# vr308/Generalised-Gaussian-Processes

Hardware: AMD Instinct MI355X
Metric: ELBO evals/sec (higher is better)
Workload: dtype f64

## Files before the change

generalised-gaussian-processes_amd/_lib.py:

```python
from __future__ import annotations

import ctypes as C
import os

HERE = os.path.dirname(os.path.abspath(__file__))
LIB_PATH = os.path.join(HERE, "csrc", "libsgp_hip.so")

SGP_ABI_VERSION = 3
SGP_MAX_DIM = 32
SGP_MAX_INDUCING = 4096
KERNEL_IDS = {"rbf": 0, "matern32": 1, "matern52": 2, "composite": 3}
COMP_LEN = 33
OPT_CONTRACTION, OPT_ASM_OVERLAP, OPT_KFU_BUDGET_BYTES, OPT_COND_LIMIT, OPT_CU_BUDGET, OPT_TIMING, OPT_SHARED_DEVICE = range(7)
OUT_F, OUT_LOGMARG, OUT_TRACE, OUT_LOGDETB, OUT_QUAD, OUT_TRW, OUT_S2BAR, OUT_KAPPABAR, OUT_LEN = range(9)


class SgpLibraryError(RuntimeError):
    pass


class SgpStatusError(RuntimeError):
    def __init__(self, fn, status, text):
        super().__init__("%s returned %d: %s" % (fn, status, text))
        self.status = status


_vp, _i64, _i32, _dbl, _sz = C.c_void_p, C.c_int64, C.c_int, C.c_double, C.c_size_t
_dp = C.POINTER(C.c_double)
_ip = C.POINTER(C.c_int)

PROTOTYPES = {
    "sgp_abi_version": (_i32, []),
    "sgp_status_string": (C.c_char_p, [_i32]),
    "sgp_ctx_create": (_vp, [_i32]),
    "sgp_ctx_destroy": (None, [_vp]),
    "sgp_ctx_device": (_i32, [_vp]),
    "sgp_ctx_set_option": (_i32, [_vp, _i32, _dbl]),
    "sgp_ctx_get_option": (_dbl, [_vp, _i32]),
    "sgp_ctx_bind_thread": (None, [_vp]),
    "sgp_ctx_set_pass1_gate": (None, [_vp, _vp]),
    "sgp_ctx_contraction_last": (_i32, [_vp]),
    "sgp_ctx_contraction_would_use_i8": (_i32, [_vp, _i64, _i32]),
    "sgp_ctx_timing_last_ms": (_i32, [_vp, _i32, C.POINTER(C.c_float)]),
    "sgp_ctx_timing_last_rows": (_i64, [_vp, _i32]),
    "sgp_ctx_suffstats_workspace_bytes": (_sz, [_vp, _i64, _i32, _i32, _i32]),
    "sgp_ctx_suffstats_fwd": (_i32, [_vp, _vp, _i64, _vp, _vp, _i64, _dp, _dbl, _i64, _i32, _i32, _i32,
                                     _vp, _vp, _vp, _vp, _vp, _vp, _sz, _vp]),
    "sgp_ctx_suffstats_bwd": (_i32, [_vp, _vp, _i64, _vp, _vp, _i64, _dp, _dbl, _vp, _vp, _dbl, _vp, _i64, _i32, _i32, _i32,
                                     _vp, _vp, _vp, _vp, _sz, _vp]),
    "sgp_ctx_kuu_factor": (_i32, [_vp, _vp, _i32, _vp, _vp, _vp, _sz, _vp]),
    "sgp_ctx_kuu_factor_ex": (_i32, [_vp, _vp, _i32, _vp, _vp, _vp, _vp, _sz, _vp]),
    "sgp_ctx_bound_from_stats": (_i32, [_vp, _vp, _vp, _vp, _vp, _vp, _dbl, _i64, _i32, _i32, _vp,
                                        _vp, _vp, _vp, _vp, _vp, _vp, _vp, _sz, _vp]),
    "sgp_ctx_suffstats_whitened_workspace_bytes": (_sz, [_vp, _i64, _i32, _i32]),
    "sgp_ctx_suffstats_fwd_whitened": (_i32, [_vp, _vp, _i64, _vp, _vp, _i64, _dp, _dbl, _i64, _i32, _i32, _i32, _vp,
                                              _vp, _vp, _vp, _vp, _vp, _sz, _vp]),
    "sgp_ctx_suffstats_whitened_rows_workspace_bytes": (_sz, [_vp, _i64, _i32, _i32, _i32]),
    "sgp_ctx_suffstats_fwd_whitened_rows": (_i32, [_vp, _vp, _i64, _vp, _vp, _i64, _dp, _dbl, _i64, _i32, _i32, _i32, _vp,
                                                   _vp, _vp, _vp, _vp, _vp, _vp, _sz, _vp]),
    "sgp_ctx_suffstats_extended_workspace_bytes": (_sz, [_vp, _i64, _i32, _i32]),
    "sgp_ctx_suffstats_fwd_extended": (_i32, [_vp, _vp, _i64, _vp, _vp, _i64, _dp, _dbl, _i64, _i32, _i32, _i32, _vp, _i32,
                                              _vp, _vp, _vp, _vp, _vp, _vp, _vp, _sz, _vp]),
    "sgp_ctx_suffstats_fwd_extended_f16": (_i32, [_vp, _vp, _i64, _vp, _vp, _i64, _dp, _dbl, _i64, _i32, _i32, _i32, _vp, _i32,
                                                  _vp, _vp, _vp, _vp, _vp, _vp, _vp, _vp, _sz, _vp]),
    "sgp_ctx_suffstats_bwd_factored_workspace_bytes": (_sz, [_vp, _i64, _i32, _i32, _i32]),
    "sgp_ctx_suffstats_bwd_factored": (_i32, [_vp, _vp, _i64, _vp, _vp, _i64, _dp, _dbl, _vp, _vp, _dbl, _vp, _dbl, _i64, _i32, _i32, _i32,
                                              _vp, _vp, _vp, _vp, _vp, _sz, _vp]),
    "sgp_ctx_bound_from_whitened_stats": (_i32, [_vp, _vp, _vp, _vp, _vp, _dbl, _i64, _i32, _i32, _vp,
                                                 _vp, _vp, _vp, _vp, _vp, _vp, _vp, _vp, _sz, _vp]),
    "sgp_ctx_mixture_predict": (_i32, [_vp, _vp, _i64, _vp, _i64, _vp, _i64, _i64, _vp, _i64, _i32, _dp, _dp, _dp, _dbl, _i32, _i32, _i32, _i32,
                                       _dbl, _vp, _vp, _vp, _vp, _vp, _vp, _sz, _vp]),
    "sgp_ctx_mixture_predict_zs": (_i32, [_vp, _vp, _i64, _vp, _i64, _vp, _i64, _i64, _vp, _i64, _i64, _i32, _dp, _dp, _dp, _dbl, _i32, _i32, _i32, _i32, _dbl, _vp, _vp, _vp, _vp, _vp, _vp, _sz, _vp]),
    "sgp_timing_enable": (None, [_i32]),
    "sgp_timing_last_ms": (_i32, [_i32, C.POINTER(C.c_float)]),
    "sgp_timing_last_rows": (_i64, [_i32]),
    "sgp_set_asm_overlap": (None, [_i32]),
    "sgp_set_cond_limit": (None, [_dbl]),
    "sgp_suffstats_workspace_bytes": (_sz, [_i64, _i32, _i32]),
    "sgp_suffstats_workspace_bytes_ex": (_sz, [_i64, _i32, _i32, _i32]),
    "sgp_suffstats_bwd_workspace_bytes_ex": (_sz, [_i64, _i32, _i32, _i32]),
    "sgp_kfu_len": (_sz, [_i64, _i32]),
    "sgp_set_kfu_budget_bytes": (None, [_sz]),
    "sgp_set_contraction": (_i32, [_i32]),
    "sgp_contraction_last": (_i32, []),
    "sgp_set_pass1_gate": (None, [_vp]),
    "sgp_suffstats_fwd": (_i32, [_vp, _i64, _vp, _vp, _i64, _dp, _dbl, _i64, _i32, _i32, _i32,
                                 _vp, _vp, _vp, _vp, _vp, _vp, _sz, _vp]),
    "sgp_stats_packed_len": (_sz, [_i32]),
    "sgp_stats_pack_lower": (_i32, [_vp, _i32, _vp, _vp]),
    "sgp_stats_unpack_lower": (_i32, [_vp, _i32, _vp, _vp]),
    "sgp_kuu": (_i32, [_vp, _i64, _dp, _dbl, _dbl, _i32, _i32, _i32, _vp, _vp]),
    "sgp_chol_workspace_bytes": (_sz, [_i32]),
    "sgp_chol_lower": (_i32, [_vp, _i64, _i32, _vp, _vp, _sz, _vp]),
    "sgp_trsm_workspace_bytes": (_sz, [_i32, _i32]),
    "sgp_trsm_lower": (_i32, [_vp, _i64, _vp, _i64, _i32, _i32, _i32, _vp, _sz, _vp]),
    "sgp_logdiag_sum": (_i32, [_vp, _i64, _i32, _vp, _vp]),
    "sgp_bound_workspace_bytes": (_sz, [_i32, _i32]),
    "sgp_bound_factors_len": (_sz, [_i32]),
    "sgp_kuu_inverse_trace_len": (_sz, []),
    "sgp_kuu_inverse_trace": (_i32, [_vp, _i32, _vp, _vp]),
    "sgp_streaming_error_estimate": (_i32, [_vp, _vp, _dbl, _i64, _i32, _vp, _vp]),
    "sgp_streaming_error_bound": (_i32, [_vp, _dbl, _dbl, _vp, _vp]),
    "sgp_streaming_error_report": (_i32, [_vp, _i64, _vp, _dbl, _dbl, _i64, _i32, _vp, _vp]),
    "sgp_kuu_factor_len": (_sz, [_i32]),
    "sgp_kuu_factor_workspace_bytes": (_sz, [_i32]),
    "sgp_kuu_factor": (_i32, [_vp, _i32, _vp, _vp, _vp, _sz, _vp]),
    "sgp_kuu_factor_ex": (_i32, [_vp, _i32, _vp, _vp, _vp, _vp, _sz, _vp]),
    "sgp_bound_from_stats": (_i32, [_vp, _vp, _vp, _vp, _vp, _dbl, _i64, _i32, _i32, _vp,
                                    _vp, _vp, _vp, _vp, _vp, _vp, _vp, _sz, _vp]),
    "sgp_suffstats_whitened_workspace_bytes": (_sz, [_i64, _i32, _i32]),
    "sgp_suffstats_fwd_whitened": (_i32, [_vp, _i64, _vp, _vp, _i64, _dp, _dbl, _i64, _i32, _i32, _i32, _vp,
                                          _vp, _vp, _vp, _vp, _vp, _sz, _vp]),
    "sgp_suffstats_whitened_rows_workspace_bytes": (_sz, [_i64, _i32, _i32, _i32]),
    "sgp_suffstats_fwd_whitened_rows": (_i32, [_vp, _i64, _vp, _vp, _i64, _dp, _dbl, _i64, _i32, _i32, _i32, _vp,
                                               _vp, _vp, _vp, _vp, _vp, _vp, _sz, _vp]),
    "sgp_suffstats_extended_workspace_bytes": (_sz, [_i64, _i32, _i32]),
    "sgp_suffstats_fwd_extended": (_i32, [_vp, _i64, _vp, _vp, _i64, _dp, _dbl, _i64, _i32, _i32, _i32, _vp, _i32,
                                          _vp, _vp, _vp, _vp, _vp, _vp, _sz, _vp]),
    "sgp_suffstats_fwd_extended_ex": (_i32, [_vp, _i64, _vp, _vp, _i64, _dp, _dbl, _i64, _i32, _i32, _i32, _vp, _i32,
                                             _vp, _vp, _vp, _vp, _vp, _vp, _vp, _sz, _vp]),
    "sgp_phibar_dd_workspace_bytes": (_sz, [_i32]),
    "sgp_phibar_dd": (_i32, [_vp, _vp, _i32, _dbl, _vp, _vp, _vp, _sz, _vp]),
    "sgp_suffstats_bwd_lo_workspace_bytes": (_sz, [_i64, _i32, _i32]),
    "sgp_suffstats_bwd_lo": (_i32, [_vp, _i64, _vp, _vp, _i64, _dp, _dbl, _vp, _vp, _i64, _i32, _i32, _i32, _vp, _vp, _vp, _vp, _sz, _vp]),
    "sgp_suffstats_bwd_lo_workspace_bytes_ex": (_sz, [_i64, _i32, _i32, _i32]),
    "sgp_suffstats_bwd_lo_f16": (_i32, [_vp, _i64, _vp, _vp, _i64, _dp, _dbl, _vp, _vp, _vp, _i64, _i32, _i32, _i32, _vp, _vp, _vp, _vp, _sz, _vp]),
    "sgp_suffstats_fwd_extended_f16": (_i32, [_vp, _i64, _vp, _vp, _i64, _dp, _dbl, _i64, _i32, _i32, _i32, _vp, _i32,
                                              _vp, _vp, _vp, _vp, _vp, _vp, _vp, _vp, _sz, _vp]),
    "sgp_bound_from_whitened_stats": (_i32, [_vp, _vp, _vp, _vp, _dbl, _i64, _i32, _i32, _vp,
                                             _vp, _vp, _vp, _vp, _vp, _vp, _vp, _sz, _vp]),
    "sgp_bound_from_whitened_stats_ex": (_i32, [_vp, _vp, _vp, _vp, _dbl, _i64, _i32, _i32, _vp,
                                                _vp, _vp, _vp, _vp, _vp, _vp, _vp, _vp, _sz, _vp]),
    "sgp_suffstats_bwd_factored_workspace_bytes": (_sz, [_i64, _i32, _i32]),
    "sgp_suffstats_bwd_factored": (_i32, [_vp, _i64, _vp, _vp, _i64, _dp, _dbl, _vp, _vp, _dbl, _vp, _dbl, _i64, _i32, _i32, _i32,
# ... 87 lines not shown
```

generalised-gaussian-processes_amd/core.py:

```python
from __future__ import annotations

import math

import numpy as np

import torch

try:
    import torch.distributed as dist
except Exception:
    dist = None

from ._lib import COMP_LEN, OUT_F, OUT_LOGMARG, OUT_S2BAR, OUT_TRACE


class NotPositiveDefiniteError(RuntimeError):

    def __init__(self, info):
        super().__init__("matrix not positive definite: leading minor of order %d (1..M: Kuu, M+1..2M: B)" % info)
        self.info = info


class SgpTimeoutError(RuntimeError):

# ... 53 lines not shown
        self.predicted = estimate
        self.open = not (estimate < 0.5 * tol) if self.open else not (estimate <= tol)

    def note_bound(self, bound, tol):
        if math.isfinite(bound) and bound > 0.0:
            self.predicted = self.ratio * bound
            self.open = not (self.predicted < 0.5 * tol)


def _world(group):
    if dist is None or not dist.is_available() or not dist.is_initialized():
        return 1
    return dist.get_world_size(group)


class CollapsedBound:

    WHITENED_MAX_WORK = 1 << 20

    def __init__(self, X, y, kernel="rbf", jitter=0.0, engine=None, group=None, form="auto"):
        if engine is None:
            from .engine import HipEngine
            engine = HipEngine(X.device if X.is_cuda else None)
        self.engine = engine
        if X.dim() == 1:
            X = X[:, None]
        self.X = X.to(dtype=torch.float64, device=engine.device).contiguous()
        self.y = y.to(dtype=torch.float64, device=engine.device).reshape(-1).contiguous()
        if self.X.shape[0] != self.y.shape[0]:
            raise ValueError("X has %d rows, y has %d" % (self.X.shape[0], self.y.shape[0]))
        self.d = int(self.X.shape[1])
        self.kernel = kernel
        self.jitter = float(jitter)
        if form not in ("auto", "streaming", "whitened", "extended"):
            raise ValueError("form must be 'auto', 'streaming', 'extended' or 'whitened'")
        self.form = form
        self.group = group
        self.world = _world(group)
        n_local = int(self.X.shape[0])
        if self.world > 1:
            t = torch.tensor([n_local], dtype=torch.int64, device=engine.device)
            dist.all_reduce(t, group=group)
            self.N = int(t.item())
            dist.all_reduce(t.fill_(n_local), op=dist.ReduceOp.MAX, group=group)
            self._rows_for_form = int(t.item())
        else:
            self.N = n_local
            self._rows_for_form = n_local
        self.n_evals = 0
        self.n_grads = 0
        self.n_collectives = 0
        self._kfu = None
        self._kfu_f16 = None
        self.kfu_budget_bytes = 64 << 30
        self.whitened_rows_min_work = 1 << 26
        self.factored_adjoint = True
        self.fused = True
        self._small = None
        self.overlap_tail = True
        self.overlap_min_work = 1 << 21
        self.early_check_min_work = 1 << 28
        self._side = None
        self.streaming_tol = 1e-9
        self.extended_level = 2
        self.extended_range = 16384.0
        self.extended_grad_range = 3.0
        self.extended_dd_phibar = True
        self.extended_lo = True
        self.extended_grad_range_lo = 1000.0
        self.extended_lo_max_correction = 1e-4
        self._lo_skip, self._lo_pause = 0, 0
        self.last_lo_correction = None
        self.n_lo_rejections = 0
        self.guard = GuardState()
        self.last_estimate = None
        self.last_tier = None
        self.n_guard_reruns = 0
        self.n_direct_whitened = 0
        self.n_extended = 0
        self.n_timeout_retries = 0
        self._phi_diag = None

    def _allreduce(self, buf):
        if self.world > 1:
            dist.all_reduce(buf, group=self.group)
            self.n_collectives += 1
        return buf

    def _allreduce_stats(self, stats, M):
        if self.world > 1:
            e = self.engine
            if hasattr(e, "pack_lower"):
                tri = e.pack_lower(stats, M)
                dist.all_reduce(tri, group=self.group)
                e.unpack_lower(tri, M, stats)
            else:
                dist.all_reduce(stats, group=self.group)
            self.n_collectives += 1
        return stats

    def _fetch(self, res, upto=None):
        buf = res["buf"] if upto is None else res["buf"][:upto]
        host = buf.detach().to("cpu")
        o, info = self.engine.read_result(host)
        if info < 0:
            raise SgpTimeoutError()
        return o, info, host

    def _prep_Z(self, Z):
        if Z.dim() == 1:
            Z = Z[:, None]
        return Z.detach().to(dtype=torch.float64, device=self.engine.device).contiguous()

    def _kfu_for(self, M):
        e = self.engine
        if not hasattr(e, "kfu_buffer"):
            return None
        n_local = int(self.X.shape[0])
        need = ((max(n_local, 1) + 255) // 256 * 256) * ((M + 127) // 128 * 128)
        if need * 8 > self.kfu_budget_bytes:
            return None
        if self._kfu is None or self._kfu.numel() < need:
            self._kfu = e.kfu_buffer(n_local, M)
        return self._kfu

    def _kfu_f16_for(self, M):
        e = self.engine
        if not hasattr(e, "kfu_f16_buffer"):
            return None
        n_local = int(self.X.shape[0])
        need = ((max(n_local, 1) + 255) // 256 * 256) * ((M + 127) // 128 * 128)
        if need * 10 > self.kfu_budget_bytes:
            return None
        if self._kfu_f16 is None or self._kfu_f16.numel() < need:
            self._kfu_f16 = e.kfu_f16_buffer(n_local, M)
        return self._kfu_f16

    def _small_ok(self, M, want_gz=False, sf2=1.0):
        e = self.engine
        if self.kernel == "composite" and (want_gz or float(sf2) != 1.0):
            return False
        return (self.fused and self.world == 1 and self.form != "streaming" and hasattr(e, "small_eval")
                and e.small_supported(int(self.X.shape[0]), int(M), self.d, self.kernel))

    def _small_eval(self, Z, theta_host, mode, want_grad, want_gz, composite=None):
        e = self.engine
        nt = len(theta_host)
        if self._small is None or self._small[0].numel() != nt:
            pin = e.device.type == "cuda"
            host = torch.empty(nt, dtype=torch.float64, pin_memory=pin)
            self._small = (host, torch.empty(nt, dtype=torch.float64, device=e.device), e.small_result(nt - 2)[0], host.numpy())
        host, dev_theta, buf, host_np = self._small
        host_np[:] = theta_host
        dev_theta.copy_(host, non_blocking=True)
        kw = {"composite": composite} if composite is not None else {}
        out, gz, _ = e.small_eval(self.X, self.y, Z, dev_theta, self.jitter, self.kernel, mode=mode, want_grad=want_grad,
                                  want_gz=want_gz, out=buf, **kw)
        h = out.detach().to("cpu")
        info = int(h.numpy()[nt + 3:nt + 4].view("int32")[0])
        if info < 0:
            if hasattr(e, "small_reset"):
                e.small_reset()
            raise SgpTimeoutError()
        return h, info, gz

    def _whitened(self, M):
        if self.form == "auto":
            return hasattr(self.engine, "suffstats_whitened") and self._rows_for_form * int(M) <= self.WHITENED_MAX_WORK
        return self.form == "whitened"

    def _side_state(self, M):
        e = self.engine
        if self._side is None:
            if getattr(e, "_side_stream", None) is None:
                e._side_stream = torch.cuda.Stream(device=e.device, priority=-1)
            self._side = (e._side_stream, (torch.cuda.Event(), torch.cuda.Event()), {})
        bufs = self._side[2].get(M)
# ... 68 lines not shown

    def _forward(self, Z, ls, sf2, s2, with_adjoints, want_factors=False, extra=0, tier=TIER_STREAMING, report=False, want_lo=True):
        e = self.engine
        M = int(Z.shape[0])
        result = e.result_buffer(extra)
        if tier == TIER_EXTENDED:
            self.n_extended += 1
            Kuu = e.kuu(Z, ls, sf2, self.jitter, self.kernel)
            linv, _ = e.kuu_factor(Kuu, info=result[2], trace_out=self._trace_buf() if report else None)
            kfu = self._kfu_for(M) if with_adjoints else None
            diag = None
            if report:
                if self._phi_diag is None or self._phi_diag.numel() < M:
                    self._phi_diag = e.empty(M)
                diag = self._phi_diag
            dd = with_adjoints and self.extended_dd_phibar and hasattr(e, "phibar_dd")
            lo = dd and want_lo and kfu is not None and self._bwd_lo_ok(M)
            kfu_f16 = self._kfu_f16_for(M) if lo else None
            packed = e.suffstats_extended(self.X, self.y, Z, ls, sf2, linv, self.kernel, kfu=kfu, level=self.extended_level,
                                          **({"phi_diag": diag} if diag is not None else {}), **({"kfu_f16": kfu_f16} if kfu_f16 is not None else {}))
            self._allreduce_stats(packed, M)
            res = e.bound(Kuu, packed, s2, self.N, with_adjoints=with_adjoints, want_factors=want_factors, kuu_linv=linv,
                          result=result, whitened=True, **({"want_cw": True} if dd else {}))
            if dd:
                res["Phibar"], res["Phibar_lo"] = e.phibar_dd(res["Cw"], linv, s2, want_lo=lo)
                res["Cw"] = None
            if report:
                self._allreduce(diag[:M])
                e.streaming_error_report(diag, 1, self._trace_buf(), sf2, s2, self.N, M, result)
                res["reported"] = True
            res.update(packed=packed, kfu=kfu, kfu_f16=kfu_f16, t_keep=None, linv=linv)
            return res
        if tier == TIER_WHITENED:
            Kuu = e.kuu(Z, ls, sf2, self.jitter, self.kernel)
            rep = report and self.kernel != "composite"
            linv, _ = e.kuu_factor(Kuu, info=result[2], trace_out=self._trace_buf() if rep else None)
            factored = with_adjoints and self.factored_adjoint and hasattr(e, "suffstats_bwd_factored")
            t_keep = None
            if (hasattr(e, "suffstats_whitened_rows") and self.kernel != "composite"
                    and int(self.X.shape[0]) * M >= self.whitened_rows_min_work):
                t_keep = self._kfu_for(M) if factored else None
                packed = e.suffstats_whitened_rows(self.X, self.y, Z, ls, sf2, linv, self.kernel, t_out=t_keep)
            else:
                packed = e.suffstats_whitened(self.X, self.y, Z, ls, sf2, linv, self.kernel)
            self._allreduce_stats(packed, M)
            kw = {"want_cw": True} if factored else {}
            res = e.bound(Kuu, packed, s2, self.N, with_adjoints=with_adjoints, want_factors=want_factors, kuu_linv=linv,
                          result=result, whitened=True, **kw)
            if rep:
                e.streaming_error_report(None, 1, self._trace_buf(), sf2, s2, self.N, M, result)
                res["reported"] = True
            res.update(packed=packed, kfu=None, t_keep=t_keep, linv=linv)
            return res
        kfu = self._kfu_for(M) if with_adjoints else None
        gate = None
        guard = report
        trace = self._trace_buf() if guard and hasattr(e, "kuu_factor") else None
        overlap = (self.overlap_tail and hasattr(e, "kuu_factor") and e.device.type == "cuda"
                   and int(self.X.shape[0]) * M >= self.overlap_min_work)
        if overlap:
            main = torch.cuda.current_stream(e.device)
            side, (z_ready, ready), (Kuu, linv) = self._side_state(M)
            z_ready.record(main)
            side.wait_event(z_ready)
            e.kuu(Z, ls, sf2, self.jitter, self.kernel, out=Kuu, stream=side)
            e.kuu_factor(Kuu, info=result[2], trace_out=trace, out=linv, stream=side)
            ready.record(side)
            if (hasattr(e, "would_use_i8") and self.kernel != "composite" and int(self.X.shape[0]) >= 300 * M
                    and e.would_use_i8(int(self.X.shape[0]), M)):
                gate = ready
        try:
            packed = e.suffstats(self.X, self.y, Z, ls, sf2, self.kernel, kfu=kfu, **({"gate": gate} if gate is not None else {}))
            self._allreduce_stats(packed, M)
        finally:
            if overlap:
                main.wait_event(ready)
        if overlap:
            res = e.bound(Kuu, packed, s2, self.N, with_adjoints=with_adjoints, want_factors=want_factors, kuu_linv=linv,
                          result=result)
        elif guard and hasattr(e, "kuu_factor"):
            Kuu = e.kuu(Z, ls, sf2, self.jitter, self.kernel)
            linv, _ = e.kuu_factor(Kuu, info=result[2], trace_out=trace)
            res = e.bound(Kuu, packed, s2, self.N, with_adjoints=with_adjoints, want_factors=want_factors, kuu_linv=linv,
                          result=result)
        else:
            Kuu = e.kuu(Z, ls, sf2, self.jitter, self.kernel)
            res = e.bound(Kuu, packed, s2, self.N, with_adjoints=with_adjoints, want_factors=want_factors, result=result)
        if guard and trace is not None:
            e.streaming_error_report(packed, M + 1, trace, sf2, s2, self.N, M, result)
            res["reported"] = True
        res["packed"] = packed
        res["kfu"] = kfu
        return res

    def _pass2(self, res, Z, ls, sf2, s2, want_gz, g):
        e = self.engine
        if res.get("Cw") is not None:
            e.suffstats_bwd_factored(self.X, self.y, Z, ls, sf2, res["linv"], res["Cw"], s2, res["bbar"], -1.0 / (2.0 * float(s2)),
                                     self.kernel, want_gz=want_gz, out=g,
                                     **({"t_in": res["t_keep"]} if res.get("t_keep") is not None else {}))
        else:
            e.suffstats_bwd(self.X, self.y, Z, ls, sf2, res["Phibar"], res["bbar"], -1.0 / (2.0 * float(s2)),
                            self.kernel, want_gz=want_gz, out=g, kfu=res["kfu"])
            if res.get("Phibar_lo") is not None:
                n_lo = int(res.get("lo_slots", 0))
                e.suffstats_bwd_lo(self.X, self.y, Z, ls, sf2, res["Phibar_lo"], res["kfu"], g, self.kernel,
                                   **({"delta": g[g.numel() - n_lo:]} if n_lo else {}),
                                   **({"kfu_f16": res["kfu_f16"]} if res.get("kfu_f16") is not None else {}))
        if int(res.get("lo_slots", 0)) and res.get("Phibar_lo") is None:
            g[g.numel() - int(res["lo_slots"]):].zero_()
        self._allreduce(g)
        e.kuu_bwd(Z, ls, sf2, res["Kuubar"], g, self.kernel, want_gz=want_gz)

    def _evaluate(self, *args, **kw):
        try:
            return self._evaluate_once(*args, **kw)
        except SgpTimeoutError:
            e = self.engine
            if "shared_device" not in getattr(e, "OPTIONS", {}) or e.get_option("shared_device") != 0:
                raise
            e.set_option("shared_device", 1)
            self.n_timeout_retries += 1
            return self._evaluate_once(*args, **kw)

    def _evaluate_once(self, Z, ls, sf2, s2, with_grad=False, want_gz=False, want_factors=False, grad_reach=None, strict=False):
        e = self.engine
        M, d = int(Z.shape[0]), int(Z.shape[1])
        guard = self._guard_on(M)
        reach = self.extended_range
        if with_grad:
            reach = float(grad_reach) if grad_reach is not None else (self.extended_grad_range_lo if self._bwd_lo_ok(M) else self.extended_grad_range)
        ext_ok = self._extended_ok(M)
        if guard:
            tier = self.guard.start_tier(self.streaming_tol, reach, ext_ok)
            if strict and tier == TIER_WHITENED:
                tier = TIER_EXTENDED if ext_ok else TIER_STREAMING
            if tier != TIER_STREAMING:
                self.n_direct_whitened += 1
        else:
            tier = self._fixed_tier(M)
        nh = (e.hyper_len(self.kernel, d) if hasattr(e, "hyper_len") else d) if with_grad else 0
        lo_slots = (nh + 1) if (with_grad and guard and ext_ok and self._bwd_lo_ok(M)) else 0
        extra = nh + 1 + (M * d if want_gz else 0) + lo_slots if with_grad else 0
        if guard and with_grad and tier == TIER_EXTENDED and grad_reach is None and self._lo_skip > 0:
            self._lo_skip -= 1
            tier = TIER_WHITENED
        early = with_grad and self._rows_for_form * M >= self.early_check_min_work
        done = {}
        may_go_down = strict
        while True:
            res = self._forward(Z, ls, sf2, s2, with_adjoints=with_grad, want_factors=want_factors, extra=extra, tier=tier, report=guard,
                                want_lo=grad_reach is None)
            head = res["buf"].numel() - extra
            g = res["buf"][head:] if with_grad else None
            res["lo_slots"] = lo_slots
            grad_upto = None if lo_slots else head + nh + 1
# ... 270 lines not shown
```

generalised-gaussian-processes_amd/csrc/sgp_ctx.hip:

```cpp
#include "sgp_common.hpp"
#include "sgp_ctx.hpp"
#include "sgp_stream.hpp"
#include <cstdlib>
#include <new>

namespace sgp {

static int env_int(const char* name, int dflt) {
  const char* v = getenv(name);
  return v ? atoi(v) : dflt;
}

static void ctx_init(Ctx& c, int device) {
  c.device = device;
  c.contraction = env_int("SGP_CONTRACTION", 1);
  if (c.contraction < 0 || c.contraction > 2) c.contraction = 1;
  c.asm_overlap = env_int("SGP_ASM_OVERLAP", 0);
  c.kfu_budget = KFU_BUDGET_DEFAULT;
  c.syrk_skip_upper = env_int("SGP_SYRK_SKIP_UPPER", 1);
  c.syrk_waves = env_int("SGP_SYRK_WAVES", 4);
  c.syrk_glds = env_int("SGP_SYRK_GLDS", 0);
  c.i8_prio = env_int("SGP_I8_PRIO", 0);
  c.shared_device = env_int("SGP_SHARED_DEVICE", 0) != 0 ? 1 : 0;
}

Ctx& default_ctx() {
  static Ctx* c = [] {
    Ctx* p = new Ctx();
    int dev = 0;
    if (hipGetDevice(&dev) != hipSuccess) dev = 0;
    ctx_init(*p, dev);
    return p;
  }();
  return *c;
}

static thread_local Ctx* t_cur = nullptr;
static thread_local Ctx* t_bound = nullptr;
Ctx& cur_ctx() { return t_cur ? *t_cur : (t_bound ? *t_bound : default_ctx()); }
void bind_thread_ctx(void* ctx) { t_bound = static_cast<Ctx*>(ctx); }
CtxScope::CtxScope(void* ctx) : prev(t_cur) { t_cur = ctx ? static_cast<Ctx*>(ctx) : &default_ctx(); }
CtxScope::~CtxScope() { t_cur = prev; }

}

using namespace sgp;

static bool ctx_on_current_device(const sgp_ctx* ctx) {
  if (!ctx) return true;
  int dev = -1;
  if (hipGetDevice(&dev) != hipSuccess) return true;
  return dev == reinterpret_cast<const Ctx*>(ctx)->device;
}

extern "C" sgp_ctx* sgp_ctx_create(int device) {
  if (device < 0) return nullptr;
  Ctx* c = new (std::nothrow) Ctx();
  if (!c) return nullptr;
  ctx_init(*c, device);
  return reinterpret_cast<sgp_ctx*>(c);
}

extern "C" void sgp_ctx_destroy(sgp_ctx* ctx) {
  if (!ctx) return;
  Ctx* c = reinterpret_cast<Ctx*>(ctx);
  if (c == &default_ctx()) return;
  if (c->ev_ready)
    for (int s = 0; s < CTX_TIMING_SLOTS; ++s)
      for (int k = 0; k < 2; ++k) (void)hipEventDestroy(c->ev[s][k]);
  if (c->side) {
    (void)hipStreamDestroy(c->side);
    (void)hipEventDestroy(c->ev_fork);
    (void)hipEventDestroy(c->ev_join);
  }
  delete c;
}

extern "C" int sgp_ctx_set_option(sgp_ctx* ctx, int option, double value) {
  Ctx& c = ctx ? *reinterpret_cast<Ctx*>(ctx) : default_ctx();
  switch (option) {
    case SGP_OPT_CONTRACTION:
      if (!(value >= 0.0 && value <= 2.0)) return SGP_ERR_ARG;
      c.contraction = (int)value;
      return SGP_OK;
    case SGP_OPT_ASM_OVERLAP:
      if (!(value >= 0.0 && value <= 2.0)) return SGP_ERR_ARG;
      c.asm_overlap = (int)value;
      return SGP_OK;
    case SGP_OPT_KFU_BUDGET_BYTES:
      if (!(value >= 0.0)) return SGP_ERR_ARG;
      c.kfu_budget = value > 0.0 ? (size_t)value : KFU_BUDGET_DEFAULT;
      return SGP_OK;
    case SGP_OPT_COND_LIMIT:
      c.cond_limit = value >= 0.0 ? value : 1e13;
      return SGP_OK;
    case SGP_OPT_CU_BUDGET:
      c.cu_budget = value > 0.0 ? (int)value : 0;
      return SGP_OK;
    case SGP_OPT_TIMING:
      c.timing = value != 0.0 ? 1 : 0;
      return SGP_OK;
    case SGP_OPT_SHARED_DEVICE:
      c.shared_device = value != 0.0 ? 1 : 0;
      return SGP_OK;
    default:
      return SGP_ERR_ARG;
  }
}

extern "C" double sgp_ctx_get_option(const sgp_ctx* ctx, int option) {
  const Ctx& c = ctx ? *reinterpret_cast<const Ctx*>(ctx) : default_ctx();
  switch (option) {
    case SGP_OPT_CONTRACTION: return (double)c.contraction;
    case SGP_OPT_ASM_OVERLAP: return (double)c.asm_overlap;
    case SGP_OPT_KFU_BUDGET_BYTES: return (double)c.kfu_budget;
    case SGP_OPT_COND_LIMIT: return c.cond_limit;
    case SGP_OPT_CU_BUDGET: return (double)c.cu_budget;
    case SGP_OPT_TIMING: return (double)c.timing;
    case SGP_OPT_SHARED_DEVICE: return (double)c.shared_device;
    default: return -1.0;
  }
}

extern "C" void sgp_ctx_bind_thread(sgp_ctx* ctx) { sgp::bind_thread_ctx(ctx); }

extern "C" int sgp_ctx_device(const sgp_ctx* ctx) { return (ctx ? *reinterpret_cast<const Ctx*>(ctx) : default_ctx()).device; }

extern "C" void sgp_ctx_set_pass1_gate(sgp_ctx* ctx, void* hip_event) {
  (ctx ? *reinterpret_cast<Ctx*>(ctx) : default_ctx()).pass1_gate = (hipEvent_t)hip_event;
}

extern "C" int sgp_ctx_contraction_last(const sgp_ctx* ctx) {
  return (ctx ? *reinterpret_cast<const Ctx*>(ctx) : default_ctx()).contraction_used;
}

extern "C" size_t sgp_ctx_suffstats_workspace_bytes(const sgp_ctx* ctx, int64_t N, int M, int d, int caller_owns_kfu) {
  CtxScope scope(const_cast<sgp_ctx*>(ctx));
  return sgp_suffstats_workspace_bytes_ex(N, M, d, caller_owns_kfu);
}
extern "C" int sgp_ctx_suffstats_fwd(sgp_ctx* ctx, const double* X, int64_t ldx, const double* y, const double* Z, int64_t ldz,
                                     const double* inv_ls, double sf2, int64_t N, int M, int d, int kernel_id, double* Phi, double* b,
                                     double* yy, double* kappa, double* Kfu_out, void* ws, size_t ws_bytes, sgp_stream_t stream) {
  if (!ctx_on_current_device(ctx)) return SGP_ERR_ARG;
  CtxScope scope(ctx);
  return sgp_suffstats_fwd(X, ldx, y, Z, ldz, inv_ls, sf2, N, M, d, kernel_id, Phi, b, yy, kappa, Kfu_out, ws, ws_bytes, stream);
}
extern "C" int sgp_ctx_suffstats_bwd(sgp_ctx* ctx, const double* X, int64_t ldx, const double* y, const double* Z, int64_t ldz,
                                     const double* inv_ls, double sf2, const double* Phibar, const double* bbar, double kappabar,
                                     const double* Kfu_in, int64_t N, int M, int d, int kernel_id, double* g_ls, double* g_sf2,
                                     double* g_Z, void* ws, size_t ws_bytes, sgp_stream_t stream) {
  if (!ctx_on_current_device(ctx)) return SGP_ERR_ARG;
  CtxScope scope(ctx);
  return sgp_suffstats_bwd(X, ldx, y, Z, ldz, inv_ls, sf2, Phibar, bbar, kappabar, Kfu_in, N, M, d, kernel_id, g_ls, g_sf2, g_Z, ws,
                           ws_bytes, stream);
}
extern "C" int sgp_ctx_kuu_factor(sgp_ctx* ctx, const double* Kuu, int M, double* Linv_out, int* info, void* ws, size_t ws_bytes,
                                  sgp_stream_t stream) {
  if (!ctx_on_current_device(ctx)) return SGP_ERR_ARG;
  CtxScope scope(ctx);
  return sgp_kuu_factor(Kuu, M, Linv_out, info, ws, ws_bytes, stream);
}
extern "C" int sgp_ctx_kuu_factor_ex(sgp_ctx* ctx, const double* Kuu, int M, double* Linv_out, int* info, double* trace_out, void* ws,
                                     size_t ws_bytes, sgp_stream_t stream) {
  if (!ctx_on_current_device(ctx)) return SGP_ERR_ARG;
  CtxScope scope(ctx);
  return sgp_kuu_factor_ex(Kuu, M, Linv_out, info, trace_out, ws, ws_bytes, stream);
}
extern "C" int sgp_ctx_bound_from_stats(sgp_ctx* ctx, const double* Kuu, const double* Phi, const double* b, const double* yy,
                                        const double* kappa, double s2, int64_t N, int M, int with_adjoints, double* out,
                                        double* Phibar, double* bbar, double* Kuubar, double* factors, const double* kuu_linv,
                                        int* info, void* ws, size_t ws_bytes, sgp_stream_t stream) {
  if (!ctx_on_current_device(ctx)) return SGP_ERR_ARG;
  CtxScope scope(ctx);
  return sgp_bound_from_stats(Kuu, Phi, b, yy, kappa, s2, N, M, with_adjoints, out, Phibar, bbar, Kuubar, factors, kuu_linv, info, ws,
                              ws_bytes, stream);
}
extern "C" int sgp_ctx_mixture_predict(sgp_ctx* ctx, const double* X, int64_t ldx, const double* y, int64_t N, const double* Xs,
                                       int64_t ldxs, int64_t T, const double* Z, int64_t ldz, int S, const double* inv_ls,
                                       const double* sf2, const double* s2, double jitter, int M, int d, int kernel_id, int pred_noise,
                                       double gate_jitter, double* mean, double* var, double* cov, int* info, int* gate_info, void* ws,
                                       size_t ws_bytes, sgp_stream_t stream) {
  if (!ctx_on_current_device(ctx)) return SGP_ERR_ARG;
  CtxScope scope(ctx);
  return sgp_mixture_predict(X, ldx, y, N, Xs, ldxs, T, Z, ldz, S, inv_ls, sf2, s2, jitter, M, d, kernel_id, pred_noise, gate_jitter,
                             mean, var, cov, info, gate_info, ws, ws_bytes, stream);
}

extern "C" size_t sgp_ctx_suffstats_whitened_workspace_bytes(const sgp_ctx* ctx, int64_t N, int M, int d) {
  CtxScope scope(const_cast<sgp_ctx*>(ctx));
  return sgp_suffstats_whitened_workspace_bytes(N, M, d);
}
extern "C" int sgp_ctx_suffstats_fwd_whitened(sgp_ctx* ctx, const double* X, int64_t ldx, const double* y, const double* Z, int64_t ldz,
                                              const double* inv_ls, double sf2, int64_t N, int M, int d, int kernel_id,
                                              const double* kuu_linv, double* W, double* u, double* yy, double* kappa, void* ws,
                                              size_t ws_bytes, sgp_stream_t stream) {
  if (!ctx_on_current_device(ctx)) return SGP_ERR_ARG;
  CtxScope scope(ctx);
  return sgp_suffstats_fwd_whitened(X, ldx, y, Z, ldz, inv_ls, sf2, N, M, d, kernel_id, kuu_linv, W, u, yy, kappa, ws, ws_bytes, stream);
}
extern "C" size_t sgp_ctx_suffstats_whitened_rows_workspace_bytes(const sgp_ctx* ctx, int64_t N, int M, int d, int caller_owns_t) {
  CtxScope scope(const_cast<sgp_ctx*>(ctx));
  return sgp_suffstats_whitened_rows_workspace_bytes(N, M, d, caller_owns_t);
}
extern "C" int sgp_ctx_suffstats_fwd_whitened_rows(sgp_ctx* ctx, const double* X, int64_t ldx, const double* y, const double* Z,
                                                   int64_t ldz, const double* inv_ls, double sf2, int64_t N, int M, int d, int kernel_id,
                                                   const double* kuu_linv, double* W, double* u, double* yy, double* kappa,
                                                   double* T_out, void* ws, size_t ws_bytes, sgp_stream_t stream) {
// ... 62 lines not shown
```

generalised-gaussian-processes_amd/csrc/sgp_ctx.hpp:

```cpp
#pragma once
#include <hip/hip_runtime.h>
#include <cstddef>
#include <cstdint>

namespace sgp {

constexpr int CTX_TIMING_SLOTS = 3;

struct Ctx {
  int device = 0;
  int contraction = 1;
  int asm_overlap = 0;
  size_t kfu_budget = 0;
  double cond_limit = 1e13;
  int cu_budget = 0;
  int timing = 0;
  int shared_device = 0;
  int syrk_skip_upper = 1, syrk_waves = 4, syrk_glds = 0, i8_prio = 0;
  int contraction_used = 0;
  hipEvent_t pass1_gate = nullptr;
  int64_t syrk_timed_rows = 0;
  hipEvent_t ev[CTX_TIMING_SLOTS][2] = {};
  int ev_ready = 0, ev_used[CTX_TIMING_SLOTS] = {0, 0, 0};
  hipStream_t side = nullptr;
  hipEvent_t ev_fork = nullptr, ev_join = nullptr;
};

Ctx& default_ctx();
Ctx& cur_ctx();

void bind_thread_ctx(void* ctx);

struct CtxScope {
  Ctx* prev;
  explicit CtxScope(void* ctx);
  ~CtxScope();
  CtxScope(const CtxScope&) = delete;
  CtxScope& operator=(const CtxScope&) = delete;
};

}
```

generalised-gaussian-processes_amd/csrc/sgp_stream.hpp:

```cpp
#pragma once
#include <cstdlib>
#include "sgp_common.hpp"

namespace sgp {

constexpr int TILE = 128;
constexpr int NB = 16;
constexpr int KROW = 2 * TILE + 16;
constexpr int ASM_ROWS = 256;
constexpr int TARGET_WGS = 2048;
constexpr int RESIDENT_WGS = 512;
constexpr size_t KFU_BUDGET_DEFAULT = size_t(16) << 30;
size_t stream_kfu_budget();

static inline int dp_for(int d) {
  const int opts[] = {2, 4, 8, 16, 24, 32};
  for (int o : opts)
    if (d <= o) return o;
  return -1;
}

struct StreamPlan {
  int Mp, ntr, ntiles, DP;
  int64_t Npad;
// ... 108 lines not shown
  if (taper_b_on && nsb % 32 == 0 && nblocks / nsb >= 8) {
    const int B = (int)(nsb / 8);
    p.taper_b[0] = 3 * B / 4; p.taper_b[1] = B / 4; p.taper_b[2] = B / 4; p.taper_b[3] = B / 2;
    p.nsplit_b = 8 * (p.taper_b[0] + p.taper_b[1] + p.taper_b[2] + p.taper_b[3]);
  }
  return p;
}

enum { TIMING_ASSEMBLE = 0, TIMING_SYRK = 1, TIMING_KBAR = 2, TIMING_SLOTS = 3 };
void timing_begin(int slot, hipStream_t st);
void timing_end(int slot, hipStream_t st);

struct PadSymJob {
  const double* P = nullptr;
  double* out = nullptr;
  const double* vec = nullptr;
  double* vout = nullptr;
};
void stream_prologue(const StreamPlan& p, const KernArgs& ka, const double* X, int64_t ldx, const double* y,
                     const double* Z, int64_t ldz, int64_t N, int M, double* Xs, double* ys, double* Zs, double* yypart,
                     hipStream_t st, const PadSymJob& pad = PadSymJob());
void stream_assemble(const StreamPlan& p, int kid, const double* Xs, const double* ys, const double* Zs, int64_t row0,
                     int64_t rows, int64_t N, int M, double* Kfu, double* bpart, hipStream_t st);

constexpr int I8_SPLIT_ROWS = 16384;
static inline int i8_nsplit(int64_t rows, int Mp) {
  const int nrt = Mp / 128, ntiles = nrt * (nrt + 1);
  int64_t lo = (rows + I8_SPLIT_ROWS - 1) / I8_SPLIT_ROWS;
  lo = (lo + 7) / 8 * 8;
  if (lo < 8) lo = 8;
  int64_t best = lo;
  double best_waste = 2.0;
  for (int64_t cand = lo; cand <= 2 * lo + 8; cand += 8) {
    if (cand > lo && rows / cand < 2048) break;
    const double r = (double)ntiles * (double)cand / 256.0;
    const double rounds = (double)(int64_t)(r + 0.999999);
    const double waste = (rounds - r) / rounds;
    if (waste < best_waste - 1e-9) {
      best_waste = waste;
      best = cand;
    }
  }
  return (int)best;
}
__host__ __device__ inline void i8_split_steps(int64_t nsteps, int nsplit, int split, int64_t& c0, int64_t& c1) {
  const int64_t per = (nsteps + nsplit - 1) / nsplit;
  c0 = (int64_t)split * per;
  c1 = c0 + per;
  if (c0 > nsteps) c0 = nsteps;
  if (c1 > nsteps) c1 = nsteps;
}
void i8_assemble(const StreamPlan& p, int kid, const double* Xs, const double* ys, const double* Zs, int64_t row0, int64_t rows,
                 int64_t N, int M, uint8_t* Q, double* Kfu , double* bpart, hipStream_t st,
                 uint16_t* Kh = nullptr );
int i8_contract(const uint8_t* Q, int Mp, int64_t rows, int nsplit, int accumulate, double* slab, hipStream_t st, double* slab_lo = nullptr,
                int level = 1);

}
```

generalised-gaussian-processes_amd/csrc/sgp_suffstats_bwd.hip:

```cpp
#include "sgp_common.hpp"
#include "sgp_stream.hpp"
#include "sgp_composite.hpp"
#include "sgp_dense.hpp"
#include <cstdlib>

namespace sgp {

constexpr int BK = 16;
constexpr int ALD = BK + 2;
constexpr int BROW = TILE + 16;
constexpr int A_DBL = TILE * ALD;
constexpr int B_DBL = BK * BROW;
constexpr int BSM = 2 * (A_DBL + B_DBL);
constexpr int CS = 129;
static_assert(64 * CS <= BSM, "epilogue image must fit in the main-loop buffers");

__global__ void bwd_pad_vec_kernel(const double* __restrict__ in, int64_t n, int64_t npad, double* __restrict__ out) {
  for (int64_t i = (int64_t)blockIdx.x * blockDim.x + threadIdx.x; i < npad; i += (int64_t)gridDim.x * blockDim.x)
    out[i] = i < n ? in[i] : 0.0;
}
__global__ void bwd_pad_plain_kernel(const double* __restrict__ P, int M, int Mp, double scale, double* __restrict__ out) {
  const int64_t total = (int64_t)Mp * Mp;
  for (int64_t e = (int64_t)blockIdx.x * blockDim.x + threadIdx.x; e < total; e += (int64_t)gridDim.x * blockDim.x) {
    const int r = (int)(e / Mp), c = (int)(e - (int64_t)r * Mp);
    out[e] = (r < M && c < M) ? scale * P[e] : 0.0;
  }
}
__global__ void bwd_pad_small_kernel(const double* __restrict__ P, int M, int Mp, double scale, double* __restrict__ out) {
  const int64_t total = (int64_t)Mp * Mp;
  for (int64_t e = (int64_t)blockIdx.x * blockDim.x + threadIdx.x; e < total; e += (int64_t)gridDim.x * blockDim.x) {
    const int r = (int)(e / Mp), c = (int)(e - (int64_t)r * Mp);
    out[e] = (r < M && c < M) ? scale * P[(int64_t)r * M + c] : 0.0;
  }
}

template <int KID>
__device__ __forceinline__ double hprime_from_k(double kp, double r2) {
  if constexpr (KID == SGP_KERNEL_RBF) {
    return -0.5 * kp;
  } else if constexpr (KID == SGP_KERNEL_MATERN32) {
    const double a = 1.7320508075688772 * sqrt(r2);
    return -1.5 * kp / (1.0 + a);
  } else {
    const double a = 2.23606797749979 * sqrt(r2);
    return -(5.0 / 6.0) * (1.0 + a) * kp / (1.0 + a + a * a * (1.0 / 3.0));
  }
}

template <int DP, int KID, bool KP>
constexpr bool kbar_two_pass() {
#ifdef SGP_AB_KBAR_TWO_PASS_ALL
  return KP && KID == SGP_KERNEL_RBF;
#else
  return KP && DP > 8 && KID == SGP_KERNEL_RBF;
#endif
}
// ... 150 lines not shown
            gl[k] = fresh ? 0.0 : gmine[(size_t)(j0 + k) * 256];
            gz[k] = (fresh || !GZ) ? 0.0 : gmine[(size_t)(DP + j0 + k) * 256];
          }
#pragma unroll 2
          for (int i = 0; i < 32; ++i) {
            const double* __restrict__ xq = Xs + (nbase + i) * DP + j0;
            const double E = Ct[half * 32 + i][erow];
#pragma unroll
            for (int k = 0; k < DG; ++k) {
              const double df = zg[k] - xq[k];
              const double t = E * df;
              if constexpr (GZ) gz[k] += t;
              gl[k] = fma(t, df, gl[k]);
            }
          }
#pragma unroll
          for (int k = 0; k < DG; ++k) {
            gmine[(size_t)(j0 + k) * 256] = gl[k];
            if constexpr (GZ) gmine[(size_t)(DP + j0 + k) * 256] = gz[k];
          }
        }
        __syncthreads();
      }
      gmine[(size_t)(2 * DP) * 256] = gs;
    } else {
    double zrow[DP], gl[DP], gz[DP], gs;
#pragma unroll
    for (int j = 0; j < DP; ++j) {
      zrow[j] = Zs[(size_t)(m0 + erow) * DP + j];
      gl[j] = first ? 0.0 : gmine[(size_t)j * 256];
      gz[j] = (first || !want_gz) ? 0.0 : gmine[(size_t)(DP + j) * 256];
    }
    gs = first ? 0.0 : gmine[(size_t)(2 * DP) * 256];
#pragma unroll
    for (int h = 0; h < 2; ++h) {
      if (wi == h) {
#pragma unroll
        for (int u = 0; u < 4; ++u)
#pragma unroll
          for (int v = 0; v < 4; ++v)
#pragma unroll
            for (int r = 0; r < 4; ++r) Ct[u * 16 + l4 + 4 * r][wj * 64 + v * 16 + l15] = acc[u][v][r];
      }
      __syncthreads();
#if defined(SGP_AB_KBAR_NO_EPI_MATH)
      for (int i = 0; i < 32; ++i) gs += Ct[half * 32 + i][erow];
      if (false)
#endif
      SGP_KBAR_EPI_UNROLL
      for (int i = 0; i < 32; ++i) {
        const int nl = half * 32 + i;
        const int64_t n = row0 + r0 + h * 64 + nl;
        const double* __restrict__ xq = Xs + n * DP;
        double df[DP];
        double r2 = 0.0;
#pragma unroll
        for (int j = 0; j < DP; ++j) {
          df[j] = zrow[j] - xq[j];
          r2 = fma(df[j], df[j], r2);
        }
        double kp, hp;
        kprofile_grad<KID>(r2, kp, hp);
        const double msk = n < N ? mmask : 0.0;
        const double kbar = (2.0 * sf2 * Ct[nl][erow] + bbm * ys[n]) * msk;
        gs = fma(kbar, kp, gs);
        const double E = kbar * sf2 * hp;
#pragma unroll
        for (int j = 0; j < DP; ++j) {
          const double t = E * df[j];
          if constexpr (GZ) gz[j] += t;
          gl[j] = fma(t, df[j], gl[j]);
        }
      }
      __syncthreads();
    }
#pragma unroll
    for (int j = 0; j < DP; ++j) {
      gmine[(size_t)j * 256] = gl[j];
      if (want_gz) gmine[(size_t)(DP + j) * 256] = gz[j];
    }
    gmine[(size_t)(2 * DP) * 256] = gs;
    }
  }

  double gl[DP], gz[DP], gs;
  {
    const bool any = nb0 < nb1;
#pragma unroll
    for (int j = 0; j < DP; ++j) {
      gl[j] = any ? gmine[(size_t)j * 256] : 0.0;
      gz[j] = (any && want_gz) ? gmine[(size_t)(DP + j) * 256] : 0.0;
    }
    gs = any ? gmine[(size_t)(2 * DP) * 256] : 0.0;
  }
  double* scratch = smem;
  if (want_gz) {
#pragma unroll
    for (int j = 0; j < DP; ++j) {
      __syncthreads();
      if (half == 1) scratch[erow] = gz[j];
      __syncthreads();
      if (half == 0) {
        double* dst = gzpart + ((size_t)split * Mp + m0 + erow) * DP + j;
        const double v = gz[j] + scratch[erow];
        *dst = accumulate ? *dst + v : v;
      }
    }
  }
  auto block_total = [&](double v, int slot) {
    v = wave_sum(v);
    __syncthreads();
    if (lane == 0) scratch[wave] = v;
    __syncthreads();
    if (tid == 0) {
      double* dst = glpart + ((size_t)split * nmb + mb) * (DP + 1) + slot;
      const double t = scratch[0] + scratch[1] + scratch[2] + scratch[3];
      *dst = accumulate ? *dst + t : t;
    }
  };
#pragma unroll
  for (int j = 0; j < DP; ++j) block_total(gl[j], j);
  block_total(gs, DP);
}

__global__ __launch_bounds__(256) void bwd_reduce_kernel(const double* __restrict__ gzpart, const double* __restrict__ glpart,
// ... 96 lines not shown
  if (kernel_id == SGP_KERNEL_COMPOSITE) {
    CompSpec cs;
    if (comp_parse(inv_ls, d, &cs) != SGP_OK) return SGP_ERR_ARG;
    fill_zero(g_sf2, 1, (hipStream_t)stream);
    return comp_suffstats_bwd(X, ldx, y, Z, ldz, cs, Phibar, bbar, kappabar, N, M, d, g_ls, g_Z, ws, ws_bytes, (hipStream_t)stream);
  }
  StreamPlan p = make_stream_plan(N, M, d);
  if (Kfu_in) p.sc_rows = p.Npad;
  BwdWs w = carve_bwd(ws, p, Kfu_in == nullptr);
  if (!ws || ws_bytes < w.bytes) return SGP_ERR_WORKSPACE;
  hipStream_t st = (hipStream_t)stream;

  KernArgs ka;
  for (int j = 0; j < SGP_MAX_DIM; ++j) ka.inv_ls[j] = j < d ? inv_ls[j] : 0.0;
  ka.sf2 = sf2;
  ka.d = d;

  {
    PadSymJob pad;
    pad.P = Phibar; pad.out = w.Pb; pad.vec = bbar; pad.vout = w.bb;
    stream_prologue(p, ka, X, ldx, y, Z, ldz, N, M, w.Xs, w.ys, w.Zs, w.yypart, st, pad);
  }

  const int want_gz = g_Z != nullptr;
  const int grid = p.nmb * p.nsplit_b;
  auto launch = [&](const double* Kfu, int64_t row0, int64_t nblocks, int accumulate) {
    int bps = (int)((nblocks + p.nsplit_b - 1) / p.nsplit_b);
    if (bps < 1) bps = 1;
    switch (p.DP) {
      case 2: launch_bwd<2>(kernel_id, grid, st, Kfu, w, sf2, row0, nblocks, bps, N, M, p, want_gz, accumulate); break;
      case 4: launch_bwd<4>(kernel_id, grid, st, Kfu, w, sf2, row0, nblocks, bps, N, M, p, want_gz, accumulate); break;
      case 8: launch_bwd<8>(kernel_id, grid, st, Kfu, w, sf2, row0, nblocks, bps, N, M, p, want_gz, accumulate); break;
      case 16: launch_bwd<16>(kernel_id, grid, st, Kfu, w, sf2, row0, nblocks, bps, N, M, p, want_gz, accumulate); break;
      case 24: launch_bwd<24>(kernel_id, grid, st, Kfu, w, sf2, row0, nblocks, bps, N, M, p, want_gz, accumulate); break;
      default: launch_bwd<32>(kernel_id, grid, st, Kfu, w, sf2, row0, nblocks, bps, N, M, p, want_gz, accumulate); break;
    }
  };
  if (p.Npad == 0) launch(nullptr, 0, 0, 0);
  for (int64_t r0 = 0; r0 < p.Npad; r0 += p.sc_rows) {
    const int64_t rows = (p.Npad - r0) < p.sc_rows ? (p.Npad - r0) : p.sc_rows;
    const double* Kfu = Kfu_in ? Kfu_in + r0 * p.Mp : nullptr;
    if (!Kfu_in) {
      stream_assemble(p, kernel_id, w.Xs, w.ys, w.Zs, r0, rows, N, M, w.Kfu, w.bpart, st);
      Kfu = w.Kfu;
    }
    timing_begin(TIMING_KBAR, st);
    launch(Kfu, r0, rows / TILE, r0 > 0 ? 1 : 0);
    timing_end(TIMING_KBAR, st);
  }
  const int64_t tot = (int64_t)M * d;
  const int rg = (int)((tot + 255) / 256 < 1024 ? (tot + 255) / 256 : 1024);
  bwd_reduce_kernel<<<rg < 1 ? 1 : rg, 256, 0, st>>>(w.gzpart, w.glpart, p.nsplit_b, p.nmb, p.Mp, M, p.DP, ka,
                                                    kappabar * (double)N, g_ls, g_sf2, g_Z);
  return check_launch();
}

static int bwd_fully_factored() {
  static const int v = getenv("SGP_BWD_FULLY_FACTORED") ? atoi(getenv("SGP_BWD_FULLY_FACTORED")) : 0;
  return v;
}
static size_t bwd_factored_workspace_bytes(int64_t N, int M, int d, bool caller_t) {
  if (N < 0 || M <= 0 || d <= 0 || d > SGP_MAX_DIM || M > SGP_MAX_INDUCING) return 0;
  StreamPlan p = make_stream_plan(N, M, d);
  p.sc_rows = p.Npad;
  const int nt = (caller_t ? 0 : 1) + (bwd_fully_factored() ? 1 : 0);
  const size_t fast = carve_bwd(nullptr, p, !caller_t).bytes + nt * round_up64((int64_t)(p.Npad > 0 ? p.Npad : 1) * p.Mp * 8 + 256, 256) +
                      3 * round_up64((int64_t)p.Mp * p.Mp * 8 + 256, 256);
  const size_t comp = d <= COMP_MAX_DIM ? comp_bwd_factored_workspace_bytes(N, M, d) : 0;
  return fast > comp ? fast : comp;
}
extern "C" size_t sgp_suffstats_bwd_factored_workspace_bytes(int64_t N, int M, int d) { return bwd_factored_workspace_bytes(N, M, d, false); }
extern "C" size_t sgp_suffstats_bwd_factored_workspace_bytes_ex(int64_t N, int M, int d, int caller_owns_t) {
  return bwd_factored_workspace_bytes(N, M, d, caller_owns_t != 0);
}

static int bwd_factored(const double* X, int64_t ldx, const double* y, const double* Z, int64_t ldz, const double* inv_ls, double sf2,
                        const double* kuu_linv, const double* Cw, double s2, const double* bbar, double kappabar, int64_t N, int M,
                        int d, int kernel_id, const double* T_in, double* g_ls, double* g_sf2, double* g_Z, void* ws, size_t ws_bytes,
                        sgp_stream_t stream) {
  if (!Z || !inv_ls || !kuu_linv || !Cw || !bbar || !g_ls || !g_sf2 || N < 0 || M <= 0 || d <= 0 || ldz < d || !(s2 > 0.0))
    return SGP_ERR_ARG;
  if (N > 0 && (!X || !y || ldx < d)) return SGP_ERR_ARG;
  if (kernel_id < 0 || kernel_id > SGP_KERNEL_COMPOSITE) return SGP_ERR_ARG;
  if (T_in && kernel_id == SGP_KERNEL_COMPOSITE) return SGP_ERR_ARG;
  if (d > SGP_MAX_DIM || M > SGP_MAX_INDUCING) return SGP_ERR_DIM;
  hipStream_t st = (hipStream_t)stream;
  if (!ws || ws_bytes < bwd_factored_workspace_bytes(N, M, d, T_in != nullptr)) return SGP_ERR_WORKSPACE;
  if (kernel_id == SGP_KERNEL_COMPOSITE) {
    CompSpec cs;
    if (comp_parse(inv_ls, d, &cs) != SGP_OK) return SGP_ERR_ARG;
    fill_zero(g_sf2, 1, st);
    return comp_suffstats_bwd_factored(X, ldx, y, Z, ldz, cs, kuu_linv, Cw, s2, bbar, kappabar, N, M, d, g_ls, g_Z, ws, ws_bytes, st);
  }
  const int fully = bwd_fully_factored();
  StreamPlan p = make_stream_plan(N, M, d);
  p.sc_rows = p.Npad;
  BwdWs w = carve_bwd(ws, p, T_in == nullptr);
  Carver c(static_cast<char*>(ws) + round_up64((int64_t)w.bytes, 256));
  const size_t rows = (size_t)(p.Npad > 0 ? p.Npad : 1);
  double* T1 = T_in ? nullptr : c.take<double>(rows * p.Mp);
  double* T2 = fully ? c.take<double>(rows * p.Mp) : nullptr;
  double* P2 = c.take<double>((size_t)p.Mp * p.Mp);
  double* Q0 = c.take<double>((size_t)p.Mp * p.Mp);
  double* R = c.take<double>((size_t)p.Mp * p.Mp);

  KernArgs ka;
// ... 71 lines not shown
```

generalised-gaussian-processes_amd/csrc/sgp_suffstats_fwd.hip:

```cpp
#include "sgp_common.hpp"
#include "sgp_stream.hpp"
#include "sgp_dense.hpp"
#include "sgp_composite.hpp"
#include "sgp_ctx.hpp"
#include <cstdlib>

namespace sgp {

static_assert(TIMING_SLOTS == CTX_TIMING_SLOTS, "timing slots");
size_t stream_kfu_budget() { return cur_ctx().kfu_budget; }

void timing_begin(int slot, hipStream_t st) {
  Ctx& c = cur_ctx();
  if (!c.timing) return;
  if (!c.ev_ready) {
    bool ok = true;
    for (int s = 0; s < TIMING_SLOTS; ++s)
      for (int k = 0; k < 2; ++k) ok = (hipEventCreate(&c.ev[s][k]) == hipSuccess) && ok;
    if (!ok) return;
    c.ev_ready = 1;
  }
  if (hipEventRecord(c.ev[slot][0], st) != hipSuccess) c.ev_used[slot] = 0;
}
void timing_end(int slot, hipStream_t st) {
// ... 754 lines not shown
  return w;
}

}

using namespace sgp;

static int ctx_timing_last_ms(Ctx& c, int slot, float* ms) {
  if (slot < 0 || slot >= TIMING_SLOTS || !ms) return SGP_ERR_ARG;
  if (!c.ev_ready || !c.ev_used[slot]) return SGP_ERR_ARG;
  if (hipEventSynchronize(c.ev[slot][1]) != hipSuccess) return SGP_ERR_LAUNCH;
  return hipEventElapsedTime(ms, c.ev[slot][0], c.ev[slot][1]) == hipSuccess ? SGP_OK : SGP_ERR_LAUNCH;
}
extern "C" int sgp_ctx_timing_last_ms(sgp_ctx* ctx, int slot, float* ms) {
  return ctx_timing_last_ms(ctx ? *reinterpret_cast<Ctx*>(ctx) : default_ctx(), slot, ms);
}
extern "C" int64_t sgp_ctx_timing_last_rows(const sgp_ctx* ctx, int slot) {
  return slot == TIMING_SYRK ? (ctx ? *reinterpret_cast<const Ctx*>(ctx) : default_ctx()).syrk_timed_rows : -1;
}
extern "C" int sgp_ctx_contraction_would_use_i8(const sgp_ctx* ctx, int64_t N, int M) {
  if (N <= 0 || M <= 0 || M > SGP_MAX_INDUCING) return 0;
  return i8_rule((ctx ? *reinterpret_cast<const Ctx*>(ctx) : default_ctx()).contraction, round_up64(N, ASM_ROWS), padded_m(M)) ? 1 : 0;
}

extern "C" void sgp_timing_enable(int on) { default_ctx().timing = on ? 1 : 0; }
extern "C" int sgp_timing_last_ms(int slot, float* ms) { return ctx_timing_last_ms(default_ctx(), slot, ms); }
extern "C" int64_t sgp_timing_last_rows(int slot) { return sgp_ctx_timing_last_rows(nullptr, slot); }
extern "C" void sgp_set_asm_overlap(int mode) { default_ctx().asm_overlap = (mode < 0 || mode > 2) ? 0 : mode; }
extern "C" int sgp_set_contraction(int mode) {
  const int prev = default_ctx().contraction;
  default_ctx().contraction = (mode < 0 || mode > 2) ? 1 : mode;
  return prev;
}
extern "C" int sgp_contraction_last(void) { return default_ctx().contraction_used; }
extern "C" void sgp_set_pass1_gate(void* hip_event) { default_ctx().pass1_gate = (hipEvent_t)hip_event; }
extern "C" void sgp_set_kfu_budget_bytes(size_t bytes) { default_ctx().kfu_budget = bytes ? bytes : KFU_BUDGET_DEFAULT; }

extern "C" size_t sgp_kfu_len(int64_t N, int M) {
  if (N < 0 || M <= 0 || M > SGP_MAX_INDUCING) return 0;
  return (size_t)round_up64(N > 0 ? N : 1, ASM_ROWS) * padded_m(M);
}

static size_t fwd_workspace_bytes(int64_t N, int M, int d, bool library_kfu) {
  if (N < 0 || M <= 0 || d <= 0 || d > SGP_MAX_DIM || M > SGP_MAX_INDUCING) return 0;
  StreamPlan p = make_stream_plan(N, M, d);
  const size_t fast = carve_fwd(nullptr, p, library_kfu, p.sc_rows).bytes, comp = comp_fwd_workspace_bytes(N, M);
  return fast > comp ? fast : comp;
}
extern "C" size_t sgp_suffstats_workspace_bytes(int64_t N, int M, int d) { return fwd_workspace_bytes(N, M, d, true); }
extern "C" size_t sgp_suffstats_workspace_bytes_ex(int64_t N, int M, int d, int caller_owns_kfu) {
  return fwd_workspace_bytes(N, M, d, caller_owns_kfu == 0);
}

extern "C" int sgp_suffstats_fwd(const double* X, int64_t ldx, const double* y, const double* Z, int64_t ldz,
                                 const double* inv_ls, double sf2, int64_t N, int M, int d, int kernel_id,
                                 double* Phi, double* b, double* yy, double* kappa, double* Kfu_out, void* ws,
                                 size_t ws_bytes, sgp_stream_t stream) {
  Ctx& cx = cur_ctx();
  hipEvent_t gate = cx.pass1_gate;
  cx.pass1_gate = nullptr;
  if (!Z || !inv_ls || !Phi || !b || !yy || !kappa || N < 0 || M <= 0 || d <= 0 || ldz < d) return SGP_ERR_ARG;
  if (N > 0 && (!X || !y || ldx < d)) return SGP_ERR_ARG;
  if (kernel_id < 0 || kernel_id > SGP_KERNEL_COMPOSITE) return SGP_ERR_ARG;
  if (d > SGP_MAX_DIM || M > SGP_MAX_INDUCING) return SGP_ERR_DIM;
  if (kernel_id == SGP_KERNEL_COMPOSITE) {
    CompSpec cs;
    if (comp_parse(inv_ls, d, &cs) != SGP_OK) return SGP_ERR_ARG;
    return comp_suffstats_fwd(X, ldx, y, Z, ldz, cs, N, M, d, Phi, b, yy, kappa, ws, ws_bytes, (hipStream_t)stream);
  }
  StreamPlan p = make_stream_plan(N, M, d);
  const int64_t qrows = p.sc_rows;
  if (Kfu_out) p.sc_rows = p.Npad;
  FwdWs w = carve_fwd(ws, p, Kfu_out == nullptr, qrows);
  if (!ws || ws_bytes < w.bytes) return SGP_ERR_WORKSPACE;
  hipStream_t st = (hipStream_t)stream;

  KernArgs ka;
  for (int j = 0; j < SGP_MAX_DIM; ++j) ka.inv_ls[j] = j < d ? inv_ls[j] : 0.0;
  ka.sf2 = sf2;
  ka.d = d;

  stream_prologue(p, ka, X, ldx, y, Z, ldz, N, M, w.Xs, w.ys, w.Zs, w.yypart, st);
  double* Kfu = Kfu_out ? Kfu_out : w.Kfu;
  const int grid = p.ntiles * p.nsplit;
  if (p.Npad == 0) {
    syrk_tile_kernel<4, false, false><<<grid, 256, 0, st>>>(Kfu, p.Mp, 0, SplitMap{{0, 0, 0, 0}, 1}, p.ntiles, 0, w.slab, p.nsplit);
  }
  auto contract = [&](const double* K, int64_t nchunks, const SplitMap& smap, int nsplit, int accum, double* slab) {
    launch_syrk(cx, K, p.Mp, nchunks, smap, p.ntiles, nsplit, accum, slab, st);
  };
  int nslabs = p.nsplit;
  int head_ns = 0;
  int64_t head_chunks = 0;
  const bool use_i8 = i8_rule(cx.contraction, p.Npad, p.Mp);
  cx.contraction_used = use_i8 ? 1 : 0;
  if (!use_i8) gate = nullptr;
  if (p.Npad > 0 && !use_i8) head_block(p, p.Npad / NB, &head_ns, &head_chunks);
  if (use_i8) {
    const int ns = i8_nsplit(qrows, p.Mp);
    for (int64_t r0 = 0; r0 < p.Npad; r0 += qrows) {
      const int64_t rows = (p.Npad - r0) < qrows ? (p.Npad - r0) : qrows;
      timing_begin(TIMING_ASSEMBLE, st);
      i8_assemble(p, kernel_id, w.Xs, w.ys, w.Zs, r0, rows, N, M, w.Q, Kfu_out ? Kfu_out + (size_t)r0 * p.Mp : nullptr, w.bpart, st);
      timing_end(TIMING_ASSEMBLE, st);
      if (gate && hipStreamWaitEvent(st, gate, 0) != hipSuccess) return SGP_ERR_LAUNCH;
      gate = nullptr;
      timing_begin(TIMING_SYRK, st);
      if (i8_contract(w.Q, p.Mp, rows, ns, r0 > 0 ? 1 : 0, w.slab, st) != SGP_OK) return SGP_ERR_LAUNCH;
      timing_end(TIMING_SYRK, st);
      cx.syrk_timed_rows = rows;
    }
    nslabs = ns;
  } else if (head_ns > 0) {
    const int64_t hrows = head_chunks * NB, trows = p.Npad - hrows, tchunks = trows / NB;
    const bool side = cx.asm_overlap == 1 && side_stream_ready(cx);
    double* head_slab = w.slab + (size_t)p.nsplit * p.ntiles * TILE * TILE;
    const int hcps = (int)((head_chunks + head_ns - 1) / head_ns);
    const int tcps = (int)((tchunks + p.nsplit - 1) / p.nsplit);
    const SplitMap hmap{{0, 0, 0, 0}, hcps < 1 ? 1 : hcps};
    const SplitMap tmap{{p.taper[0], p.taper[1], p.taper[2], p.taper[3]}, tcps < 1 ? 1 : tcps};
    timing_begin(TIMING_ASSEMBLE, st);
    stream_assemble(p, kernel_id, w.Xs, w.ys, w.Zs, 0, hrows, N, M, Kfu, w.bpart, st);
    bool forked = false;
    if (side && hipEventRecord(cx.ev_fork, st) == hipSuccess && hipStreamWaitEvent(cx.side, cx.ev_fork, 0) == hipSuccess) {
      stream_assemble(p, kernel_id, w.Xs, w.ys, w.Zs, hrows, trows, N, M, Kfu + (size_t)hrows * p.Mp, w.bpart, cx.side);
      forked = hipEventRecord(cx.ev_join, cx.side) == hipSuccess;
      if (!forked) (void)hipStreamSynchronize(cx.side);
    } else {
      stream_assemble(p, kernel_id, w.Xs, w.ys, w.Zs, hrows, trows, N, M, Kfu + (size_t)hrows * p.Mp, w.bpart, st);
    }
    timing_end(TIMING_ASSEMBLE, st);
    contract(Kfu, head_chunks, hmap, head_ns, 0, head_slab);
    if (forked && hipStreamWaitEvent(st, cx.ev_join, 0) != hipSuccess) (void)hipStreamSynchronize(cx.side);
    timing_begin(TIMING_SYRK, st);
    contract(Kfu + (size_t)hrows * p.Mp, tchunks, tmap, p.nsplit, 0, w.slab);
    timing_end(TIMING_SYRK, st);
    cx.syrk_timed_rows = trows;
    nslabs = p.nsplit + head_ns;
  } else {
    for (int64_t r0 = 0; r0 < p.Npad; r0 += p.sc_rows) {
      const int64_t rows = (p.Npad - r0) < p.sc_rows ? (p.Npad - r0) : p.sc_rows;
      timing_begin(TIMING_ASSEMBLE, st);
      stream_assemble(p, kernel_id, w.Xs, w.ys, w.Zs, r0, rows, N, M, Kfu, w.bpart, st);
      timing_end(TIMING_ASSEMBLE, st);
      const int64_t nchunks = rows / NB;
      const int cps = (int)((nchunks + p.nsplit - 1) / p.nsplit);
      const SplitMap smap{{p.taper[0], p.taper[1], p.taper[2], p.taper[3]}, cps < 1 ? 1 : cps};
      timing_begin(TIMING_SYRK, st);
      contract(Kfu, nchunks, smap, p.nsplit, r0 > 0 ? 1 : 0, w.slab);
      timing_end(TIMING_SYRK, st);
      cx.syrk_timed_rows = rows;
    }
  }
  const int nb32 = p.Mp / 32;
  reduce_phi_kernel<<<nb32 * (nb32 + 1) / 2, 256, 0, st>>>(w.slab, nslabs, p.ntiles, M, sf2 * sf2, Phi);
  bpart_stage1_kernel<<<dim3(p.Mp / 64, BRED_G), 256, 0, st>>>(w.bpart, p.Npad / ASM_ROWS * (use_i8 ? 1 : p.asm_sub), p.Mp, BRED_G, w.btmp);
  finalize_stats_kernel<<<(M + 255) / 256, 256, 0, st>>>(w.btmp, BRED_G, p.Mp, M, w.yypart, 256, sf2,
                                                         sf2 * (double)N, b, yy, kappa);
  return check_launch();
}

extern "C" size_t sgp_suffstats_whitened_rows_workspace_bytes(int64_t N, int M, int d, int caller_owns_t) {
  if (N < 0 || M <= 0 || d <= 0 || d > SGP_MAX_DIM || M > SGP_MAX_INDUCING) return 0;
  StreamPlan p = make_stream_plan(N, M, d);
  if (caller_owns_t) p.sc_rows = p.Npad;
  return carve_wh_rows(nullptr, p, caller_owns_t != 0).bytes;
}
extern "C" int sgp_suffstats_fwd_whitened_rows(const double* X, int64_t ldx, const double* y, const double* Z, int64_t ldz,
                                               const double* inv_ls, double sf2, int64_t N, int M, int d, int kernel_id,
                                               const double* kuu_linv, double* W, double* u, double* yy, double* kappa, double* T_out,
                                               void* ws, size_t ws_bytes, sgp_stream_t stream) {
  Ctx& cx = cur_ctx();
  if (!Z || !inv_ls || !kuu_linv || !W || !u || !yy || !kappa || N < 0 || M <= 0 || d <= 0 || ldz < d) return SGP_ERR_ARG;
  if (N > 0 && (!X || !y || ldx < d)) return SGP_ERR_ARG;
  if (kernel_id < 0 || kernel_id >= SGP_KERNEL_COMPOSITE) return SGP_ERR_ARG;
  if (d > SGP_MAX_DIM || M > SGP_MAX_INDUCING) return SGP_ERR_DIM;
  StreamPlan p = make_stream_plan(N, M, d);
  if (T_out) p.sc_rows = p.Npad;
  WhRowsWs w = carve_wh_rows(ws, p, T_out != nullptr);
  if (!ws || ws_bytes < w.bytes) return SGP_ERR_WORKSPACE;
  hipStream_t st = (hipStream_t)stream;
  KernArgs ka;
  for (int j = 0; j < SGP_MAX_DIM; ++j) ka.inv_ls[j] = j < d ? inv_ls[j] : 0.0;
  ka.sf2 = sf2;
  ka.d = d;
  stream_prologue(p, ka, X, ldx, y, Z, ldz, N, M, w.f.Xs, w.f.ys, w.f.Zs, w.f.yypart, st);
  transpose_square(kuu_linv, p.Mp, w.R, st);
  if (p.Npad == 0)
    syrk_tile_kernel<4, false, false><<<p.ntiles * p.nsplit, 256, 0, st>>>(w.f.Kfu, p.Mp, 0, SplitMap{{0, 0, 0, 0}, 1}, p.ntiles, 0, w.f.slab,
                                                                           p.nsplit);
  for (int64_t r0 = 0; r0 < p.Npad; r0 += p.sc_rows) {
    const int64_t rows = (p.Npad - r0) < p.sc_rows ? (p.Npad - r0) : p.sc_rows;
    double* T = T_out ? T_out + (size_t)r0 * p.Mp : w.T;
    timing_begin(TIMING_ASSEMBLE, st);
    stream_assemble(p, kernel_id, w.f.Xs, w.f.ys, w.f.Zs, r0, rows, N, M, w.f.Kfu, w.f.bpart, st);
    timing_end(TIMING_ASSEMBLE, st);
    GemmDesc g;
    g.A = w.f.Kfu; g.lda = p.Mp; g.B = w.R; g.ldb = p.Mp; g.C = T; g.ldc = p.Mp;
    g.m = (int)rows; g.n = p.Mp; g.k = p.Mp; g.khi_mask = 2;
    gemm(g, st);
    tpart_kernel<<<dim3((unsigned)(rows / ASM_ROWS), (p.Mp + 255) / 256), 256, 0, st>>>(T, w.f.ys, r0, p.Mp, w.f.bpart);
    const int64_t nchunks = rows / NB;
    const int cps = (int)((nchunks + p.nsplit - 1) / p.nsplit);
    const SplitMap smap{{p.taper[0], p.taper[1], p.taper[2], p.taper[3]}, cps < 1 ? 1 : cps};
    timing_begin(TIMING_SYRK, st);
    launch_syrk(cx, T, p.Mp, nchunks, smap, p.ntiles, p.nsplit, r0 > 0 ? 1 : 0, w.f.slab, st);
    timing_end(TIMING_SYRK, st);
    cx.syrk_timed_rows = rows;
  }
  const int nb32 = p.Mp / 32;
  reduce_phi_kernel<<<nb32 * (nb32 + 1) / 2, 256, 0, st>>>(w.f.slab, p.nsplit, p.ntiles, M, sf2 * sf2, W);
  bpart_stage1_kernel<<<dim3(p.Mp / 64, BRED_G), 256, 0, st>>>(w.f.bpart, p.Npad / ASM_ROWS, p.Mp, BRED_G, w.f.btmp);
// ... 74 lines not shown
```

generalised-gaussian-processes_amd/csrc/sgp_suffstats_i8.hip:

```cpp
#include <atomic>
#include "sgp_common.hpp"
#include "sgp_stream.hpp"
#include "sgp_ctx.hpp"
#include <cstdlib>
#include <type_traits>

namespace sgp {

typedef int i4v __attribute__((ext_vector_type(4)));
typedef int i16v __attribute__((ext_vector_type(16)));

constexpr int I8_NP = 7;
constexpr int I8_TR = 128, I8_TC = 64;
constexpr int I8_SCOLS = I8_TR + I8_TC;
constexpr int I8_STAGE_BYTES = 2 * I8_NP * I8_SCOLS * 16;
constexpr int I8_NSTAGE = 3;
constexpr int I8_PIECES = 2 * I8_NP * 3;
constexpr int I8_PPW = (I8_PIECES + 7) / 8;
constexpr int I8_LDS_BYTES = I8_NSTAGE * I8_STAGE_BYTES;

template <int DP, int KID, bool WK>
__global__ __launch_bounds__(256) void kfu_digits_kernel(const double* __restrict__ Xs, const double* __restrict__ ys,
                                                         const double* __restrict__ Zs, int64_t row0, int64_t N, int M, int Mp,
                                                         uint8_t* __restrict__ Q, double* __restrict__ Kfu, uint16_t* __restrict__ Kh,
                                                         double* __restrict__ bpart) {
  __shared__ double xs[ASM_ROWS][DP];
  __shared__ double ysh[ASM_ROWS];
  __shared__ double etab[EXP_TAB_N];
  const int64_t rbase = (int64_t)blockIdx.x * ASM_ROWS;
  {
    const double* src = Xs + (row0 + rbase) * DP;
    double* dst = &xs[0][0];
    for (int e = threadIdx.x; e < ASM_ROWS * DP; e += 256) dst[e] = src[e];
    ysh[threadIdx.x] = ys[row0 + rbase + threadIdx.x];
    sgp_exp_tab_load(etab);
  }
  __syncthreads();
  const int m = blockIdx.y * 256 + threadIdx.x;
  if (m >= Mp) return;
  const double zmask = m < M ? 1.0 : 0.0;
  double zr[DP];
#pragma unroll
  for (int j = 0; j < DP; ++j) zr[j] = Zs[(size_t)m * DP + j];

  constexpr unsigned long long C = 0x0080808080808080ULL;
  double bacc = 0.0;
#ifdef SGP_AB_DIGITS_NO_INTERIOR
  const bool interior = false;
#else
  const bool interior = (row0 + rbase + ASM_ROWS <= N) && ((int)(blockIdx.y * 256 + 255) < M);
#endif
  auto run = [&](auto masked_tag) {
  constexpr bool MASKED = decltype(masked_tag)::value;
  for (int g = 0; g < ASM_ROWS / 16; ++g) {
    unsigned lo[16], hi[16];
#pragma unroll
    for (int e = 0; e < 16; ++e) {
      const int i = g * 16 + e;
      const int64_t n = row0 + rbase + i;
      double r2 = 0.0;
#pragma unroll
      for (int j = 0; j < DP; ++j) {
        const double df = xs[i][j] - zr[j];
        r2 = fma(df, df, r2);
      }
      double kv = kprofile_tab<KID>(r2, etab);
      if constexpr (MASKED) kv *= (n < N ? zmask : 0.0);
      bacc = fma(kv, ysh[i], bacc);
      if constexpr (WK) {
        __builtin_nontemporal_store(kv, &Kfu[(rbase + i) * Mp + m]);
        if (Kh) {
          float kf = (float)kv;
          asm volatile("" : "+v"(kf));
          Kh[(rbase + i) * Mp + m] = __builtin_bit_cast(uint16_t, (_Float16)kf);
        }
      }
      const double th = fma(kv, 0x1p22, 0x1p52);
      const double hf = th - 0x1p52;
      const double tl = fma(-hf, 0x1p32, kv * 0x1p54) + 0x1.8p52;
      const unsigned long long tb = (unsigned long long)__double_as_longlong(tl);
      const unsigned q_hi = (unsigned)__double_as_longlong(th) - ((unsigned)(tb >> 32) & 1u);
      const unsigned long long q = ((unsigned long long)q_hi << 32) | (unsigned)tb;
      const unsigned long long qq = (q + C) ^ C;
      lo[e] = (unsigned)qq;
      hi[e] = (unsigned)(qq >> 32);
    }
    const size_t rb = (size_t)(rbase / 16 + g);
    i4v plane[8];
#pragma unroll
    for (int j = 0; j < 4; ++j) {
#pragma unroll
      for (int h = 0; h < 2; ++h) {
        const unsigned* s4 = (h ? hi : lo) + 4 * j;
        const unsigned u0 = __builtin_amdgcn_perm(s4[1], s4[0], 0x05010400u), u1 = __builtin_amdgcn_perm(s4[1], s4[0], 0x07030602u);
        const unsigned v0 = __builtin_amdgcn_perm(s4[3], s4[2], 0x05010400u), v1 = __builtin_amdgcn_perm(s4[3], s4[2], 0x07030602u);
        plane[4 * h + 0][j] = (int)__builtin_amdgcn_perm(v0, u0, 0x05040100u);
        plane[4 * h + 1][j] = (int)__builtin_amdgcn_perm(v0, u0, 0x07060302u);
        plane[4 * h + 2][j] = (int)__builtin_amdgcn_perm(v1, u1, 0x05040100u);
        if (h == 0) plane[3][j] = (int)__builtin_amdgcn_perm(v1, u1, 0x07060302u);
      }
    }
#pragma unroll
    for (int p = 0; p < I8_NP; ++p)
      __builtin_nontemporal_store(plane[p], reinterpret_cast<i4v*>(Q + ((rb * I8_NP + p) * Mp + m) * 16));
  }
  };
  if (interior) run(std::false_type{}); else run(std::true_type{});
  bpart[((row0 + rbase) / ASM_ROWS) * Mp + m] = bacc;
}

constexpr int I8_PSPLIT = 5;
#ifdef SGP_AB_I8_PAIRS34
constexpr int I8_MINSUM_DEFAULT = 5;
#else
constexpr int I8_MINSUM_DEFAULT = 6;
#endif
static_assert(2 * I8_PPW - 1 <= I8_PSPLIT * (I8_PSPLIT + 1) / 2, "every DMA piece must find its MFMA in the first half");

template <bool ACT, int I8_MINSUM, bool DD>
__device__ __forceinline__ void i8_tile_loop(uint8_t* lds, const uint8_t* __restrict__ Q, int Mp, int64_t c0, int64_t c1, int I0,
                                             int J0, int accumulate, double* __restrict__ out, size_t lo_off, int wave, int lane, int prio) {
  constexpr int I8_NG = 13 - I8_MINSUM;
  const int grp = wave >> 2, w4 = wave & 3;
  const int wi = (w4 >> 1) * 2 + grp, wj = w4 & 1;
  const int l32 = lane & 31, lh = lane >> 5;
  i16v acc[I8_NG];
#pragma unroll
  for (int g = 0; g < I8_NG; ++g)
#pragma unroll
    for (int r = 0; r < 16; ++r) acc[g][r] = 0;

  unsigned goff[I8_PPW];
  int soff[I8_PPW];
#pragma unroll
  for (int k = 0; k < I8_PPW; ++k) {
    int e = wave + 8 * k;
    if (e >= I8_PIECES) e -= I8_PIECES;
    const int rbl = e / (I8_NP * 3), rem = e % (I8_NP * 3), p = rem / 3, cg = rem % 3;
    const int col = cg < 2 ? I0 + cg * 64 : J0;
    goff[k] = (unsigned)(((rbl * I8_NP + p) * Mp + col + lane) * 16);
    soff[k] = __builtin_amdgcn_readfirstlane(((rbl * I8_NP + p) * I8_SCOLS + cg * 64) * 16);
  }
  const size_t gstride = (size_t)2 * I8_NP * Mp * 16;
  auto dma_piece = [&](const uint8_t* gbase, int sbase, int k) {
    __builtin_amdgcn_global_load_lds((const __attribute__((address_space(1))) void*)(gbase + goff[k]),
                                     (__attribute__((address_space(3))) void*)(lds + sbase + soff[k]), 16, 0, 0);
  };
  const int64_t nst = c1 - c0;
  auto wait_stage = [&](int64_t sE) {
    if (sE + 1 >= nst)
      __builtin_amdgcn_s_waitcnt(0 | (7 << 4) | (15 << 8));
    else
      __builtin_amdgcn_s_waitcnt((I8_PPW & 15) | ((I8_PPW >> 4) << 14) | (7 << 4) | (15 << 8));
  };
  auto bar = [&]() {
    __builtin_amdgcn_s_barrier();
    asm volatile("" ::: "memory");
  };
  i4v b[I8_NP], a[I8_NP];
  auto reads = [&](int64_t sidx) {
    if (ACT) {
      const uint8_t* sb = lds + (int)(sidx % I8_NSTAGE) * I8_STAGE_BYTES + lh * (I8_NP * I8_SCOLS * 16);
#pragma unroll
      for (int p = 0; p < I8_NP; ++p) {
        b[I8_NP - 1 - p] = *reinterpret_cast<const i4v*>(sb + ((I8_NP - 1 - p) * I8_SCOLS + I8_TR + wj * 32 + l32) * 16);
        a[p] = *reinterpret_cast<const i4v*>(sb + (p * I8_SCOLS + wi * 32 + l32) * 16);
      }
    }
    __builtin_amdgcn_sched_barrier(0);
  };
  auto half = [&](int p0, int p1, bool dma_on, int64_t sE) {
    if (prio) { if (dma_on) __builtin_amdgcn_s_setprio(1); else __builtin_amdgcn_s_setprio(0); }
    const bool pre = dma_on && sE + 2 < nst;
    const uint8_t* gnext = Q + (size_t)(c0 + sE + 2) * gstride;
    const int snext = (int)((sE + 2) % I8_NSTAGE) * I8_STAGE_BYTES;
    int issued = 0, kpiece = 0;
#pragma unroll
    for (int p = p0; p < p1; ++p)
#pragma unroll
      for (int r = (I8_MINSUM - p > 0 ? I8_MINSUM - p : 0); r < I8_NP; ++r) {
        if (ACT) acc[p + r - I8_MINSUM] = __builtin_amdgcn_mfma_i32_32x32x32_i8(a[p], b[r], acc[p + r - I8_MINSUM], 0, 0, 0);
        ++issued;
        if (dma_on && (issued & 1) && kpiece < I8_PPW) {
          __builtin_amdgcn_sched_barrier(0);
          if (pre) dma_piece(gnext, snext, kpiece);
          __builtin_amdgcn_sched_barrier(0);
          ++kpiece;
        }
      }
  };
  if (nst > 0) {
#pragma unroll
    for (int k = 0; k < I8_PPW; ++k) dma_piece(Q + (size_t)c0 * gstride, 0, k);
    if (nst > 1) {
#pragma unroll
      for (int k = 0; k < I8_PPW; ++k) dma_piece(Q + (size_t)(c0 + 1) * gstride, I8_STAGE_BYTES, k);
    }
    if (grp == 0) {
      for (int64_t sidx = 0; sidx < nst; ++sidx) {
        wait_stage(sidx);
        bar();
        reads(sidx);
        half(0, I8_PSPLIT, true, sidx);
        bar();
        half(I8_PSPLIT, I8_NP, false, sidx);
      }
      wait_stage(nst);
      bar();
    } else {
      wait_stage(0);
      bar();
      for (int64_t sidx = 0; sidx < nst; ++sidx) {
        bar();
        reads(sidx);
        half(0, I8_PSPLIT, true, sidx);
        __builtin_amdgcn_s_waitcnt(15 | (3 << 14) | (7 << 4) | (0 << 8));
        wait_stage(sidx + 1);
        bar();
        half(I8_PSPLIT, I8_NP, false, sidx + 1);
      }
    }
  }
  if (ACT) {
#pragma unroll
    for (int r = 0; r < 16; ++r) {
      const int row = wi * 32 + (r >> 2) * 8 + lh * 4 + (r & 3);
      double* dst = out + row * TILE + wj * 32 + l32;
      if constexpr (DD) {
#pragma clang fp contract(off)
        double hi = 0.0, lo = 0.0;
        if (accumulate) { hi = dst[0]; lo = dst[lo_off]; }
#pragma unroll
        for (int g = 0; g < I8_NG; ++g) {
          const double t = (double)acc[g][r] * __builtin_ldexp(1.0, 8 * (g + I8_MINSUM) - 108);
          const double sum = hi + t;
          const double z = sum - hi;
          lo += (hi - (sum - z)) + (t - z);
          hi = sum;
        }
        const double sum = hi + lo;
        dst[lo_off] = lo - (sum - hi);
        dst[0] = sum;
      } else {
        double v = 0.0;
#pragma unroll
        for (int g = 0; g < I8_NG; ++g) v = fma((double)acc[g][r], __builtin_ldexp(1.0, 8 * (g + I8_MINSUM) - 108), v);
        *dst = accumulate ? *dst + v : v;
      }
    }
  }
}

template <int MINSUM, bool DD>
__global__ __launch_bounds__(512, 1) void i8_syrk_tile_kernel(const uint8_t* __restrict__ Q, int Mp, int64_t nsteps, int nsplit,
                                                              int ntiles, int ntiles128, int accumulate, double* __restrict__ slab,
                                                              size_t lo_off, int prio) {
  extern __shared__ __attribute__((aligned(16))) uint8_t i8_lds[];
  const int id = blockIdx.x;
  const int xcd = id & 7, jj = id >> 3;
  const int t = jj % ntiles, split = (jj / ntiles) * 8 + xcd;
  if (split >= nsplit) return;
  int ti = (int)((sqrtf(4.0f * t + 1.0f) - 1.0f) * 0.5f);
  while ((ti + 1) * (ti + 2) <= t) ++ti;
  while (ti * (ti + 1) > t) --ti;
  const int tj = t - ti * (ti + 1);
  const int I0 = ti * I8_TR, J0 = tj * I8_TC;
  int64_t c0, c1;
  i8_split_steps(nsteps, nsplit, split, c0, c1);
  const int lane = threadIdx.x & 63;
  const int wave = __builtin_amdgcn_readfirstlane(threadIdx.x >> 6);
  double* out = slab + ((size_t)split * ntiles128 + (ti * (ti + 1) / 2 + (tj >> 1))) * (TILE * TILE) + (tj & 1) * I8_TC;
  const int grp = wave >> 2, w4 = wave & 3;
  const int wi = (w4 >> 1) * 2 + grp, wj = w4 & 1;
  if (J0 + 32 * wj <= I0 + 32 * wi + 31)
    i8_tile_loop<true, MINSUM, DD>(i8_lds, Q, Mp, c0, c1, I0, J0, accumulate, out, lo_off, wave, lane, prio);
  else
    i8_tile_loop<false, MINSUM, DD>(i8_lds, Q, Mp, c0, c1, I0, J0, accumulate, out, lo_off, wave, lane, prio);
}

template <int DP, bool WK>
static void launch_digits(int kid, dim3 grid, hipStream_t st, const double* Xs, const double* ys, const double* Zs, int64_t row0,
                          int64_t N, int M, int Mp, uint8_t* Q, double* Kfu, uint16_t* Kh, double* bpart) {
  switch (kid) {
    case SGP_KERNEL_RBF: kfu_digits_kernel<DP, SGP_KERNEL_RBF, WK><<<grid, 256, 0, st>>>(Xs, ys, Zs, row0, N, M, Mp, Q, Kfu, Kh, bpart); break;
    case SGP_KERNEL_MATERN32: kfu_digits_kernel<DP, SGP_KERNEL_MATERN32, WK><<<grid, 256, 0, st>>>(Xs, ys, Zs, row0, N, M, Mp, Q, Kfu, Kh, bpart); break;
    default: kfu_digits_kernel<DP, SGP_KERNEL_MATERN52, WK><<<grid, 256, 0, st>>>(Xs, ys, Zs, row0, N, M, Mp, Q, Kfu, Kh, bpart); break;
  }
}
template <bool WK>
static void launch_digits_dp(int DP, int kid, dim3 grid, hipStream_t st, const double* Xs, const double* ys, const double* Zs,
                             int64_t row0, int64_t N, int M, int Mp, uint8_t* Q, double* Kfu, uint16_t* Kh, double* bpart) {
  switch (DP) {
    case 2: launch_digits<2, WK>(kid, grid, st, Xs, ys, Zs, row0, N, M, Mp, Q, Kfu, Kh, bpart); break;
    case 4: launch_digits<4, WK>(kid, grid, st, Xs, ys, Zs, row0, N, M, Mp, Q, Kfu, Kh, bpart); break;
    case 8: launch_digits<8, WK>(kid, grid, st, Xs, ys, Zs, row0, N, M, Mp, Q, Kfu, Kh, bpart); break;
    case 16: launch_digits<16, WK>(kid, grid, st, Xs, ys, Zs, row0, N, M, Mp, Q, Kfu, Kh, bpart); break;
    case 24: launch_digits<24, WK>(kid, grid, st, Xs, ys, Zs, row0, N, M, Mp, Q, Kfu, Kh, bpart); break;
    default: launch_digits<32, WK>(kid, grid, st, Xs, ys, Zs, row0, N, M, Mp, Q, Kfu, Kh, bpart); break;
  }
}

void i8_assemble(const StreamPlan& p, int kid, const double* Xs, const double* ys, const double* Zs, int64_t row0, int64_t rows,
                 int64_t N, int M, uint8_t* Q, double* Kfu, double* bpart, hipStream_t st, uint16_t* Kh) {
  dim3 grid((unsigned)(rows / ASM_ROWS), (p.Mp + 255) / 256);
  if (Kfu)
    launch_digits_dp<true>(p.DP, kid, grid, st, Xs, ys, Zs, row0, N, M, p.Mp, Q, Kfu, Kh, bpart);
  else
    launch_digits_dp<false>(p.DP, kid, grid, st, Xs, ys, Zs, row0, N, M, p.Mp, Q, nullptr, nullptr, bpart);
}

int i8_contract(const uint8_t* Q, int Mp, int64_t rows, int nsplit, int accumulate, double* slab, hipStream_t st, double* slab_lo, int level) {
  Ctx& cx = cur_ctx();
  static std::atomic<bool> attr_done[64];
  int dev = 0;
  if (hipGetDevice(&dev) != hipSuccess || dev < 0) return SGP_ERR_LAUNCH;
  if (dev >= 64 || !attr_done[dev].load(std::memory_order_acquire)) {
    if (hipFuncSetAttribute((const void*)i8_syrk_tile_kernel<I8_MINSUM_DEFAULT, false>, hipFuncAttributeMaxDynamicSharedMemorySize,
                            I8_LDS_BYTES) != hipSuccess ||
        hipFuncSetAttribute((const void*)i8_syrk_tile_kernel<5, true>, hipFuncAttributeMaxDynamicSharedMemorySize, I8_LDS_BYTES) !=
            hipSuccess ||
        hipFuncSetAttribute((const void*)i8_syrk_tile_kernel<4, true>, hipFuncAttributeMaxDynamicSharedMemorySize, I8_LDS_BYTES) !=
            hipSuccess)
      return SGP_ERR_LAUNCH;
    if (dev < 64) attr_done[dev].store(true, std::memory_order_release);
  }
  const int nrt = Mp / I8_TR, ntiles = nrt * (nrt + 1), ntiles128 = nrt * (nrt + 1) / 2;
  const int prio = cx.i8_prio;
  if (slab_lo && level >= 2)
    i8_syrk_tile_kernel<4, true><<<nsplit * ntiles, 512, I8_LDS_BYTES, st>>>(Q, Mp, rows / 32, nsplit, ntiles, ntiles128, accumulate, slab,
                                                                             (size_t)(slab_lo - slab), prio);
  else if (slab_lo)
    i8_syrk_tile_kernel<5, true><<<nsplit * ntiles, 512, I8_LDS_BYTES, st>>>(Q, Mp, rows / 32, nsplit, ntiles, ntiles128, accumulate, slab,
                                                                             (size_t)(slab_lo - slab), prio);
  else
    i8_syrk_tile_kernel<I8_MINSUM_DEFAULT, false><<<nsplit * ntiles, 512, I8_LDS_BYTES, st>>>(Q, Mp, rows / 32, nsplit, ntiles, ntiles128,
                                                                                               accumulate, slab, 0, prio);
  return SGP_OK;
}

}
```

generalised-gaussian-processes_amd/engine.py:

```python
from __future__ import annotations

import ctypes as C
from typing import Optional, Sequence

import numpy as np
import torch

from . import _lib
from ._lib import COMP_LEN, KERNEL_IDS, OUT_LEN

RESULT_HEAD = OUT_LEN + 4


def _kernel_id(kernel) -> int:
    if isinstance(kernel, int):
        if kernel not in KERNEL_IDS.values():
            raise ValueError("unknown kernel id %r" % (kernel,))
        return kernel
    try:
        return KERNEL_IDS[str(kernel).lower()]
    except KeyError:
        raise ValueError("unknown kernel %r (expected one of %s)" % (kernel, sorted(KERNEL_IDS))) from None


class HipEngine:

    OPTIONS = {"contraction": _lib.OPT_CONTRACTION, "asm_overlap": _lib.OPT_ASM_OVERLAP, "kfu_budget_bytes": _lib.OPT_KFU_BUDGET_BYTES,
               "cond_limit": _lib.OPT_COND_LIMIT, "cu_budget": _lib.OPT_CU_BUDGET, "timing": _lib.OPT_TIMING,
               "shared_device": _lib.OPT_SHARED_DEVICE}

    def __init__(self, device: Optional[torch.device] = None, own_context: bool = False):
        self.lib = _lib.load_library()
        if not torch.cuda.is_available():
            raise _lib.SgpLibraryError("HipEngine needs a HIP device (torch.cuda.is_available() is False); "
                                       "there is no CPU implementation of the sparse-GP core")
        self.device = torch.device(device) if device is not None else torch.device("cuda", torch.cuda.current_device())
        self._ws = {}
        self._ctx = None
        if own_context:
            self._ctx = self.lib.sgp_ctx_create(self.device.index if self.device.index is not None else torch.cuda.current_device())
            if not self._ctx:
                raise _lib.SgpLibraryError("sgp_ctx_create failed")

    def __del__(self):
        ctx, self._ctx = getattr(self, "_ctx", None), None
        if ctx:
            try:
                self.lib.sgp_ctx_destroy(C.c_void_p(ctx))
            except Exception:
                pass

    class _ContextFree:

        def __init__(self, eng):
            self._eng = eng

        def __getattr__(self, name):
            eng = self._eng
            fn = getattr(eng.lib, name)
            if not eng._ctx:
                return fn
            bind = eng.lib.sgp_ctx_bind_thread

            def call(*a):
                bind(C.c_void_p(eng._ctx))
                try:
                    return fn(*a)
                finally:
                    bind(C.c_void_p(0))
            return call

    @property
    def _cf(self):
        cf = self.__dict__.get("_cf_obj")
        if cf is None:
            cf = self.__dict__["_cf_obj"] = HipEngine._ContextFree(self)
        return cf

    def _c(self):
        return C.c_void_p(self._ctx) if self._ctx else C.c_void_p(0)

    def set_option(self, name: str, value) -> float:
        prev = self.lib.sgp_ctx_get_option(self._c(), self.OPTIONS[name])
        _lib.check("sgp_ctx_set_option", self.lib.sgp_ctx_set_option(self._c(), self.OPTIONS[name], float(value)))
        return prev

    def get_option(self, name: str) -> float:
        return self.lib.sgp_ctx_get_option(self._c(), self.OPTIONS[name])

    def contraction_last(self) -> int:
        return int(self.lib.sgp_ctx_contraction_last(self._c()))

    def would_use_i8(self, N: int, M: int) -> bool:
        return bool(self.lib.sgp_ctx_contraction_would_use_i8(self._c(), int(N), int(M)))

    def _workspace(self, name: str, nbytes: int) -> torch.Tensor:
        buf = self._ws.get(name)
        if buf is None or buf.numel() < nbytes:
            buf = torch.empty(max(int(nbytes), 256), dtype=torch.uint8, device=self.device)
            self._ws[name] = buf
        return buf

    def _stream(self, stream=None):
        return C.c_void_p((stream if stream is not None else torch.cuda.current_stream(self.device)).cuda_stream)

    def _chk(self, t: torch.Tensor, name: str) -> torch.Tensor:
        if t.dtype != torch.float64 or t.device != self.device or not t.is_contiguous():
            raise ValueError("%s must be a contiguous float64 tensor on %s (got %s, %s)" % (name, self.device, t.dtype, t.device))
        return t

    @staticmethod
    def hyper_len(kernel, d: int) -> int:
        return COMP_LEN if _kernel_id(kernel) == KERNEL_IDS["composite"] else d

    def _inv_ls(self, ls: Sequence[float], d: int, kernel="rbf"):
        c = self.__dict__.get("_ils")
        if c is not None and type(ls) is list and c[1] == d and c[2] == kernel and c[0] == ls:
            return c[3]
        vals = [float(v) for v in (ls.tolist() if hasattr(ls, "tolist") else ls)]
        if _kernel_id(kernel) == KERNEL_IDS["composite"]:
            if len(vals) != COMP_LEN:
                raise ValueError("a composite kernel takes a %d-entry parameter block (got %d)" % (COMP_LEN, len(vals)))
            arr = (C.c_double * COMP_LEN)(*vals)
        else:
            if len(vals) == 1 and d > 1:
                vals = vals * d
            if len(vals) != d:
                raise ValueError("lengthscale has %d entries, expected %d" % (len(vals), d))
            arr = (C.c_double * d)(*[1.0 / v for v in vals])
        if type(ls) is list:
            self._ils = (list(ls), d, kernel, arr)
        return arr

    @staticmethod
    def _ptr(t: Optional[torch.Tensor]):
        return C.c_void_p(t.data_ptr()) if t is not None and t.numel() > 0 else C.c_void_p(0)

    def empty(self, *shape):
        return torch.empty(*shape, dtype=torch.float64, device=self.device)

    def kfu_buffer(self, N: int, M: int) -> torch.Tensor:
        return self.empty(self.lib.sgp_kfu_len(N, M))

    def kfu_f16_buffer(self, N: int, M: int) -> torch.Tensor:
        return torch.empty(self.lib.sgp_kfu_len(N, M), dtype=torch.float16, device=self.device)

    def suffstats(self, X, y, Z, ls, sf2, kernel="rbf", out: Optional[torch.Tensor] = None,
                  kfu: Optional[torch.Tensor] = None, gate: Optional[torch.cuda.Event] = None) -> torch.Tensor:
        N, d = X.shape
        M = Z.shape[0]
        self._chk(Z, "Z")
        if N > 0:
            self._chk(X, "X"), self._chk(y, "y")
        if out is None:
            out = self.empty(M * M + M + 2)
        nbytes = self.lib.sgp_ctx_suffstats_workspace_bytes(self._c(), N, M, d, 1 if kfu is not None else 0)
        if nbytes == 0:
            raise ValueError("unsupported shape N=%d M=%d d=%d (d <= %d, M <= %d)" % (N, M, d, _lib.SGP_MAX_DIM, _lib.SGP_MAX_INDUCING))
        ws = self._workspace("fwd_kfu" if kfu is not None else "fwd", nbytes)
        base = out.data_ptr()
        if gate is not None:
            self.lib.sgp_ctx_set_pass1_gate(self._c(), C.c_void_p(gate.cuda_event))
        st = self.lib.sgp_ctx_suffstats_fwd(
            self._c(), self._ptr(X), d, self._ptr(y), self._ptr(Z), d, self._inv_ls(ls, d, kernel), float(sf2), N, M, d, _kernel_id(kernel),
            C.c_void_p(base), C.c_void_p(base + 8 * M * M), C.c_void_p(base + 8 * (M * M + M)),
            C.c_void_p(base + 8 * (M * M + M + 1)), self._ptr(kfu), self._ptr(ws), ws.numel(), self._stream())
        _lib.check("sgp_suffstats_fwd", st)
        return out

    def suffstats_whitened(self, X, y, Z, ls, sf2, kuu_linv, kernel="rbf", out: Optional[torch.Tensor] = None) -> torch.Tensor:
        N, d = X.shape
        M = Z.shape[0]
        self._chk(Z, "Z"), self._chk(kuu_linv, "kuu_linv")
        if N > 0:
            self._chk(X, "X"), self._chk(y, "y")
        if out is None:
            out = self.empty(M * M + M + 2)
        nbytes = self.lib.sgp_ctx_suffstats_whitened_workspace_bytes(self._c(), N, M, d)
        if nbytes == 0:
            raise ValueError("unsupported shape N=%d M=%d d=%d" % (N, M, d))
        ws = self._workspace("fwd_whitened", nbytes)
        base = out.data_ptr()
        st = self.lib.sgp_ctx_suffstats_fwd_whitened(
            self._c(), self._ptr(X), d, self._ptr(y), self._ptr(Z), d, self._inv_ls(ls, d, kernel), float(sf2), N, M, d, _kernel_id(kernel),
            self._ptr(kuu_linv), C.c_void_p(base), C.c_void_p(base + 8 * M * M), C.c_void_p(base + 8 * (M * M + M)),
            C.c_void_p(base + 8 * (M * M + M + 1)), self._ptr(ws), ws.numel(), self._stream())
        _lib.check("sgp_suffstats_fwd_whitened", st)
        return out

    def suffstats_whitened_rows(self, X, y, Z, ls, sf2, kuu_linv, kernel="rbf", out: Optional[torch.Tensor] = None,
                                t_out: Optional[torch.Tensor] = None) -> torch.Tensor:
        N, d = X.shape
        M = Z.shape[0]
        self._chk(Z, "Z"), self._chk(kuu_linv, "kuu_linv")
        if N > 0:
            self._chk(X, "X"), self._chk(y, "y")
        if out is None:
            out = self.empty(M * M + M + 2)
        if t_out is not None:
            self._chk(t_out, "t_out")
            if t_out.numel() < self.lib.sgp_kfu_len(N, M):
                raise ValueError("t_out holds %d doubles, sgp_kfu_len(N, M) = %d" % (t_out.numel(), self.lib.sgp_kfu_len(N, M)))
        nbytes = self.lib.sgp_ctx_suffstats_whitened_rows_workspace_bytes(self._c(), N, M, d, 1 if t_out is not None else 0)
        if nbytes == 0:
            raise ValueError("unsupported shape N=%d M=%d d=%d" % (N, M, d))
        ws = self._workspace("fwd_whitened_rows_t" if t_out is not None else "fwd_whitened_rows", nbytes)
        base = out.data_ptr()
        st = self.lib.sgp_ctx_suffstats_fwd_whitened_rows(
            self._c(), self._ptr(X), d, self._ptr(y), self._ptr(Z), d, self._inv_ls(ls, d, kernel), float(sf2), N, M, d, _kernel_id(kernel),
            self._ptr(kuu_linv), C.c_void_p(base), C.c_void_p(base + 8 * M * M), C.c_void_p(base + 8 * (M * M + M)),
            C.c_void_p(base + 8 * (M * M + M + 1)), self._ptr(t_out) if t_out is not None else C.c_void_p(0), self._ptr(ws), ws.numel(),
            self._stream())
        _lib.check("sgp_suffstats_fwd_whitened_rows", st)
        return out

# ... 292 lines not shown
        c = counters.to("cpu")
        res = {"samples": samples.to("cpu"), "stats": h[: n_draws * (cols - 1)].reshape(n_draws, cols - 1),
               "seconds": h[n_draws * (cols - 1):], "evaluations": int(c[0]), "draws": int(c[1]), "info": int(info.to("cpu")[0])}
        if res["info"] < 0:
            self.small_reset()
        return res

    def small_nuts_joint(self, X, y, M, q0, n_tune, n_draws, seed, jitter=1e-6, kernel="rbf", max_treedepth=10, step_scale=0.25,
                         target_accept=0.8):
        N, d = X.shape
        M = int(M)
        for t, n in ((X, "X"), (y, "y")):
            self._chk(t, n)
        if _kernel_id(kernel) == _kernel_id("composite"):
            raise ValueError("the joint sampler takes stationary kernels")
        nd = d + 2 + M * d
        q0d = torch.as_tensor(np.asarray(q0, dtype=np.float64).reshape(-1)).to(self.device)
        if q0d.numel() != nd:
            raise ValueError("q0 has %d entries, expected %d" % (q0d.numel(), nd))
        nbytes = self.lib.sgp_small_nuts_joint_workspace_bytes(N, M, d)
        if nbytes == 0:
            raise ValueError("shape N=%d M=%d d=%d is outside the single-launch path" % (N, M, d))
        small = self._small_ws(N, M, d, nbytes)
        cols = int(self.lib.sgp_small_nuts_stat_cols())
        samples = self.empty(n_draws, nd)
        stats = torch.zeros(n_draws * cols, dtype=torch.float64, device=self.device)
        counters = torch.zeros(4, dtype=torch.int64, device=self.device)
        out = self.empty(d + 5)
        info = torch.zeros(1, dtype=torch.int32, device=self.device)
        _lib.check("sgp_small_nuts_joint", self._cf.sgp_small_nuts_joint(
            self._ptr(X), d, self._ptr(y), self._ptr(q0d), N, M, d, _kernel_id(kernel), float(jitter), int(n_tune), int(n_draws),
            int(max_treedepth), float(step_scale), float(target_accept), int(seed) & ((1 << 64) - 1), self._ptr(samples),
            self._ptr(stats), C.c_void_p(counters.data_ptr()), self._ptr(out), C.c_void_p(info.data_ptr()), self._ptr(small),
            small.numel(), self._stream()))
        h = stats.to("cpu")
        c = counters.to("cpu")
        res = {"samples": samples.to("cpu"), "stats": h[: n_draws * (cols - 1)].reshape(n_draws, cols - 1),
               "seconds": h[n_draws * (cols - 1):], "evaluations": int(c[0]), "draws": int(c[1]), "info": int(info.to("cpu")[0]),
               "sampler_seconds": int(c[2]) * 1e-8, "eval_seconds": int(c[3]) * 1e-8}
        if res["info"] < 0:
            self.small_reset()
        return res

    def small_result(self, d: int):
        buf = self.empty(d + 6)
        return buf, buf[d + 5:d + 6].view(torch.int32)[:1]

    def small_reset(self):
        for key, ws in self._ws.items():
            if isinstance(key, tuple) and key[0] == "small":
                ws[: self.lib.sgp_small_sync_bytes()].zero_()

    def suffstats_bwd(self, X, y, Z, ls, sf2, Phibar, bbar, kappabar, kernel="rbf", want_gz=False,
                      out: Optional[torch.Tensor] = None, kfu: Optional[torch.Tensor] = None) -> torch.Tensor:
        N, d = X.shape
        M = Z.shape[0]
        nh = self.hyper_len(kernel, d)
        if out is None:
            out = self.empty(nh + 1 + (M * d if want_gz else 0))
        nbytes = self.lib.sgp_suffstats_bwd_workspace_bytes_ex(N, M, d, 1 if kfu is not None else 0)
        ws = self._workspace("bwd_kfu" if kfu is not None else "bwd", nbytes)
        base = out.data_ptr()
        st = self.lib.sgp_ctx_suffstats_bwd(
            self._c(), self._ptr(X), d, self._ptr(y), self._ptr(Z), d, self._inv_ls(ls, d, kernel), float(sf2), self._ptr(Phibar),
            self._ptr(bbar), float(kappabar), self._ptr(kfu), N, M, d, _kernel_id(kernel), C.c_void_p(base),
            C.c_void_p(base + 8 * nh),
            C.c_void_p(base + 8 * (nh + 1)) if want_gz else C.c_void_p(0), self._ptr(ws), ws.numel(), self._stream())
        _lib.check("sgp_suffstats_bwd", st)
        return out

    def suffstats_bwd_factored(self, X, y, Z, ls, sf2, kuu_linv, Cw, s2, bbar, kappabar, kernel="rbf", want_gz=False,
                               out: Optional[torch.Tensor] = None, t_in: Optional[torch.Tensor] = None) -> torch.Tensor:
        N, d = X.shape
        M = Z.shape[0]
        nh = self.hyper_len(kernel, d)
        if out is None:
            out = self.empty(nh + 1 + (M * d if want_gz else 0))
        if t_in is not None:
            self._chk(t_in, "t_in")
        nbytes = self.lib.sgp_ctx_suffstats_bwd_factored_workspace_bytes(self._c(), N, M, d, 1 if t_in is not None else 0)
        ws = self._workspace("bwd_factored_t" if t_in is not None else "bwd_factored", nbytes)
        base = out.data_ptr()
        st = self.lib.sgp_ctx_suffstats_bwd_factored(
            self._c(), self._ptr(X), d, self._ptr(y), self._ptr(Z), d, self._inv_ls(ls, d, kernel), float(sf2), self._ptr(kuu_linv),
            self._ptr(Cw), float(s2), self._ptr(bbar), float(kappabar), N, M, d, _kernel_id(kernel),
            self._ptr(t_in) if t_in is not None else C.c_void_p(0), C.c_void_p(base),
            C.c_void_p(base + 8 * nh), C.c_void_p(base + 8 * (nh + 1)) if want_gz else C.c_void_p(0), self._ptr(ws), ws.numel(),
            self._stream())
        _lib.check("sgp_suffstats_bwd_factored_ex", st)
        return out

    def kuu_bwd(self, Z, ls, sf2, Kuubar, grads: torch.Tensor, kernel="rbf", want_gz=False) -> torch.Tensor:
        M, d = Z.shape
        nbytes = self.lib.sgp_kuu_bwd_workspace_bytes(M, d)
        ws = self._workspace("kuu_bwd", nbytes)
        base = grads.data_ptr()
        nh = self.hyper_len(kernel, d)
        st = self.lib.sgp_kuu_bwd(
            self._ptr(Z), d, self._inv_ls(ls, d, kernel), float(sf2), self._ptr(Kuubar), M, d, _kernel_id(kernel),
            C.c_void_p(base), C.c_void_p(base + 8 * nh), C.c_void_p(base + 8 * (nh + 1)) if want_gz else C.c_void_p(0),
            self._ptr(ws), ws.numel(), self._stream())
        _lib.check("sgp_kuu_bwd", st)
        return grads

    def predict(self, Xs, Z, ls, sf2, s2, factors, kernel="rbf", pred_noise=True, full_cov=False):
        T, d = Xs.shape
        M = Z.shape[0]
        self._chk(Xs, "Xs"), self._chk(factors, "factors")
        mean, var = self.empty(T), self.empty(T)
        cov = self.empty(T, T) if full_cov else None
        nbytes = self.lib.sgp_predict_workspace_bytes(T, M, d, 1 if full_cov else 0)
        ws = self._workspace("predict", nbytes)
# ... 206 lines not shown
```

include/sgp.h:

```cpp
#ifndef SGP_H
#define SGP_H

#include <stddef.h>
#include <stdint.h>

#ifdef __cplusplus
extern "C" {
#endif
#if defined(__GNUC__) || defined(__clang__)
#pragma GCC visibility push(default)
#endif

typedef void* sgp_stream_t;

#define SGP_ABI_VERSION 3
#define SGP_MAX_DIM 32
#define SGP_MAX_INDUCING 4096

#define SGP_INFO_TIMEOUT (-7777)

#define SGP_KERNEL_RBF 0
#define SGP_KERNEL_MATERN32 1
#define SGP_KERNEL_MATERN52 2
#define SGP_KERNEL_COMPOSITE 3
#define SGP_COMP_MAX_TERMS 4
#define SGP_COMP_MAX_FACTORS 2
#define SGP_COMP_LEN 33
#define SGP_FAC_EXPQUAD 0
#define SGP_FAC_MATERN32 1
#define SGP_FAC_MATERN52 2
#define SGP_FAC_RATQUAD 3
#define SGP_FAC_PERIODIC 4

#define SGP_OK 0
#define SGP_ERR_ARG (-1)
#define SGP_ERR_DIM (-2)
#define SGP_ERR_WORKSPACE (-3)
#define SGP_ERR_LAUNCH (-4)

#define SGP_OUT_F 0
#define SGP_OUT_LOGMARG 1
#define SGP_OUT_TRACE 2
#define SGP_OUT_LOGDETB 3
#define SGP_OUT_QUAD 4
#define SGP_OUT_TRW 5
#define SGP_OUT_S2BAR 6
#define SGP_OUT_KAPPABAR 7
#define SGP_OUT_LEN 8

int sgp_abi_version(void);

typedef struct sgp_ctx sgp_ctx;
#define SGP_OPT_CONTRACTION 0
#define SGP_OPT_ASM_OVERLAP 1
#define SGP_OPT_KFU_BUDGET_BYTES 2
#define SGP_OPT_COND_LIMIT 3
#define SGP_OPT_CU_BUDGET 4
#define SGP_OPT_TIMING 5
#define SGP_OPT_SHARED_DEVICE 6
sgp_ctx* sgp_ctx_create(int device);
void sgp_ctx_destroy(sgp_ctx* ctx);
int sgp_ctx_device(const sgp_ctx* ctx);
int sgp_ctx_set_option(sgp_ctx* ctx, int option, double value);
double sgp_ctx_get_option(const sgp_ctx* ctx, int option);
void sgp_ctx_bind_thread(sgp_ctx* ctx);
void sgp_ctx_set_pass1_gate(sgp_ctx* ctx, void* hip_event);
int sgp_ctx_contraction_last(const sgp_ctx* ctx);
int sgp_ctx_contraction_would_use_i8(const sgp_ctx* ctx, int64_t N, int M);
int sgp_ctx_timing_last_ms(sgp_ctx* ctx, int slot, float* ms);
int64_t sgp_ctx_timing_last_rows(const sgp_ctx* ctx, int slot);
size_t sgp_ctx_suffstats_workspace_bytes(const sgp_ctx* ctx, int64_t N, int M, int d, int caller_owns_kfu);
int sgp_ctx_suffstats_fwd(sgp_ctx* ctx, const double* X, int64_t ldx, const double* y, const double* Z, int64_t ldz,
                          const double* inv_ls, double sf2, int64_t N, int M, int d, int kernel_id, double* Phi, double* b,
                          double* yy, double* kappa, double* Kfu_out, void* ws, size_t ws_bytes, sgp_stream_t stream);
int sgp_ctx_suffstats_bwd(sgp_ctx* ctx, const double* X, int64_t ldx, const double* y, const double* Z, int64_t ldz,
                          const double* inv_ls, double sf2, const double* Phibar, const double* bbar, double kappabar,
                          const double* Kfu_in, int64_t N, int M, int d, int kernel_id, double* g_ls, double* g_sf2, double* g_Z,
                          void* ws, size_t ws_bytes, sgp_stream_t stream);
int sgp_ctx_kuu_factor(sgp_ctx* ctx, const double* Kuu, int M, double* Linv_out, int* info, void* ws, size_t ws_bytes,
                       sgp_stream_t stream);
int sgp_ctx_kuu_factor_ex(sgp_ctx* ctx, const double* Kuu, int M, double* Linv_out, int* info, double* trace_out, void* ws,
                          size_t ws_bytes, sgp_stream_t stream);
int sgp_ctx_bound_from_stats(sgp_ctx* ctx, const double* Kuu, const double* Phi, const double* b, const double* yy,
                             const double* kappa, double s2, int64_t N, int M, int with_adjoints, double* out, double* Phibar,
                             double* bbar, double* Kuubar, double* factors, const double* kuu_linv, int* info, void* ws,
                             size_t ws_bytes, sgp_stream_t stream);
size_t sgp_ctx_suffstats_whitened_workspace_bytes(const sgp_ctx* ctx, int64_t N, int M, int d);
int sgp_ctx_suffstats_fwd_whitened(sgp_ctx* ctx, const double* X, int64_t ldx, const double* y, const double* Z, int64_t ldz,
                                   const double* inv_ls, double sf2, int64_t N, int M, int d, int kernel_id, const double* kuu_linv,
                                   double* W, double* u, double* yy, double* kappa, void* ws, size_t ws_bytes, sgp_stream_t stream);
size_t sgp_ctx_suffstats_whitened_rows_workspace_bytes(const sgp_ctx* ctx, int64_t N, int M, int d, int caller_owns_t);
int sgp_ctx_suffstats_fwd_whitened_rows(sgp_ctx* ctx, const double* X, int64_t ldx, const double* y, const double* Z, int64_t ldz,
                                        const double* inv_ls, double sf2, int64_t N, int M, int d, int kernel_id,
                                        const double* kuu_linv, double* W, double* u, double* yy, double* kappa, double* T_out,
                                        void* ws, size_t ws_bytes, sgp_stream_t stream);
size_t sgp_ctx_suffstats_extended_workspace_bytes(const sgp_ctx* ctx, int64_t N, int M, int d);
int sgp_ctx_suffstats_fwd_extended(sgp_ctx* ctx, const double* X, int64_t ldx, const double* y, const double* Z, int64_t ldz,
                                   const double* inv_ls, double sf2, int64_t N, int M, int d, int kernel_id, const double* kuu_linv,
                                   int level, double* W, double* u, double* yy, double* kappa, double* Kfu_out, double* phi_diag,
                                   void* ws, size_t ws_bytes, sgp_stream_t stream);
size_t sgp_ctx_suffstats_bwd_factored_workspace_bytes(const sgp_ctx* ctx, int64_t N, int M, int d, int caller_owns_t);
int sgp_ctx_suffstats_bwd_factored(sgp_ctx* ctx, const double* X, int64_t ldx, const double* y, const double* Z, int64_t ldz,
                                   const double* inv_ls, double sf2, const double* kuu_linv, const double* Cw, double s2,
                                   const double* bbar, double kappabar, int64_t N, int M, int d, int kernel_id, const double* T_in,
                                   double* g_ls, double* g_sf2, double* g_Z, void* ws, size_t ws_bytes, sgp_stream_t stream);
int sgp_ctx_bound_from_whitened_stats(sgp_ctx* ctx, const double* W, const double* u, const double* yy, const double* kappa, double s2,
                                      int64_t N, int M, int with_adjoints, double* out, double* Phibar, double* bbar, double* Kuubar,
                                      double* factors, const double* kuu_linv, int* info, double* Cw, void* ws, size_t ws_bytes,
                                      sgp_stream_t stream);
int sgp_ctx_mixture_predict(sgp_ctx* ctx, const double* X, int64_t ldx, const double* y, int64_t N, const double* Xs, int64_t ldxs,
                            int64_t T, const double* Z, int64_t ldz, int S, const double* inv_ls, const double* sf2, const double* s2,
                            double jitter, int M, int d, int kernel_id, int pred_noise, double gate_jitter, double* mean, double* var,
                            double* cov, int* info, int* gate_info, void* ws, size_t ws_bytes, sgp_stream_t stream);
int sgp_ctx_mixture_predict_zs(sgp_ctx* ctx, const double* X, int64_t ldx, const double* y, int64_t N, const double* Xs,
                               int64_t ldxs, int64_t T, const double* Z, int64_t ldz, int64_t z_stride, int S, const double* inv_ls,
                               const double* sf2, const double* s2, double jitter, int M, int d, int kernel_id, int pred_noise,
                               double gate_jitter, double* mean, double* var, double* cov, int* info, int* gate_info, void* ws,
                               size_t ws_bytes, sgp_stream_t stream);

void sgp_set_cu_budget(int n);
const char* sgp_status_string(int status);

void sgp_timing_enable(int on);
int sgp_timing_last_ms(int slot, float* ms);
int64_t sgp_timing_last_rows(int slot);
void sgp_set_asm_overlap(int mode);

size_t sgp_suffstats_workspace_bytes(int64_t N, int M, int d);
size_t sgp_suffstats_workspace_bytes_ex(int64_t N, int M, int d, int caller_owns_kfu);
size_t sgp_kfu_len(int64_t N, int M);
int sgp_set_contraction(int mode);
int sgp_contraction_last(void);
void sgp_set_pass1_gate(void* hip_event);

void sgp_set_kfu_budget_bytes(size_t bytes);
int sgp_suffstats_fwd(const double* X, int64_t ldx, const double* y,
                      const double* Z, int64_t ldz, const double* inv_ls, double sf2,
                      int64_t N, int M, int d, int kernel_id,
                      double* Phi, double* b, double* yy, double* kappa, double* Kfu_out,
                      void* ws, size_t ws_bytes, sgp_stream_t stream);

size_t sgp_stats_packed_len(int M);
int sgp_stats_pack_lower(const double* stats, int M, double* tri, sgp_stream_t stream);
int sgp_stats_unpack_lower(const double* tri, int M, double* stats, sgp_stream_t stream);

int sgp_kuu(const double* Z, int64_t ldz, const double* inv_ls, double sf2, double jitter,
            int M, int d, int kernel_id, double* Kuu, sgp_stream_t stream);

size_t sgp_chol_workspace_bytes(int M);
int sgp_chol_lower(double* A, int64_t lda, int M, int* info, void* ws, size_t ws_bytes, sgp_stream_t stream);
size_t sgp_trsm_workspace_bytes(int M, int k);
int sgp_trsm_lower(const double* L, int64_t ldl, double* B, int64_t ldb, int trans, int M, int k,
                   void* ws, size_t ws_bytes, sgp_stream_t stream);
int sgp_logdiag_sum(const double* L, int64_t ldl, int M, double* out, sgp_stream_t stream);

size_t sgp_bound_workspace_bytes(int M, int with_adjoints);
size_t sgp_bound_factors_len(int M);
void sgp_set_cond_limit(double limit);
size_t sgp_kuu_inverse_trace_len(void);
int sgp_kuu_inverse_trace(const double* kuu_linv, int M, double* trace_out, sgp_stream_t stream);
int sgp_streaming_error_estimate(const double* stats, const double* trace_inv, double s2, int64_t N, int M, double* est,
                                 sgp_stream_t stream);
int sgp_streaming_error_bound(const double* trace_inv, double sf2, double s2, double* est, sgp_stream_t stream);
int sgp_streaming_error_report(const double* diag, int64_t stride, const double* trace_inv, double sf2, double s2, int64_t N, int M,
                               double* est, sgp_stream_t stream);
size_t sgp_kuu_factor_len(int M);
size_t sgp_kuu_factor_workspace_bytes(int M);
int sgp_kuu_factor(const double* Kuu, int M, double* Linv_out, int* info,
                   void* ws, size_t ws_bytes, sgp_stream_t stream);
int sgp_kuu_factor_ex(const double* Kuu, int M, double* Linv_out, int* info, double* trace_out,
                      void* ws, size_t ws_bytes, sgp_stream_t stream);
int sgp_bound_from_stats(const double* Kuu, const double* Phi, const double* b,
                         const double* yy, const double* kappa, double s2, int64_t N, int M,
                         int with_adjoints, double* out,
                         double* Phibar, double* bbar, double* Kuubar, double* factors,
                         const double* kuu_linv ,
                         int* info, void* ws, size_t ws_bytes, sgp_stream_t stream);

size_t sgp_suffstats_whitened_workspace_bytes(int64_t N, int M, int d);
int sgp_suffstats_fwd_whitened(const double* X, int64_t ldx, const double* y,
                               const double* Z, int64_t ldz, const double* inv_ls, double sf2,
                               int64_t N, int M, int d, int kernel_id, const double* kuu_linv,
                               double* W, double* u, double* yy, double* kappa,
// ... 42 lines not shown
                                  const double* kuu_linv, int* info, void* ws, size_t ws_bytes, sgp_stream_t stream);

int sgp_bound_from_whitened_stats_ex(const double* W, const double* u, const double* yy, const double* kappa,
                                     double s2, int64_t N, int M, int with_adjoints, double* out,
                                     double* Phibar, double* bbar, double* Kuubar, double* factors,
                                     const double* kuu_linv, int* info, double* Cw,
                                     void* ws, size_t ws_bytes, sgp_stream_t stream);

#define SGP_SMALL_NATURAL 0
#define SGP_SMALL_HMC 1
int sgp_small_supported(int64_t N, int M, int d, int kernel_id);
void sgp_small_debug_stamps(void* dev_buffer);
size_t sgp_small_workspace_bytes(int64_t N, int M, int d);
size_t sgp_small_sync_bytes(void);
int sgp_small_eval(const double* X, int64_t ldx, const double* y, const double* Z, int64_t ldz,
                   const double* theta, int64_t N, int M, int d, int kernel_id, double jitter, int mode,
                   int want_grad, double* out, double* g_Z, int* info,
                   void* ws, size_t ws_bytes, sgp_stream_t stream);

int sgp_small_eval_composite(const double* X, int64_t ldx, const double* y, const double* Z, int64_t ldz,
                             const double* theta, const double* structure, int n_free, const int* free_slot,
                             const int* free_role, const double* free_prior_sd, int64_t N, int M, int d,
                             double jitter, int mode, int want_grad, double* out, int* info,
                             void* ws, size_t ws_bytes, sgp_stream_t stream);

int sgp_small_eval_batch(const double* X, int64_t ldx, const double* y, const double* Z, int64_t ldz,
                         const double* thetas, int S, int64_t N, int M, int d, int kernel_id, double jitter, int mode,
                         int want_grad, double* theta_scratch, double* outs, double* g_Z, int* infos,
                         void* ws, size_t ws_bytes, sgp_stream_t stream);

size_t sgp_small_nuts_stat_cols(void);
int sgp_small_nuts(const double* X, int64_t ldx, const double* y, const double* Z, int64_t ldz, const double* q0,
                   int64_t N, int M, int d, int kernel_id, double jitter, int n_tune, int n_draws, int max_treedepth,
                   double step_scale, double target_accept, uint64_t seed, double* theta_scratch, double* samples,
                   double* stats, long long* counters, double* out, int* info,
                   void* ws, size_t ws_bytes, sgp_stream_t stream);

size_t sgp_small_nuts_joint_workspace_bytes(int64_t N, int M, int d);
int sgp_small_nuts_joint(const double* X, int64_t ldx, const double* y, const double* q0, int64_t N, int M, int d,
                         int kernel_id, double jitter, int n_tune, int n_draws, int max_treedepth, double step_scale,
                         double target_accept, uint64_t seed, double* samples, double* stats, long long* counters,
                         double* out, int* info, void* ws, size_t ws_bytes, sgp_stream_t stream);

int sgp_small_nuts_composite(const double* X, int64_t ldx, const double* y, const double* Z, int64_t ldz,
                             const double* q0, const double* structure, int n_free, const int* free_slot,
                             const int* free_role, const double* free_prior_sd, int64_t N, int M, int d,
                             double jitter, int n_tune, int n_draws, int max_treedepth, double step_scale,
                             double target_accept, uint64_t seed, double* theta_scratch, double* samples,
                             double* stats, long long* counters, double* out, int* info,
                             void* ws, size_t ws_bytes, sgp_stream_t stream);

size_t sgp_suffstats_bwd_workspace_bytes(int64_t N, int M, int d);
size_t sgp_suffstats_bwd_workspace_bytes_ex(int64_t N, int M, int d, int caller_owns_kfu);
int sgp_suffstats_bwd(const double* X, int64_t ldx, const double* y,
                      const double* Z, int64_t ldz, const double* inv_ls, double sf2,
                      const double* Phibar, const double* bbar, double kappabar,
                      const double* Kfu_in ,
                      int64_t N, int M, int d, int kernel_id,
                      double* g_ls, double* g_sf2, double* g_Z,
                      void* ws, size_t ws_bytes, sgp_stream_t stream);
size_t sgp_suffstats_bwd_factored_workspace_bytes(int64_t N, int M, int d);
int sgp_suffstats_bwd_factored(const double* X, int64_t ldx, const double* y,
                               const double* Z, int64_t ldz, const double* inv_ls, double sf2,
                               const double* kuu_linv, const double* Cw, double s2,
                               const double* bbar, double kappabar,
                               int64_t N, int M, int d, int kernel_id,
                               double* g_ls, double* g_sf2, double* g_Z,
                               void* ws, size_t ws_bytes, sgp_stream_t stream);

size_t sgp_suffstats_bwd_factored_workspace_bytes_ex(int64_t N, int M, int d, int caller_owns_t);
int sgp_suffstats_bwd_factored_ex(const double* X, int64_t ldx, const double* y,
                                  const double* Z, int64_t ldz, const double* inv_ls, double sf2,
                                  const double* kuu_linv, const double* Cw, double s2,
                                  const double* bbar, double kappabar,
                                  int64_t N, int M, int d, int kernel_id, const double* T_in,
                                  double* g_ls, double* g_sf2, double* g_Z,
                                  void* ws, size_t ws_bytes, sgp_stream_t stream);

size_t sgp_kuu_bwd_workspace_bytes(int M, int d);
int sgp_kuu_bwd(const double* Z, int64_t ldz, const double* inv_ls, double sf2,
                const double* Kuubar, int M, int d, int kernel_id,
                double* g_ls, double* g_sf2, double* g_Z,
                void* ws, size_t ws_bytes, sgp_stream_t stream);

size_t sgp_predict_workspace_bytes(int64_t T, int M, int d, int want_cov);
int sgp_predict(const double* Xs, int64_t ldxs, int64_t T,
                const double* Z, int64_t ldz, const double* inv_ls, double sf2, double s2,
                const double* factors, int M, int d, int kernel_id, int pred_noise,
                double* mean, double* var, double* cov,
                void* ws, size_t ws_bytes, sgp_stream_t stream);

#define SGP_LIK_GAUSSIAN 0
#define SGP_LIK_BERNOULLI_PROBIT 1
size_t sgp_svgp_workspace_bytes(int64_t B, int M, int d);
int sgp_svgp_elbo(const double* Xb, int64_t ldx, const double* yb, int64_t B,
                  const double* Z, int64_t ldz, const double* inv_ls, double sf2, double s2, double jitter,
                  const double* m, const double* LS, int64_t N_total, int M, int d, int kernel_id, int likelihood_id,
                  int with_grads, double* out,
                  double* g_m, double* g_LS, double* g_Z, double* g_ls, double* g_sf2, double* g_s2,
                  int* info, void* ws, size_t ws_bytes, sgp_stream_t stream);
size_t sgp_svgp_batch_workspace_bytes(int64_t B, int M, int d, int S);
int sgp_svgp_elbo_batch(const double* Xb, int64_t ldx, const double* yb, int64_t B, const double* Z, int64_t ldz,
                        int S, const double* inv_ls, const double* sf2, const double* s2, double jitter,
                        const double* m, const double* LS, int64_t N_total, int M, int d, int kernel_id, int likelihood_id,
                        int with_grads, double* out,
                        double* g_m, double* g_LS, double* g_Z, double* g_ls, double* g_sf2, double* g_s2,
// ... 40 lines not shown
```

Measured before the change: 70.28.

## Reuse int8 digit-split Kfu from pass 1 in backward kbar contraction

The forward pass now writes the int8 digit-decomposed Kfu (7 digit planes) as a side output. The backward pass reuses those digits with a digit-quantized Phibar in a new int8 kbar kernel, replacing the f64 Kfu buffer and its dense contraction. This cuts pass-2 memory traffic and moves the contraction onto integer matrix throughput. In exchange it adds a separate code path gated by shape, kernel type and budget, relies on the digit-split arithmetic reproducing f64 accuracy, and needs a large uint8 buffer.

Result: no change. 70.15, median of 6 (-0.2%).

```diff
diff --git a/generalised-gaussian-processes_amd/_lib.py b/generalised-gaussian-processes_amd/_lib.py
--- a/generalised-gaussian-processes_amd/_lib.py
+++ b/generalised-gaussian-processes_amd/_lib.py
@@ -11,7 +11,7 @@
 SGP_MAX_INDUCING = 4096
 KERNEL_IDS = {"rbf": 0, "matern32": 1, "matern52": 2, "composite": 3}
 COMP_LEN = 33
-OPT_CONTRACTION, OPT_ASM_OVERLAP, OPT_KFU_BUDGET_BYTES, OPT_COND_LIMIT, OPT_CU_BUDGET, OPT_TIMING, OPT_SHARED_DEVICE = range(7)
+OPT_CONTRACTION, OPT_ASM_OVERLAP, OPT_KFU_BUDGET_BYTES, OPT_COND_LIMIT, OPT_CU_BUDGET, OPT_TIMING, OPT_SHARED_DEVICE, OPT_PASS2 = range(8)
 OUT_F, OUT_LOGMARG, OUT_TRACE, OUT_LOGDETB, OUT_QUAD, OUT_TRW, OUT_S2BAR, OUT_KAPPABAR, OUT_LEN = range(9)
 
 
@@ -41,6 +41,8 @@
     "sgp_ctx_set_pass1_gate": (None, [_vp, _vp]),
     "sgp_ctx_contraction_last": (_i32, [_vp]),
     "sgp_ctx_contraction_would_use_i8": (_i32, [_vp, _i64, _i32]),
+    "sgp_ctx_pass2_would_use_i8": (_i32, [_vp, _i64, _i32, _i32, _i32]),
+    "sgp_ctx_pass2_last": (_i32, [_vp]),
     "sgp_ctx_timing_last_ms": (_i32, [_vp, _i32, C.POINTER(C.c_float)]),
     "sgp_ctx_timing_last_rows": (_i64, [_vp, _i32]),
     "sgp_ctx_suffstats_workspace_bytes": (_sz, [_vp, _i64, _i32, _i32, _i32]),
@@ -48,6 +50,10 @@
                                      _vp, _vp, _vp, _vp, _vp, _vp, _sz, _vp]),
     "sgp_ctx_suffstats_bwd": (_i32, [_vp, _vp, _i64, _vp, _vp, _i64, _dp, _dbl, _vp, _vp, _dbl, _vp, _i64, _i32, _i32, _i32,
                                      _vp, _vp, _vp, _vp, _sz, _vp]),
+    "sgp_ctx_suffstats_fwd_qt": (_i32, [_vp, _vp, _i64, _vp, _vp, _i64, _dp, _dbl, _i64, _i32, _i32, _i32,
+                                        _vp, _vp, _vp, _vp, _vp, _vp, _sz, _vp]),
+    "sgp_ctx_suffstats_bwd_qt": (_i32, [_vp, _vp, _i64, _vp, _vp, _i64, _dp, _dbl, _vp, _vp, _dbl, _vp, _i64, _i32, _i32, _i32,
+                                        _vp, _vp, _vp, _vp, _sz, _vp]),
     "sgp_ctx_kuu_factor": (_i32, [_vp, _vp, _i32, _vp, _vp, _vp, _sz, _vp]),
     "sgp_ctx_kuu_factor_ex": (_i32, [_vp, _vp, _i32, _vp, _vp, _vp, _vp, _sz, _vp]),
     "sgp_ctx_bound_from_stats": (_i32, [_vp, _vp, _vp, _vp, _vp, _vp, _dbl, _i64, _i32, _i32, _vp,
@@ -80,6 +86,12 @@
     "sgp_suffstats_workspace_bytes_ex": (_sz, [_i64, _i32, _i32, _i32]),
     "sgp_suffstats_bwd_workspace_bytes_ex": (_sz, [_i64, _i32, _i32, _i32]),
     "sgp_kfu_len": (_sz, [_i64, _i32]),
+    "sgp_kfu_digits_len": (_sz, [_i64, _i32]),
+    "sgp_suffstats_fwd_qt": (_i32, [_vp, _i64, _vp, _vp, _i64, _dp, _dbl, _i64, _i32, _i32, _i32,
+                                    _vp, _vp, _vp, _vp, _vp, _vp, _sz, _vp]),
+    "sgp_suffstats_bwd_qt_workspace_bytes": (_sz, [_i64, _i32, _i32]),
+    "sgp_suffstats_bwd_qt": (_i32, [_vp, _i64, _vp, _vp, _i64, _dp, _dbl, _vp, _vp, _dbl, _vp, _i64, _i32, _i32, _i32,
+                                    _vp, _vp, _vp, _vp, _sz, _vp]),
     "sgp_set_kfu_budget_bytes": (None, [_sz]),
     "sgp_set_contraction": (_i32, [_i32]),
     "sgp_contraction_last": (_i32, []),
diff --git a/generalised-gaussian-processes_amd/core.py b/generalised-gaussian-processes_amd/core.py
--- a/generalised-gaussian-processes_amd/core.py
+++ b/generalised-gaussian-processes_amd/core.py
@@ -129,6 +129,7 @@
         self.n_collectives = 0
         self._kfu = None
         self._kfu_f16 = None
+        self._kfu_q = None
         self.kfu_budget_bytes = 64 << 30
         self.whitened_rows_min_work = 1 << 26
         self.factored_adjoint = True
@@ -200,6 +201,21 @@
         if self._kfu is None or self._kfu.numel() < need:
             self._kfu = e.kfu_buffer(n_local, M)
         return self._kfu
+
+    def _kfu_q_for(self, M):
+        e = self.engine
+        if not hasattr(e, "kfu_digits_buffer") or not hasattr(e, "pass2_would_use_i8") or self.kernel == "composite":
+            return None
+        n_local, d = int(self.X.shape[0]), int(self.X.shape[1])
+        if not e.pass2_would_use_i8(n_local, M, d, self.kernel):
+            return None
+        need = ((max(n_local, 1) + 255) // 256 * 256) * ((M + 127) // 128 * 128) * 7
+        if need > self.kfu_budget_bytes:
+            return None
+        if self._kfu_q is None or self._kfu_q.numel() < need:
+            self._kfu_q = None
+            self._kfu_q = e.kfu_digits_buffer(n_local, M)
+        return self._kfu_q
 
     def _kfu_f16_for(self, M):
         e = self.engine
@@ -374,7 +390,8 @@
                 res["reported"] = True
             res.update(packed=packed, kfu=None, t_keep=t_keep, linv=linv)
             return res
-        kfu = self._kfu_for(M) if with_adjoints else None
+        kfu_q = self._kfu_q_for(M) if with_adjoints else None
+        kfu = self._kfu_for(M) if with_adjoints and kfu_q is None else None
         gate = None
         guard = report
         trace = self._trace_buf() if guard and hasattr(e, "kuu_factor") else None
@@ -392,7 +409,8 @@
                     and e.would_use_i8(int(self.X.shape[0]), M)):
                 gate = ready
         try:
-            packed = e.suffstats(self.X, self.y, Z, ls, sf2, self.kernel, kfu=kfu, **({"gate": gate} if gate is not None else {}))
+            packed = e.suffstats(self.X, self.y, Z, ls, sf2, self.kernel, kfu=kfu, **({"gate": gate} if gate is not None else {}),
+                                 **({"kfu_q": kfu_q} if kfu_q is not None else {}))
             self._allreduce_stats(packed, M)
         finally:
             if overlap:
@@ -413,6 +431,7 @@
             res["reported"] = True
         res["packed"] = packed
         res["kfu"] = kfu
+        res["kfu_q"] = kfu_q
         return res
 
     def _pass2(self, res, Z, ls, sf2, s2, want_gz, g):
@@ -423,7 +442,8 @@
                                      **({"t_in": res["t_keep"]} if res.get("t_keep") is not None else {}))
         else:
             e.suffstats_bwd(self.X, self.y, Z, ls, sf2, res["Phibar"], res["bbar"], -1.0 / (2.0 * float(s2)),
-                            self.kernel, want_gz=want_gz, out=g, kfu=res["kfu"])
+                            self.kernel, want_gz=want_gz, out=g, kfu=res["kfu"],
+                            **({"kfu_q": res["kfu_q"]} if res.get("kfu_q") is not None else {}))
             if res.get("Phibar_lo") is not None:
                 n_lo = int(res.get("lo_slots", 0))
                 e.suffstats_bwd_lo(self.X, self.y, Z, ls, sf2, res["Phibar_lo"], res["kfu"], g, self.kernel,
diff --git a/generalised-gaussian-processes_amd/csrc/sgp_ctx.hip b/generalised-gaussian-processes_amd/csrc/sgp_ctx.hip
--- a/generalised-gaussian-processes_amd/csrc/sgp_ctx.hip
+++ b/generalised-gaussian-processes_amd/csrc/sgp_ctx.hip
@@ -22,6 +22,8 @@
   c.syrk_glds = env_int("SGP_SYRK_GLDS", 0);
   c.i8_prio = env_int("SGP_I8_PRIO", 0);
   c.shared_device = env_int("SGP_SHARED_DEVICE", 0) != 0 ? 1 : 0;
+  c.pass2 = env_int("SGP_PASS2", 1);
+  if (c.pass2 < 0 || c.pass2 > 2) c.pass2 = 1;
 }
 
 Ctx& default_ctx() {
@@ -103,6 +105,10 @@
     case SGP_OPT_SHARED_DEVICE:
       c.shared_device = value != 0.0 ? 1 : 0;
       return SGP_OK;
+    case SGP_OPT_PASS2:
+      if (!(value >= 0.0 && value <= 2.0)) return SGP_ERR_ARG;
+      c.pass2 = (int)value;
+      return SGP_OK;
     default:
       return SGP_ERR_ARG;
   }
@@ -118,6 +124,7 @@
     case SGP_OPT_CU_BUDGET: return (double)c.cu_budget;
     case SGP_OPT_TIMING: return (double)c.timing;
     case SGP_OPT_SHARED_DEVICE: return (double)c.shared_device;
+    case SGP_OPT_PASS2: return (double)c.pass2;
     default: return -1.0;
   }
 }
@@ -132,6 +139,10 @@
 
 extern "C" int sgp_ctx_contraction_last(const sgp_ctx* ctx) {
   return (ctx ? *reinterpret_cast<const Ctx*>(ctx) : default_ctx()).contraction_used;
+}
+
+extern "C" int sgp_ctx_pass2_last(const sgp_ctx* ctx) {
+  return (ctx ? *reinterpret_cast<const Ctx*>(ctx) : default_ctx()).pass2_used;
 }
 
 extern "C" size_t sgp_ctx_suffstats_workspace_bytes(const sgp_ctx* ctx, int64_t N, int M, int d, int caller_owns_kfu) {
@@ -153,6 +164,22 @@
   CtxScope scope(ctx);
   return sgp_suffstats_bwd(X, ldx, y, Z, ldz, inv_ls, sf2, Phibar, bbar, kappabar, Kfu_in, N, M, d, kernel_id, g_ls, g_sf2, g_Z, ws,
                            ws_bytes, stream);
+}
+extern "C" int sgp_ctx_suffstats_fwd_qt(sgp_ctx* ctx, const double* X, int64_t ldx, const double* y, const double* Z, int64_t ldz,
+                                        const double* inv_ls, double sf2, int64_t N, int M, int d, int kernel_id, double* Phi, double* b,
+                                        double* yy, double* kappa, void* Qt_out, void* ws, size_t ws_bytes, sgp_stream_t stream) {
+  if (!ctx_on_current_device(ctx)) return SGP_ERR_ARG;
+  CtxScope scope(ctx);
+  return sgp_suffstats_fwd_qt(X, ldx, y, Z, ldz, inv_ls, sf2, N, M, d, kernel_id, Phi, b, yy, kappa, Qt_out, ws, ws_bytes, stream);
+}
+extern "C" int sgp_ctx_suffstats_bwd_qt(sgp_ctx* ctx, const double* X, int64_t ldx, const double* y, const double* Z, int64_t ldz,
+                                        const double* inv_ls, double sf2, const double* Phibar, const double* bbar, double kappabar,
+                                        const void* Qt_in, int64_t N, int M, int d, int kernel_id, double* g_ls, double* g_sf2,
+                                        double* g_Z, void* ws, size_t ws_bytes, sgp_stream_t stream) {
+  if (!ctx_on_current_device(ctx)) return SGP_ERR_ARG;
+  CtxScope scope(ctx);
+  return sgp_suffstats_bwd_qt(X, ldx, y, Z, ldz, inv_ls, sf2, Phibar, bbar, kappabar, Qt_in, N, M, d, kernel_id, g_ls, g_sf2, g_Z, ws,
+                              ws_bytes, stream);
 }
 extern "C" int sgp_ctx_kuu_factor(sgp_ctx* ctx, const double* Kuu, int M, double* Linv_out, int* info, void* ws, size_t ws_bytes,
                                   sgp_stream_t stream) {
diff --git a/generalised-gaussian-processes_amd/csrc/sgp_ctx.hpp b/generalised-gaussian-processes_amd/csrc/sgp_ctx.hpp
--- a/generalised-gaussian-processes_amd/csrc/sgp_ctx.hpp
+++ b/generalised-gaussian-processes_amd/csrc/sgp_ctx.hpp
@@ -16,8 +16,10 @@
   int cu_budget = 0;
   int timing = 0;
   int shared_device = 0;
+  int pass2 = 1;
   int syrk_skip_upper = 1, syrk_waves = 4, syrk_glds = 0, i8_prio = 0;
   int contraction_used = 0;
+  int pass2_used = 0;
   hipEvent_t pass1_gate = nullptr;
   int64_t syrk_timed_rows = 0;
   hipEvent_t ev[CTX_TIMING_SLOTS][2] = {};
diff --git a/generalised-gaussian-processes_amd/csrc/sgp_kbar_epi.hpp b/generalised-gaussian-processes_amd/csrc/sgp_kbar_epi.hpp
--- /dev/null
+++ b/generalised-gaussian-processes_amd/csrc/sgp_kbar_epi.hpp
@@ -0,0 +1,29 @@
+#pragma once
+#include "sgp_common.hpp"
+
+namespace sgp {
+
+template <int DP, int KID, bool GZ>
+__device__ __forceinline__ void kbar_epi_elem(double c, double bbm, double yn, double msk, double sf2, const double (&zrow)[DP],
+                                              const double* __restrict__ xq, double (&gl)[DP], double (&gz)[DP], double& gs) {
+  double df[DP];
+  double r2 = 0.0;
+#pragma unroll
+  for (int j = 0; j < DP; ++j) {
+    df[j] = zrow[j] - xq[j];
+    r2 = fma(df[j], df[j], r2);
+  }
+  double kp, hp;
+  kprofile_grad<KID>(r2, kp, hp);
+  const double kbar = (2.0 * sf2 * c + bbm * yn) * msk;
+  gs = fma(kbar, kp, gs);
+  const double E = kbar * sf2 * hp;
+#pragma unroll
+  for (int j = 0; j < DP; ++j) {
+    const double t = E * df[j];
+    if constexpr (GZ) gz[j] += t;
+    gl[j] = fma(t, df[j], gl[j]);
+  }
+}
+
+}
diff --git a/generalised-gaussian-processes_amd/csrc/sgp_stream.hpp b/generalised-gaussian-processes_amd/csrc/sgp_stream.hpp
--- a/generalised-gaussian-processes_amd/csrc/sgp_stream.hpp
+++ b/generalised-gaussian-processes_amd/csrc/sgp_stream.hpp
@@ -184,8 +184,16 @@
 }
 void i8_assemble(const StreamPlan& p, int kid, const double* Xs, const double* ys, const double* Zs, int64_t row0, int64_t rows,
                  int64_t N, int M, uint8_t* Q, double* Kfu , double* bpart, hipStream_t st,
-                 uint16_t* Kh = nullptr );
+                 uint16_t* Kh = nullptr ,
+                 uint8_t* Qt = nullptr );
 int i8_contract(const uint8_t* Q, int Mp, int64_t rows, int nsplit, int accumulate, double* slab, hipStream_t st, double* slab_lo = nullptr,
                 int level = 1);
+int i8_kbar_nsplit(int64_t Npad, int Mp);
+struct Ctx;
+bool i8_pass2_rule(const Ctx& c, int64_t N, int M, int d, int kernel_id);
+void i8_pq_digits(const double* Pb, int Mp, uint8_t* Pq, double* psc, hipStream_t st);
+int i8_kbar(const uint8_t* Qt, const uint8_t* Pq, const double* psc, const double* Xs, const double* ys, const double* Zs, const double* bb,
+            double sf2, int64_t Npad, int nsplit, int64_t N, int M, int Mp, int DP, int kid, int want_gz, double* gzpart, double* glpart,
+            hipStream_t st);
 
 }
diff --git a/generalised-gaussian-processes_amd/csrc/sgp_suffstats_bwd.hip b/generalised-gaussian-processes_amd/csrc/sgp_suffstats_bwd.hip
--- a/generalised-gaussian-processes_amd/csrc/sgp_suffstats_bwd.hip
+++ b/generalised-gaussian-processes_amd/csrc/sgp_suffstats_bwd.hip
@@ -2,6 +2,8 @@
 #include "sgp_stream.hpp"
 #include "sgp_composite.hpp"
 #include "sgp_dense.hpp"
+#include "sgp_kbar_epi.hpp"
+#include "sgp_ctx.hpp"
 #include <cstdlib>
 
 namespace sgp {
@@ -258,25 +260,7 @@
         const int nl = half * 32 + i;
         const int64_t n = row0 + r0 + h * 64 + nl;
         const double* __restrict__ xq = Xs + n * DP;
-        double df[DP];
-        double r2 = 0.0;
-#pragma unroll
-        for (int j = 0; j < DP; ++j) {
-          df[j] = zrow[j] - xq[j];
-          r2 = fma(df[j], df[j], r2);
-        }
-        double kp, hp;
-        kprofile_grad<KID>(r2, kp, hp);
-        const double msk = n < N ? mmask : 0.0;
-        const double kbar = (2.0 * sf2 * Ct[nl][erow] + bbm * ys[n]) * msk;
-        gs = fma(kbar, kp, gs);
-        const double E = kbar * sf2 * hp;
-#pragma unroll
-        for (int j = 0; j < DP; ++j) {
-          const double t = E * df[j];
-          if constexpr (GZ) gz[j] += t;
-          gl[j] = fma(t, df[j], gl[j]);
-        }
+        kbar_epi_elem<DP, KID, GZ>(Ct[nl][erow], bbm, ys[n], n < N ? mmask : 0.0, sf2, zrow, xq, gl, gz, gs);
       }
       __syncthreads();
     }
@@ -479,6 +463,70 @@
   const int rg = (int)((tot + 255) / 256 < 1024 ? (tot + 255) / 256 : 1024);
   bwd_reduce_kernel<<<rg < 1 ? 1 : rg, 256, 0, st>>>(w.gzpart, w.glpart, p.nsplit_b, p.nmb, p.Mp, M, p.DP, ka,
                                                     kappabar * (double)N, g_ls, g_sf2, g_Z);
+  cur_ctx().pass2_used = 0;
+  return check_launch();
+}
+
+struct BwdI8Ws {
+  double *Xs, *ys, *Zs, *Pb, *bb, *gzpart, *glpart, *yypart, *psc;
+  uint8_t* Pq;
+  int nsplit;
+  size_t bytes;
+};
+static BwdI8Ws carve_bwd_i8(void* ws, const StreamPlan& p) {
+  Carver c(ws);
+  BwdI8Ws w;
+  w.nsplit = i8_kbar_nsplit(p.Npad, p.Mp);
+  w.Xs = c.take<double>((size_t)(p.Npad > 0 ? p.Npad : 1) * p.DP);
+  w.ys = c.take<double>((size_t)(p.Npad > 0 ? p.Npad : 1));
+  w.Zs = c.take<double>((size_t)p.Mp * p.DP);
+  w.Pb = c.take<double>((size_t)p.Mp * p.Mp);
+  w.bb = c.take<double>((size_t)p.Mp);
+  w.gzpart = c.take<double>((size_t)w.nsplit * p.Mp * p.DP);
+  w.glpart = c.take<double>((size_t)w.nsplit * (p.Mp / 64) * (p.DP + 1));
+  w.yypart = c.take<double>(256);
+  w.psc = c.take<double>((size_t)p.Mp);
+  w.Pq = c.take<uint8_t>((size_t)p.Mp * p.Mp * 7);
+  w.bytes = c.used();
+  return w;
+}
+extern "C" size_t sgp_suffstats_bwd_qt_workspace_bytes(int64_t N, int M, int d) {
+  if (N < 0 || M <= 0 || d <= 0 || d > SGP_MAX_DIM || M > SGP_MAX_INDUCING || dp_for(d) > 8) return 0;
+  return carve_bwd_i8(nullptr, make_stream_plan(N, M, d)).bytes;
+}
+extern "C" int sgp_suffstats_bwd_qt(const double* X, int64_t ldx, const double* y, const double* Z, int64_t ldz,
+                                    const double* inv_ls, double sf2, const double* Phibar, const double* bbar,
+                                    double kappabar, const void* Qt_in, int64_t N, int M, int d, int kernel_id,
+                                    double* g_ls, double* g_sf2, double* g_Z, void* ws, size_t ws_bytes,
+                                    sgp_stream_t stream) {
+  if (!Z || !inv_ls || !Phibar || !bbar || !g_ls || !g_sf2 || N < 0 || M <= 0 || d <= 0 || ldz < d) return SGP_ERR_ARG;
+  if (N > 0 && (!X || !y || !Qt_in || ldx < d)) return SGP_ERR_ARG;
+  if (kernel_id != SGP_KERNEL_RBF && kernel_id != SGP_KERNEL_MATERN32 && kernel_id != SGP_KERNEL_MATERN52) return SGP_ERR_ARG;
+  if (d > SGP_MAX_DIM || M > SGP_MAX_INDUCING || dp_for(d) > 8) return SGP_ERR_DIM;
+  StreamPlan p = make_stream_plan(N, M, d);
+  BwdI8Ws w = carve_bwd_i8(ws, p);
+  if (!ws || ws_bytes < w.bytes) return SGP_ERR_WORKSPACE;
+  hipStream_t st = (hipStream_t)stream;
+  KernArgs ka;
+  for (int j = 0; j < SGP_MAX_DIM; ++j) ka.inv_ls[j] = j < d ? inv_ls[j] : 0.0;
+  ka.sf2 = sf2;
+  ka.d = d;
+  {
+    PadSymJob pad;
+    pad.P = Phibar; pad.out = w.Pb; pad.vec = bbar; pad.vout = w.bb;
+    stream_prologue(p, ka, X, ldx, y, Z, ldz, N, M, w.Xs, w.ys, w.Zs, w.yypart, st, pad);
+  }
+  i8_pq_digits(w.Pb, p.Mp, w.Pq, w.psc, st);
+  timing_begin(TIMING_KBAR, st);
+  if (i8_kbar(static_cast<const uint8_t*>(Qt_in), w.Pq, w.psc, w.Xs, w.ys, w.Zs, w.bb, sf2, p.Npad, w.nsplit, N, M, p.Mp, p.DP, kernel_id,
+              g_Z != nullptr, w.gzpart, w.glpart, st) != SGP_OK)
+    return SGP_ERR_LAUNCH;
+  timing_end(TIMING_KBAR, st);
+  const int64_t tot = (int64_t)M * d;
+  const int rg = (int)((tot + 255) / 256 < 1024 ? (tot + 255) / 256 : 1024);
+  bwd_reduce_kernel<<<rg < 1 ? 1 : rg, 256, 0, st>>>(w.gzpart, w.glpart, w.nsplit, p.Mp / 64, p.Mp, M, p.DP, ka, kappabar * (double)N,
+                                                    g_ls, g_sf2, g_Z);
+  cur_ctx().pass2_used = 1;
   return check_launch();
 }
 
diff --git a/generalised-gaussian-processes_amd/csrc/sgp_suffstats_fwd.hip b/generalised-gaussian-processes_amd/csrc/sgp_suffstats_fwd.hip
--- a/generalised-gaussian-processes_amd/csrc/sgp_suffstats_fwd.hip
+++ b/generalised-gaussian-processes_amd/csrc/sgp_suffstats_fwd.hip
@@ -830,10 +830,9 @@
   return fwd_workspace_bytes(N, M, d, caller_owns_kfu == 0);
 }
 
-extern "C" int sgp_suffstats_fwd(const double* X, int64_t ldx, const double* y, const double* Z, int64_t ldz,
-                                 const double* inv_ls, double sf2, int64_t N, int M, int d, int kernel_id,
-                                 double* Phi, double* b, double* yy, double* kappa, double* Kfu_out, void* ws,
-                                 size_t ws_bytes, sgp_stream_t stream) {
+static int suffstats_fwd(const double* X, int64_t ldx, const double* y, const double* Z, int64_t ldz, const double* inv_ls, double sf2,
+                         int64_t N, int M, int d, int kernel_id, double* Phi, double* b, double* yy, double* kappa, double* Kfu_out,
+                         uint8_t* Qt_out, void* ws, size_t ws_bytes, sgp_stream_t stream) {
   Ctx& cx = cur_ctx();
   hipEvent_t gate = cx.pass1_gate;
   cx.pass1_gate = nullptr;
@@ -841,6 +840,8 @@
   if (N > 0 && (!X || !y || ldx < d)) return SGP_ERR_ARG;
   if (kernel_id < 0 || kernel_id > SGP_KERNEL_COMPOSITE) return SGP_ERR_ARG;
   if (d > SGP_MAX_DIM || M > SGP_MAX_INDUCING) return SGP_ERR_DIM;
+  if (Qt_out && (Kfu_out || kernel_id == SGP_KERNEL_COMPOSITE)) return SGP_ERR_ARG;
+  if (Qt_out && dp_for(d) > 8) return SGP_ERR_DIM;
   if (kernel_id == SGP_KERNEL_COMPOSITE) {
     CompSpec cs;
     if (comp_parse(inv_ls, d, &cs) != SGP_OK) return SGP_ERR_ARG;
@@ -870,7 +871,7 @@
   int nslabs = p.nsplit;
   int head_ns = 0;
   int64_t head_chunks = 0;
-  const bool use_i8 = i8_rule(cx.contraction, p.Npad, p.Mp);
+  const bool use_i8 = Qt_out ? p.Npad > 0 : i8_rule(cx.contraction, p.Npad, p.Mp);
   cx.contraction_used = use_i8 ? 1 : 0;
   if (!use_i8) gate = nullptr;
   if (p.Npad > 0 && !use_i8) head_block(p, p.Npad / NB, &head_ns, &head_chunks);
@@ -879,7 +880,8 @@
     for (int64_t r0 = 0; r0 < p.Npad; r0 += qrows) {
       const int64_t rows = (p.Npad - r0) < qrows ? (p.Npad - r0) : qrows;
       timing_begin(TIMING_ASSEMBLE, st);
-      i8_assemble(p, kernel_id, w.Xs, w.ys, w.Zs, r0, rows, N, M, w.Q, Kfu_out ? Kfu_out + (size_t)r0 * p.Mp : nullptr, w.bpart, st);
+      i8_assemble(p, kernel_id, w.Xs, w.ys, w.Zs, r0, rows, N, M, w.Q, Kfu_out ? Kfu_out + (size_t)r0 * p.Mp : nullptr, w.bpart, st, nullptr,
+                  Qt_out ? Qt_out + (size_t)r0 * p.Mp * 7 : nullptr);
       timing_end(TIMING_ASSEMBLE, st);
       if (gate && hipStreamWaitEvent(st, gate, 0) != hipSuccess) return SGP_ERR_LAUNCH;
       gate = nullptr;
@@ -936,6 +938,32 @@
   finalize_stats_kernel<<<(M + 255) / 256, 256, 0, st>>>(w.btmp, BRED_G, p.Mp, M, w.yypart, 256, sf2,
                                                          sf2 * (double)N, b, yy, kappa);
   return check_launch();
+}
+
+extern "C" int sgp_suffstats_fwd(const double* X, int64_t ldx, const double* y, const double* Z, int64_t ldz,
+                                 const double* inv_ls, double sf2, int64_t N, int M, int d, int kernel_id,
+                                 double* Phi, double* b, double* yy, double* kappa, double* Kfu_out, void* ws,
+                                 size_t ws_bytes, sgp_stream_t stream) {
+  return suffstats_fwd(X, ldx, y, Z, ldz, inv_ls, sf2, N, M, d, kernel_id, Phi, b, yy, kappa, Kfu_out, nullptr, ws, ws_bytes, stream);
+}
+extern "C" size_t sgp_kfu_digits_len(int64_t N, int M) { return sgp_kfu_len(N, M) * 7; }
+extern "C" int sgp_suffstats_fwd_qt(const double* X, int64_t ldx, const double* y, const double* Z, int64_t ldz, const double* inv_ls,
+                                    double sf2, int64_t N, int M, int d, int kernel_id, double* Phi, double* b, double* yy, double* kappa,
+                                    void* Qt_out, void* ws, size_t ws_bytes, sgp_stream_t stream) {
+  if (!Qt_out) return SGP_ERR_ARG;
+  return suffstats_fwd(X, ldx, y, Z, ldz, inv_ls, sf2, N, M, d, kernel_id, Phi, b, yy, kappa, nullptr, static_cast<uint8_t*>(Qt_out), ws,
+                       ws_bytes, stream);
+}
+namespace sgp {
+bool i8_pass2_rule(const Ctx& c, int64_t N, int M, int d, int kernel_id) {
+  if (N <= 0 || M <= 0 || M > SGP_MAX_INDUCING || d <= 0 || d > SGP_MAX_DIM || dp_for(d) > 8) return false;
+  if (kernel_id != SGP_KERNEL_RBF && kernel_id != SGP_KERNEL_MATERN32 && kernel_id != SGP_KERNEL_MATERN52) return false;
+  if (c.pass2 == 2) return true;
+  return c.pass2 == 1 && i8_rule(c.contraction, round_up64(N, ASM_ROWS), padded_m(M));
+}
+}
+extern "C" int sgp_ctx_pass2_would_use_i8(const sgp_ctx* ctx, int64_t N, int M, int d, int kernel_id) {
+  return i8_pass2_rule(ctx ? *reinterpret_cast<const Ctx*>(ctx) : default_ctx(), N, M, d, kernel_id) ? 1 : 0;
 }
 
 extern "C" size_t sgp_suffstats_whitened_rows_workspace_bytes(int64_t N, int M, int d, int caller_owns_t) {
diff --git a/generalised-gaussian-processes_amd/csrc/sgp_suffstats_i8.hip b/generalised-gaussian-processes_amd/csrc/sgp_suffstats_i8.hip
--- a/generalised-gaussian-processes_amd/csrc/sgp_suffstats_i8.hip
+++ b/generalised-gaussian-processes_amd/csrc/sgp_suffstats_i8.hip
@@ -2,6 +2,7 @@
 #include "sgp_common.hpp"
 #include "sgp_stream.hpp"
 #include "sgp_ctx.hpp"
+#include "sgp_kbar_epi.hpp"
 #include <cstdlib>
 #include <type_traits>
 
@@ -19,14 +20,31 @@
 constexpr int I8_PPW = (I8_PIECES + 7) / 8;
 constexpr int I8_LDS_BYTES = I8_NSTAGE * I8_STAGE_BYTES;
 
-template <int DP, int KID, bool WK>
+__device__ __forceinline__ void byte_planes(const unsigned (&lo)[16], const unsigned (&hi)[16], i4v (&plane)[8]) {
+#pragma unroll
+  for (int j = 0; j < 4; ++j) {
+#pragma unroll
+    for (int h = 0; h < 2; ++h) {
+      const unsigned* s4 = (h ? hi : lo) + 4 * j;
+      const unsigned u0 = __builtin_amdgcn_perm(s4[1], s4[0], 0x05010400u), u1 = __builtin_amdgcn_perm(s4[1], s4[0], 0x07030602u);
+      const unsigned v0 = __builtin_amdgcn_perm(s4[3], s4[2], 0x05010400u), v1 = __builtin_amdgcn_perm(s4[3], s4[2], 0x07030602u);
+      plane[4 * h + 0][j] = (int)__builtin_amdgcn_perm(v0, u0, 0x05040100u);
+      plane[4 * h + 1][j] = (int)__builtin_amdgcn_perm(v0, u0, 0x07060302u);
+      plane[4 * h + 2][j] = (int)__builtin_amdgcn_perm(v1, u1, 0x05040100u);
+      if (h == 0) plane[3][j] = (int)__builtin_amdgcn_perm(v1, u1, 0x07060302u);
+    }
+  }
+}
+constexpr int QT_LD = 256 + 2;
+template <int DP, int KID, bool WK, bool QT = false>
 __global__ __launch_bounds__(256) void kfu_digits_kernel(const double* __restrict__ Xs, const double* __restrict__ ys,
                                                          const double* __restrict__ Zs, int64_t row0, int64_t N, int M, int Mp,
                                                          uint8_t* __restrict__ Q, double* __restrict__ Kfu, uint16_t* __restrict__ Kh,
-                                                         double* __restrict__ bpart) {
+                                                         double* __restrict__ bpart, uint8_t* __restrict__ Qt) {
   __shared__ double xs[ASM_ROWS][DP];
   __shared__ double ysh[ASM_ROWS];
   __shared__ double etab[EXP_TAB_N];
+  __shared__ __attribute__((aligned(16))) unsigned long long qsh[QT ? 16 : 1][QT ? QT_LD : 1];
   const int64_t rbase = (int64_t)blockIdx.x * ASM_ROWS;
   {
     const double* src = Xs + (row0 + rbase) * DP;
@@ -36,8 +54,10 @@
     sgp_exp_tab_load(etab);
   }
   __syncthreads();
-  const int m = blockIdx.y * 256 + threadIdx.x;
-  if (m >= Mp) return;
+  const int m_raw = blockIdx.y * 256 + threadIdx.x;
+  if (!QT && m_raw >= Mp) return;
+  const bool mact = m_raw < Mp;
+  const int m = mact ? m_raw : Mp - 1;
   const double zmask = m < M ? 1.0 : 0.0;
   double zr[DP];
 #pragma unroll
@@ -87,26 +107,37 @@
     }
     const size_t rb = (size_t)(rbase / 16 + g);
     i4v plane[8];
-#pragma unroll
-    for (int j = 0; j < 4; ++j) {
-#pragma unroll
-      for (int h = 0; h < 2; ++h) {
-        const unsigned* s4 = (h ? hi : lo) + 4 * j;
-        const unsigned u0 = __builtin_amdgcn_perm(s4[1], s4[0], 0x05010400u), u1 = __builtin_amdgcn_perm(s4[1], s4[0], 0x07030602u);
-        const unsigned v0 = __builtin_amdgcn_perm(s4[3], s4[2], 0x05010400u), v1 = __builtin_amdgcn_perm(s4[3], s4[2], 0x07030602u);
-        plane[4 * h + 0][j] = (int)__builtin_amdgcn_perm(v0, u0, 0x05040100u);
-        plane[4 * h + 1][j] = (int)__builtin_amdgcn_perm(v0, u0, 0x07060302u);
-        plane[4 * h + 2][j] = (int)__builtin_amdgcn_perm(v1, u1, 0x05040100u);
-        if (h == 0) plane[3][j] = (int)__builtin_amdgcn_perm(v1, u1, 0x07060302u);
-      }
-    }
-#pragma unroll
-    for (int p = 0; p < I8_NP; ++p)
-      __builtin_nontemporal_store(plane[p], reinterpret_cast<i4v*>(Q + ((rb * I8_NP + p) * Mp + m) * 16));
+    byte_planes(lo, hi, plane);
+    if (mact) {
+#pragma unroll
+      for (int p = 0; p < I8_NP; ++p)
+        __builtin_nontemporal_store(plane[p], reinterpret_cast<i4v*>(Q + ((rb * I8_NP + p) * Mp + m) * 16));
+    }
+    if constexpr (QT) {
+#pragma unroll
+      for (int e = 0; e < 16; ++e) qsh[e][threadIdx.x] = ((unsigned long long)hi[e] << 32) | lo[e];
+      __syncthreads();
+      const int e = threadIdx.x & 15, jb = threadIdx.x >> 4;
+      const unsigned long long* src = &qsh[e][jb * 16];
+#pragma unroll
+      for (int k = 0; k < 16; k += 2) {
+        const i4v v = *reinterpret_cast<const i4v*>(src + k);
+        lo[k] = (unsigned)v[0]; hi[k] = (unsigned)v[1]; lo[k + 1] = (unsigned)v[2]; hi[k + 1] = (unsigned)v[3];
+      }
+      __syncthreads();
+      byte_planes(lo, hi, plane);
+      const int jbg = blockIdx.y * 16 + jb;
+      const int64_t rr = rbase + g * 16 + e;
+      if (jbg * 16 < Mp) {
+        uint8_t* dst = Qt + ((size_t)((rr >> 7) * (Mp / 16) + jbg) * I8_NP * 128 + (rr & 127)) * 16;
+#pragma unroll
+        for (int p = 0; p < I8_NP; ++p) __builtin_nontemporal_store(plane[p], reinterpret_cast<i4v*>(dst + (size_t)p * 128 * 16));
+      }
+    }
   }
   };
   if (interior) run(std::false_type{}); else run(std::true_type{});
-  bpart[((row0 + rbase) / ASM_ROWS) * Mp + m] = bacc;
+  if (mact) bpart[((row0 + rbase) / ASM_ROWS) * Mp + m] = bacc;
 }
 
 constexpr int I8_PSPLIT = 5;
@@ -117,9 +148,13 @@
 #endif
 static_assert(2 * I8_PPW - 1 <= I8_PSPLIT * (I8_PSPLIT + 1) / 2, "every DMA piece must find its MFMA in the first half");
 
-template <bool ACT, int I8_MINSUM, bool DD>
+struct I8NoEpi {
+  __device__ void operator()(const i16v*) const {}
+};
+template <bool ACT, int I8_MINSUM, bool DD, bool P2 = false, class Epi = I8NoEpi>
 __device__ __forceinline__ void i8_tile_loop(uint8_t* lds, const uint8_t* __restrict__ Q, int Mp, int64_t c0, int64_t c1, int I0,
-                                             int J0, int accumulate, double* __restrict__ out, size_t lo_off, int wave, int lane, int prio) {
+                                             int J0, int accumulate, double* __restrict__ out, size_t lo_off, int wave, int lane, int prio,
+                                             const uint8_t* __restrict__ QB = nullptr, int ldb = 0, Epi* epi = nullptr) {
   constexpr int I8_NG = 13 - I8_MINSUM;
   const int grp = wave >> 2, w4 = wave & 3;
   const int wi = (w4 >> 1) * 2 + grp, wj = w4 & 1;
@@ -132,19 +167,26 @@
 
   unsigned goff[I8_PPW];
   int soff[I8_PPW];
+  bool bsel[I8_PPW];
 #pragma unroll
   for (int k = 0; k < I8_PPW; ++k) {
     int e = wave + 8 * k;
     if (e >= I8_PIECES) e -= I8_PIECES;
     const int rbl = e / (I8_NP * 3), rem = e % (I8_NP * 3), p = rem / 3, cg = rem % 3;
     const int col = cg < 2 ? I0 + cg * 64 : J0;
-    goff[k] = (unsigned)(((rbl * I8_NP + p) * Mp + col + lane) * 16);
+    bsel[k] = P2 && cg == 2;
+    goff[k] = (unsigned)(((rbl * I8_NP + p) * (bsel[k] ? ldb : Mp) + col + lane) * 16);
     soff[k] = __builtin_amdgcn_readfirstlane(((rbl * I8_NP + p) * I8_SCOLS + cg * 64) * 16);
   }
   const size_t gstride = (size_t)2 * I8_NP * Mp * 16;
+  const size_t gstride_b = (size_t)2 * I8_NP * ldb * 16;
   auto dma_piece = [&](const uint8_t* gbase, int sbase, int k) {
     __builtin_amdgcn_global_load_lds((const __attribute__((address_space(1))) void*)(gbase + goff[k]),
                                      (__attribute__((address_space(3))) void*)(lds + sbase + soff[k]), 16, 0, 0);
+  };
+  auto piece_base = [&](int64_t s, int k) -> const uint8_t* {
+    if constexpr (P2) return bsel[k] ? QB + (size_t)s * gstride_b : Q + (size_t)s * gstride;
+    else return Q + (size_t)s * gstride;
   };
   const int64_t nst = c1 - c0;
   auto wait_stage = [&](int64_t sE) {
@@ -173,6 +215,7 @@
     if (prio) { if (dma_on) __builtin_amdgcn_s_setprio(1); else __builtin_amdgcn_s_setprio(0); }
     const bool pre = dma_on && sE + 2 < nst;
     const uint8_t* gnext = Q + (size_t)(c0 + sE + 2) * gstride;
+    const uint8_t* gnext_b = P2 ? QB + (size_t)(c0 + sE + 2) * gstride_b : nullptr;
     const int snext = (int)((sE + 2) % I8_NSTAGE) * I8_STAGE_BYTES;
     int issued = 0, kpiece = 0;
 #pragma unroll
@@ -183,7 +226,7 @@
         ++issued;
         if (dma_on && (issued & 1) && kpiece < I8_PPW) {
           __builtin_amdgcn_sched_barrier(0);
-          if (pre) dma_piece(gnext, snext, kpiece);
+          if (pre) dma_piece(bsel[kpiece] ? gnext_b : gnext, snext, kpiece);
           __builtin_amdgcn_sched_barrier(0);
           ++kpiece;
         }
@@ -191,10 +234,10 @@
   };
   if (nst > 0) {
 #pragma unroll
-    for (int k = 0; k < I8_PPW; ++k) dma_piece(Q + (size_t)c0 * gstride, 0, k);
+    for (int k = 0; k < I8_PPW; ++k) dma_piece(piece_base(c0, k), 0, k);
     if (nst > 1) {
 #pragma unroll
-      for (int k = 0; k < I8_PPW; ++k) dma_piece(Q + (size_t)(c0 + 1) * gstride, I8_STAGE_BYTES, k);
+      for (int k = 0; k < I8_PPW; ++k) dma_piece(piece_base(c0 + 1, k), I8_STAGE_BYTES, k);
     }
     if (grp == 0) {
       for (int64_t sidx = 0; sidx < nst; ++sidx) {
@@ -220,6 +263,10 @@
         half(I8_PSPLIT, I8_NP, false, sidx + 1);
       }
     }
+  }
+  if constexpr (P2) {
+    if (ACT) (*epi)(acc);
+    return;
   }
   if (ACT) {
 #pragma unroll
@@ -278,32 +325,143 @@
     i8_tile_loop<false, MINSUM, DD>(i8_lds, Q, Mp, c0, c1, I0, J0, accumulate, out, lo_off, wave, lane, prio);
 }
 
-template <int DP, bool WK>
+__global__ __launch_bounds__(256) void pq_digits_kernel(const double* __restrict__ Pb, int Mp, uint8_t* __restrict__ Pq,
+                                                        double* __restrict__ psc) {
+  __shared__ double red[4];
+  __shared__ int bad_any;
+  const int m = blockIdx.x, tid = threadIdx.x;
+  const double* row = Pb + (size_t)m * Mp;
+  if (tid == 0) bad_any = 0;
+  double mx = 0.0;
+  bool bad = false;
+  for (int j = tid; j < Mp; j += 256) {
+    const double a = fabs(row[j]);
+    bad |= !(a <= 1.7976931348623157e308);
+    mx = fmax(mx, a);
+  }
+  __syncthreads();
+  if (bad) bad_any = 1;
+#pragma unroll
+  for (int o = 32; o > 0; o >>= 1) mx = fmax(mx, __shfl_xor(mx, o));
+  if ((tid & 63) == 0) red[tid >> 6] = mx;
+  __syncthreads();
+  mx = fmax(fmax(red[0], red[1]), fmax(red[2], red[3]));
+  const bool nonfinite = bad_any != 0;
+  int ex = 0;
+  (void)frexp(mx, &ex);
+  const bool tiny = !(mx > 0.0) || ex < -900;
+  if (tid == 0) psc[m] = nonfinite ? __builtin_nan("") : (tiny ? 0.0 : ldexp(1.0, ex - 60));
+  const double sc = tiny ? 0.0 : ldexp(1.0, 54 - ex);
+  constexpr unsigned long long C = 0x0080808080808080ULL;
+  for (int j = tid; j < Mp; j += 256) {
+    const long long q = nonfinite ? 0 : (long long)rint(row[j] * sc);
+    const unsigned long long qq = ((unsigned long long)q + C) ^ C;
+#pragma unroll
+    for (int p = 0; p < I8_NP; ++p) Pq[((size_t)((j >> 4) * I8_NP + p) * Mp + m) * 16 + (j & 15)] = (uint8_t)(qq >> (8 * p));
+  }
+}
+
+template <int DP, int KID, bool GZ>
+__global__ __launch_bounds__(512, 1) void i8_kbar_kernel(const uint8_t* __restrict__ Qt, const uint8_t* __restrict__ Pq,
+                                                         const double* __restrict__ psc, const double* __restrict__ Xs,
+                                                         const double* __restrict__ ys, const double* __restrict__ Zs,
+                                                         const double* __restrict__ bb, double sf2, int64_t nblocks, int nsplit, int64_t N,
+                                                         int M, int Mp, int nmb, double* __restrict__ gzpart, double* __restrict__ glpart) {
+  extern __shared__ __attribute__((aligned(16))) uint8_t i8_lds[];
+  const int id = blockIdx.x;
+  const int xcd = id & 7, jj = id >> 3;
+  const int mb = jj % nmb, split = (jj / nmb) * 8 + xcd;
+  if (split >= nsplit) return;
+  int64_t nb0, nb1;
+  i8_split_steps(nblocks, nsplit, split, nb0, nb1);
+  const int lane = threadIdx.x & 63;
+  const int wave = __builtin_amdgcn_readfirstlane(threadIdx.x >> 6);
+  const int grp = wave >> 2, w4 = wave & 3;
+  const int wi = (w4 >> 1) * 2 + grp, wj = w4 & 1, l32 = lane & 31, lh = lane >> 5;
+  const int J0 = mb * I8_TC;
+  const int m = J0 + wj * 32 + l32;
+  double zrow[DP], gl[DP], gz[DP], gs = 0.0;
+#pragma unroll
+  for (int j = 0; j < DP; ++j) {
+    zrow[j] = Zs[(size_t)m * DP + j];
+    gl[j] = 0.0;
+    gz[j] = 0.0;
+  }
+  const double bbm = bb[m], mmask = m < M ? 1.0 : 0.0, fsc = psc[m];
+  const size_t ablk = (size_t)(Mp / 16) * I8_NP * 128 * 16;
+  int64_t nb = nb0;
+  auto epi = [&](const i16v* acc) {
+#pragma unroll 2
+    for (int r = 0; r < 16; ++r) {
+      const int64_t n = nb * 128 + wi * 32 + (r >> 2) * 8 + lh * 4 + (r & 3);
+      double v = 0.0;
+#pragma unroll
+      for (int g = 0; g < I8_NP; ++g) v = fma((double)acc[g][r], __builtin_ldexp(1.0, 8 * g), v);
+      kbar_epi_elem<DP, KID, GZ>(v * fsc, bbm, ys[n], n < N ? mmask : 0.0, sf2, zrow, Xs + n * DP, gl, gz, gs);
+    }
+  };
+  for (; nb < nb1; ++nb)
+    i8_tile_loop<true, 6, false, true>(i8_lds, Qt + (size_t)nb * ablk, 128, 0, Mp / 32, 0, J0, 0, nullptr, 0, wave, lane, 0, Pq, Mp, &epi);
+
+  __syncthreads();
+  double* red = reinterpret_cast<double*>(i8_lds);
+  if constexpr (GZ) {
+#pragma unroll
+    for (int j = 0; j < DP; ++j) red[j * 512 + threadIdx.x] = gz[j];
+    __syncthreads();
+    const int c = threadIdx.x & 63, j = threadIdx.x >> 6;
+    if (j < DP) {
+      const int cwj = c >> 5, cl = c & 31;
+      double t = 0.0;
+#pragma unroll
+      for (int w = cwj; w < 8; w += 2) t += red[j * 512 + w * 64 + cl] + red[j * 512 + w * 64 + 32 + cl];
+      gzpart[((size_t)split * Mp + J0 + c) * DP + j] = t;
+    }
+    __syncthreads();
+  }
+#pragma unroll
+  for (int q = 0; q <= DP; ++q) {
+    const double v = wave_sum(q < DP ? gl[q] : gs);
+    if (lane == 0) red[q * 8 + wave] = v;
+  }
+  __syncthreads();
+  if (threadIdx.x <= DP) {
+    double t = 0.0;
+#pragma unroll
+    for (int w = 0; w < 8; ++w) t += red[threadIdx.x * 8 + w];
+    glpart[((size_t)split * nmb + mb) * (DP + 1) + threadIdx.x] = t;
+  }
+}
+
+template <int DP, bool WK, bool QT>
 static void launch_digits(int kid, dim3 grid, hipStream_t st, const double* Xs, const double* ys, const double* Zs, int64_t row0,
-                          int64_t N, int M, int Mp, uint8_t* Q, double* Kfu, uint16_t* Kh, double* bpart) {
+                          int64_t N, int M, int Mp, uint8_t* Q, double* Kfu, uint16_t* Kh, double* bpart, uint8_t* Qt) {
   switch (kid) {
-    case SGP_KERNEL_RBF: kfu_digits_kernel<DP, SGP_KERNEL_RBF, WK><<<grid, 256, 0, st>>>(Xs, ys, Zs, row0, N, M, Mp, Q, Kfu, Kh, bpart); break;
-    case SGP_KERNEL_MATERN32: kfu_digits_kernel<DP, SGP_KERNEL_MATERN32, WK><<<grid, 256, 0, st>>>(Xs, ys, Zs, row0, N, M, Mp, Q, Kfu, Kh, bpart); break;
-    default: kfu_digits_kernel<DP, SGP_KERNEL_MATERN52, WK><<<grid, 256, 0, st>>>(Xs, ys, Zs, row0, N, M, Mp, Q, Kfu, Kh, bpart); break;
-  }
-}
-template <bool WK>
+    case SGP_KERNEL_RBF: kfu_digits_kernel<DP, SGP_KERNEL_RBF, WK, QT><<<grid, 256, 0, st>>>(Xs, ys, Zs, row0, N, M, Mp, Q, Kfu, Kh, bpart, Qt); break;
+    case SGP_KERNEL_MATERN32: kfu_digits_kernel<DP, SGP_KERNEL_MATERN32, WK, QT><<<grid, 256, 0, st>>>(Xs, ys, Zs, row0, N, M, Mp, Q, Kfu, Kh, bpart, Qt); break;
+    default: kfu_digits_kernel<DP, SGP_KERNEL_MATERN52, WK, QT><<<grid, 256, 0, st>>>(Xs, ys, Zs, row0, N, M, Mp, Q, Kfu, Kh, bpart, Qt); break;
+  }
+}
+template <bool WK, bool QT = false>
 static void launch_digits_dp(int DP, int kid, dim3 grid, hipStream_t st, const double* Xs, const double* ys, const double* Zs,
-                             int64_t row0, int64_t N, int M, int Mp, uint8_t* Q, double* Kfu, uint16_t* Kh, double* bpart) {
+                             int64_t row0, int64_t N, int M, int Mp, uint8_t* Q, double* Kfu, uint16_t* Kh, double* bpart,
+                             uint8_t* Qt = nullptr) {
   switch (DP) {
-    case 2: launch_digits<2, WK>(kid, grid, st, Xs, ys, Zs, row0, N, M, Mp, Q, Kfu, Kh, bpart); break;
-    case 4: launch_digits<4, WK>(kid, grid, st, Xs, ys, Zs, row0, N, M, Mp, Q, Kfu, Kh, bpart); break;
-    case 8: launch_digits<8, WK>(kid, grid, st, Xs, ys, Zs, row0, N, M, Mp, Q, Kfu, Kh, bpart); break;
-    case 16: launch_digits<16, WK>(kid, grid, st, Xs, ys, Zs, row0, N, M, Mp, Q, Kfu, Kh, bpart); break;
-    case 24: launch_digits<24, WK>(kid, grid, st, Xs, ys, Zs, row0, N, M, Mp, Q, Kfu, Kh, bpart); break;
-    default: launch_digits<32, WK>(kid, grid, st, Xs, ys, Zs, row0, N, M, Mp, Q, Kfu, Kh, bpart); break;
+    case 2: launch_digits<2, WK, QT>(kid, grid, st, Xs, ys, Zs, row0, N, M, Mp, Q, Kfu, Kh, bpart, Qt); break;
+    case 4: launch_digits<4, WK, QT>(kid, grid, st, Xs, ys, Zs, row0, N, M, Mp, Q, Kfu, Kh, bpart, Qt); break;
+    case 8: launch_digits<8, WK, QT>(kid, grid, st, Xs, ys, Zs, row0, N, M, Mp, Q, Kfu, Kh, bpart, Qt); break;
+    case 16: if constexpr (!QT) launch_digits<16, WK, QT>(kid, grid, st, Xs, ys, Zs, row0, N, M, Mp, Q, Kfu, Kh, bpart, Qt); break;
+    case 24: if constexpr (!QT) launch_digits<24, WK, QT>(kid, grid, st, Xs, ys, Zs, row0, N, M, Mp, Q, Kfu, Kh, bpart, Qt); break;
+    default: if constexpr (!QT) launch_digits<32, WK, QT>(kid, grid, st, Xs, ys, Zs, row0, N, M, Mp, Q, Kfu, Kh, bpart, Qt); break;
   }
 }
 
 void i8_assemble(const StreamPlan& p, int kid, const double* Xs, const double* ys, const double* Zs, int64_t row0, int64_t rows,
-                 int64_t N, int M, uint8_t* Q, double* Kfu, double* bpart, hipStream_t st, uint16_t* Kh) {
+                 int64_t N, int M, uint8_t* Q, double* Kfu, double* bpart, hipStream_t st, uint16_t* Kh, uint8_t* Qt) {
   dim3 grid((unsigned)(rows / ASM_ROWS), (p.Mp + 255) / 256);
-  if (Kfu)
+  if (Qt)
+    launch_digits_dp<false, true>(p.DP, kid, grid, st, Xs, ys, Zs, row0, N, M, p.Mp, Q, nullptr, nullptr, bpart, Qt);
+  else if (Kfu)
     launch_digits_dp<true>(p.DP, kid, grid, st, Xs, ys, Zs, row0, N, M, p.Mp, Q, Kfu, Kh, bpart);
   else
     launch_digits_dp<false>(p.DP, kid, grid, st, Xs, ys, Zs, row0, N, M, p.Mp, Q, nullptr, nullptr, bpart);
@@ -338,4 +496,67 @@
   return SGP_OK;
 }
 
-}
+int i8_kbar_nsplit(int64_t Npad, int Mp) {
+  const int nmb = Mp / I8_TC;
+  int64_t ns = (256 / nmb) / 8 * 8;
+  if (ns < 8) ns = 8;
+  const int64_t nblocks = Npad / 128;
+  const int64_t cap = (nblocks + 7) / 8 * 8;
+  if (ns > cap) ns = cap < 8 ? 8 : cap;
+  return (int)ns;
+}
+
+void i8_pq_digits(const double* Pb, int Mp, uint8_t* Pq, double* psc, hipStream_t st) {
+  pq_digits_kernel<<<Mp, 256, 0, st>>>(Pb, Mp, Pq, psc);
+}
+
+template <int DP, int KID>
+static void launch_i8_kbar(int want_gz, int grid, hipStream_t st, const uint8_t* Qt, const uint8_t* Pq, const double* psc,
+                           const double* Xs, const double* ys, const double* Zs, const double* bb, double sf2, int64_t nblocks, int nsplit,
+                           int64_t N, int M, int Mp, double* gzpart, double* glpart) {
+  if (want_gz)
+    i8_kbar_kernel<DP, KID, true><<<grid, 512, I8_LDS_BYTES, st>>>(Qt, Pq, psc, Xs, ys, Zs, bb, sf2, nblocks, nsplit, N, M, Mp, Mp / I8_TC,
+                                                                  gzpart, glpart);
+  else
+    i8_kbar_kernel<DP, KID, false><<<grid, 512, I8_LDS_BYTES, st>>>(Qt, Pq, psc, Xs, ys, Zs, bb, sf2, nblocks, nsplit, N, M, Mp, Mp / I8_TC,
+                                                                   gzpart, glpart);
+}
+template <int DP>
+static int set_kbar_attrs() {
+  const void* fns[] = {(const void*)i8_kbar_kernel<DP, SGP_KERNEL_RBF, true>,       (const void*)i8_kbar_kernel<DP, SGP_KERNEL_RBF, false>,
+                       (const void*)i8_kbar_kernel<DP, SGP_KERNEL_MATERN32, true>,  (const void*)i8_kbar_kernel<DP, SGP_KERNEL_MATERN32, false>,
+                       (const void*)i8_kbar_kernel<DP, SGP_KERNEL_MATERN52, true>,  (const void*)i8_kbar_kernel<DP, SGP_KERNEL_MATERN52, false>};
+  for (const void* f : fns)
+    if (hipFuncSetAttribute(f, hipFuncAttributeMaxDynamicSharedMemorySize, I8_LDS_BYTES) != hipSuccess) return SGP_ERR_LAUNCH;
+  return SGP_OK;
+}
+
+int i8_kbar(const uint8_t* Qt, const uint8_t* Pq, const double* psc, const double* Xs, const double* ys, const double* Zs, const double* bb,
+            double sf2, int64_t Npad, int nsplit, int64_t N, int M, int Mp, int DP, int kid, int want_gz, double* gzpart, double* glpart,
+            hipStream_t st) {
+  static std::atomic<bool> attr_done[64];
+  int dev = 0;
+  if (hipGetDevice(&dev) != hipSuccess || dev < 0) return SGP_ERR_LAUNCH;
+  if (dev >= 64 || !attr_done[dev].load(std::memory_order_acquire)) {
+    if (set_kbar_attrs<2>() != SGP_OK || set_kbar_attrs<4>() != SGP_OK || set_kbar_attrs<8>() != SGP_OK) return SGP_ERR_LAUNCH;
+    if (dev < 64) attr_done[dev].store(true, std::memory_order_release);
+  }
+  const int grid = (Mp / I8_TC) * nsplit;
+  const int64_t nblocks = Npad / 128;
+#define SGP_I8_KBAR(D) \
+  switch (kid) { \
+    case SGP_KERNEL_RBF: launch_i8_kbar<D, SGP_KERNEL_RBF>(want_gz, grid, st, Qt, Pq, psc, Xs, ys, Zs, bb, sf2, nblocks, nsplit, N, M, Mp, gzpart, glpart); break; \
+    case SGP_KERNEL_MATERN32: launch_i8_kbar<D, SGP_KERNEL_MATERN32>(want_gz, grid, st, Qt, Pq, psc, Xs, ys, Zs, bb, sf2, nblocks, nsplit, N, M, Mp, gzpart, glpart); break; \
+    default: launch_i8_kbar<D, SGP_KERNEL_MATERN52>(want_gz, grid, st, Qt, Pq, psc, Xs, ys, Zs, bb, sf2, nblocks, nsplit, N, M, Mp, gzpart, glpart); break; \
+  }
+  switch (DP) {
+    case 2: SGP_I8_KBAR(2); break;
+    case 4: SGP_I8_KBAR(4); break;
+    case 8: SGP_I8_KBAR(8); break;
+    default: return SGP_ERR_DIM;
+  }
+#undef SGP_I8_KBAR
+  return SGP_OK;
+}
+
+}
diff --git a/generalised-gaussian-processes_amd/engine.py b/generalised-gaussian-processes_amd/engine.py
--- a/generalised-gaussian-processes_amd/engine.py
+++ b/generalised-gaussian-processes_amd/engine.py
@@ -27,7 +27,7 @@
 
     OPTIONS = {"contraction": _lib.OPT_CONTRACTION, "asm_overlap": _lib.OPT_ASM_OVERLAP, "kfu_budget_bytes": _lib.OPT_KFU_BUDGET_BYTES,
                "cond_limit": _lib.OPT_COND_LIMIT, "cu_budget": _lib.OPT_CU_BUDGET, "timing": _lib.OPT_TIMING,
-               "shared_device": _lib.OPT_SHARED_DEVICE}
+               "shared_device": _lib.OPT_SHARED_DEVICE, "pass2": _lib.OPT_PASS2}
 
     def __init__(self, device: Optional[torch.device] = None, own_context: bool = False):
         self.lib = _lib.load_library()
@@ -93,6 +93,13 @@
 
     def would_use_i8(self, N: int, M: int) -> bool:
         return bool(self.lib.sgp_ctx_contraction_would_use_i8(self._c(), int(N), int(M)))
+
+    def pass2_would_use_i8(self, N: int, M: int, d: int, kernel: str = "rbf") -> bool:
+        kid = _lib.KERNEL_IDS.get(kernel, -1)
+        return bool(self.lib.sgp_ctx_pass2_would_use_i8(self._c(), int(N), int(M), int(d), kid))
+
+    def pass2_last(self) -> int:
+        return int(self.lib.sgp_ctx_pass2_last(self._c()))
 
     def _workspace(self, name: str, nbytes: int) -> torch.Tensor:
         buf = self._ws.get(name)
@@ -142,11 +149,20 @@
     def kfu_buffer(self, N: int, M: int) -> torch.Tensor:
         return self.empty(self.lib.sgp_kfu_len(N, M))
 
+    def kfu_digits_buffer(self, N: int, M: int) -> torch.Tensor:
+        return torch.empty(self.lib.sgp_kfu_digits_len(N, M), dtype=torch.uint8, device=self.device)
+
+    def _chk_q(self, kfu_q, N, M):
+        if kfu_q.dtype != torch.uint8 or not kfu_q.is_contiguous() or kfu_q.device != self.device \
+                or kfu_q.numel() < self.lib.sgp_kfu_digits_len(N, M):
+            raise ValueError("kfu_q: a contiguous uint8 tensor of sgp_kfu_digits_len(N, M) bytes on this device (kfu_digits_buffer)")
+
     def kfu_f16_buffer(self, N: int, M: int) -> torch.Tensor:
         return torch.empty(self.lib.sgp_kfu_len(N, M), dtype=torch.float16, device=self.device)
 
     def suffstats(self, X, y, Z, ls, sf2, kernel="rbf", out: Optional[torch.Tensor] = None,
-                  kfu: Optional[torch.Tensor] = None, gate: Optional[torch.cuda.Event] = None) -> torch.Tensor:
+                  kfu: Optional[torch.Tensor] = None, gate: Optional[torch.cuda.Event] = None,
+                  kfu_q: Optional[torch.Tensor] = None) -> torch.Tensor:
         N, d = X.shape
         M = Z.shape[0]
         self._chk(Z, "Z")
@@ -159,8 +175,19 @@
             raise ValueError("unsupported shape N=%d M=%d d=%d (d <= %d, M <= %d)" % (N, M, d, _lib.SGP_MAX_DIM, _lib.SGP_MAX_INDUCING))
         ws = self._workspace("fwd_kfu" if kfu is not None else "fwd", nbytes)
         base = out.data_ptr()
+        if kfu_q is not None:
+            if kfu is not None:
+                raise ValueError("suffstats: kfu and kfu_q exclude each other")
+            self._chk_q(kfu_q, N, M)
         if gate is not None:
             self.lib.sgp_ctx_set_pass1_gate(self._c(), C.c_void_p(gate.cuda_event))
+        if kfu_q is not None:
+            st = self.lib.sgp_ctx_suffstats_fwd_qt(
+                self._c(), self._ptr(X), d, self._ptr(y), self._ptr(Z), d, self._inv_ls(ls, d, kernel), float(sf2), N, M, d,
+                _kernel_id(kernel), C.c_void_p(base), C.c_void_p(base + 8 * M * M), C.c_void_p(base + 8 * (M * M + M)),
+                C.c_void_p(base + 8 * (M * M + M + 1)), C.c_void_p(kfu_q.data_ptr()), self._ptr(ws), ws.numel(), self._stream())
+            _lib.check("sgp_suffstats_fwd_qt", st)
+            return out
         st = self.lib.sgp_ctx_suffstats_fwd(
             self._c(), self._ptr(X), d, self._ptr(y), self._ptr(Z), d, self._inv_ls(ls, d, kernel), float(sf2), N, M, d, _kernel_id(kernel),
             C.c_void_p(base), C.c_void_p(base + 8 * M * M), C.c_void_p(base + 8 * (M * M + M)),
@@ -559,12 +586,29 @@
                 ws[: self.lib.sgp_small_sync_bytes()].zero_()
 
     def suffstats_bwd(self, X, y, Z, ls, sf2, Phibar, bbar, kappabar, kernel="rbf", want_gz=False,
-                      out: Optional[torch.Tensor] = None, kfu: Optional[torch.Tensor] = None) -> torch.Tensor:
+                      out: Optional[torch.Tensor] = None, kfu: Optional[torch.Tensor] = None,
+                      kfu_q: Optional[torch.Tensor] = None) -> torch.Tensor:
         N, d = X.shape
         M = Z.shape[0]
         nh = self.hyper_len(kernel, d)
         if out is None:
             out = self.empty(nh + 1 + (M * d if want_gz else 0))
+        if kfu_q is not None:
+            if kfu is not None:
+                raise ValueError("suffstats_bwd: kfu and kfu_q exclude each other")
+            self._chk_q(kfu_q, N, M)
+            nbytes = self.lib.sgp_suffstats_bwd_qt_workspace_bytes(N, M, d)
+            if nbytes == 0:
+                raise ValueError("suffstats_bwd(kfu_q=): unsupported shape N=%d M=%d d=%d (d <= 8)" % (N, M, d))
+            ws = self._workspace("bwd_q", nbytes)
+            base = out.data_ptr()
+            st = self.lib.sgp_ctx_suffstats_bwd_qt(
+                self._c(), self._ptr(X), d, self._ptr(y), self._ptr(Z), d, self._inv_ls(ls, d, kernel), float(sf2), self._ptr(Phibar),
+                self._ptr(bbar), float(kappabar), C.c_void_p(kfu_q.data_ptr()), N, M, d, _kernel_id(kernel), C.c_void_p(base),
+                C.c_void_p(base + 8 * nh), C.c_void_p(base + 8 * (nh + 1)) if want_gz else C.c_void_p(0), self._ptr(ws), ws.numel(),
+                self._stream())
+            _lib.check("sgp_suffstats_bwd_qt", st)
+            return out
         nbytes = self.lib.sgp_suffstats_bwd_workspace_bytes_ex(N, M, d, 1 if kfu is not None else 0)
         ws = self._workspace("bwd_kfu" if kfu is not None else "bwd", nbytes)
         base = out.data_ptr()
diff --git a/include/sgp.h b/include/sgp.h
--- a/include/sgp.h
+++ b/include/sgp.h
@@ -58,6 +58,7 @@
 #define SGP_OPT_CU_BUDGET 4
 #define SGP_OPT_TIMING 5
 #define SGP_OPT_SHARED_DEVICE 6
+#define SGP_OPT_PASS2 7
 sgp_ctx* sgp_ctx_create(int device);
 void sgp_ctx_destroy(sgp_ctx* ctx);
 int sgp_ctx_device(const sgp_ctx* ctx);
@@ -67,6 +68,8 @@
 void sgp_ctx_set_pass1_gate(sgp_ctx* ctx, void* hip_event);
 int sgp_ctx_contraction_last(const sgp_ctx* ctx);
 int sgp_ctx_contraction_would_use_i8(const sgp_ctx* ctx, int64_t N, int M);
+int sgp_ctx_pass2_would_use_i8(const sgp_ctx* ctx, int64_t N, int M, int d, int kernel_id);
+int sgp_ctx_pass2_last(const sgp_ctx* ctx);
 int sgp_ctx_timing_last_ms(sgp_ctx* ctx, int slot, float* ms);
 int64_t sgp_ctx_timing_last_rows(const sgp_ctx* ctx, int slot);
 size_t sgp_ctx_suffstats_workspace_bytes(const sgp_ctx* ctx, int64_t N, int M, int d, int caller_owns_kfu);
@@ -77,6 +80,13 @@
                           const double* inv_ls, double sf2, const double* Phibar, const double* bbar, double kappabar,
                           const double* Kfu_in, int64_t N, int M, int d, int kernel_id, double* g_ls, double* g_sf2, double* g_Z,
                           void* ws, size_t ws_bytes, sgp_stream_t stream);
+int sgp_ctx_suffstats_fwd_qt(sgp_ctx* ctx, const double* X, int64_t ldx, const double* y, const double* Z, int64_t ldz,
+                             const double* inv_ls, double sf2, int64_t N, int M, int d, int kernel_id, double* Phi, double* b,
+                             double* yy, double* kappa, void* Qt_out, void* ws, size_t ws_bytes, sgp_stream_t stream);
+int sgp_ctx_suffstats_bwd_qt(sgp_ctx* ctx, const double* X, int64_t ldx, const double* y, const double* Z, int64_t ldz,
+                             const double* inv_ls, double sf2, const double* Phibar, const double* bbar, double kappabar,
+                             const void* Qt_in, int64_t N, int M, int d, int kernel_id, double* g_ls, double* g_sf2, double* g_Z,
+                             void* ws, size_t ws_bytes, sgp_stream_t stream);
 int sgp_ctx_kuu_factor(sgp_ctx* ctx, const double* Kuu, int M, double* Linv_out, int* info, void* ws, size_t ws_bytes,
                        sgp_stream_t stream);
 int sgp_ctx_kuu_factor_ex(sgp_ctx* ctx, const double* Kuu, int M, double* Linv_out, int* info, double* trace_out, void* ws,
@@ -129,6 +139,10 @@
 size_t sgp_suffstats_workspace_bytes(int64_t N, int M, int d);
 size_t sgp_suffstats_workspace_bytes_ex(int64_t N, int M, int d, int caller_owns_kfu);
 size_t sgp_kfu_len(int64_t N, int M);
+size_t sgp_kfu_digits_len(int64_t N, int M);
+int sgp_suffstats_fwd_qt(const double* X, int64_t ldx, const double* y, const double* Z, int64_t ldz, const double* inv_ls, double sf2,
+                         int64_t N, int M, int d, int kernel_id, double* Phi, double* b, double* yy, double* kappa, void* Qt_out, void* ws,
+                         size_t ws_bytes, sgp_stream_t stream);
 int sgp_set_contraction(int mode);
 int sgp_contraction_last(void);
 void sgp_set_pass1_gate(void* hip_event);
@@ -277,6 +291,10 @@
 
 size_t sgp_suffstats_bwd_workspace_bytes(int64_t N, int M, int d);
 size_t sgp_suffstats_bwd_workspace_bytes_ex(int64_t N, int M, int d, int caller_owns_kfu);
+size_t sgp_suffstats_bwd_qt_workspace_bytes(int64_t N, int M, int d);
+int sgp_suffstats_bwd_qt(const double* X, int64_t ldx, const double* y, const double* Z, int64_t ldz, const double* inv_ls, double sf2,
+                         const double* Phibar, const double* bbar, double kappabar, const void* Qt_in, int64_t N, int M, int d, int kernel_id,
+                         double* g_ls, double* g_sf2, double* g_Z, void* ws, size_t ws_bytes, sgp_stream_t stream);
 int sgp_suffstats_bwd(const double* X, int64_t ldx, const double* y,
                       const double* Z, int64_t ldz, const double* inv_ls, double sf2,
                       const double* Phibar, const double* bbar, double kappabar,
```
